# sandyresearch/chipmunk

Measured on AMD Instinct MI355X. Metric: DiT denoise steps/sec at fixed sparsity, higher is better.
Workload: dtype bf16

## Files before the change

chipmunk_amd/_native.py:

```python
from __future__ import annotations

import ctypes
import os

_HERE = os.path.dirname(os.path.abspath(__file__))
LIB_PATH = os.environ.get("CHIPMUNK_HIP_LIB") or os.path.join(_HERE, "lib", "libchipmunk_hip.so")

SYMBOLS = [
    "chipmunk_last_error", "chipmunk_abi_version", "chipmunk_set_option", "chipmunk_set_random_seed",
    "chipmunk_csp_attn", "chipmunk_csp_attn_out", "chipmunk_csp_128_attn", "chipmunk_dense_attn", "chipmunk_dense_colsum_attn",
    "chipmunk_csp_mlp_mm1", "chipmunk_csp_mlp_mm1_scatter", "chipmunk_csp_mlp_mm1_fp8", "chipmunk_csp_mlp_mm2_and_scatter_add", "chipmunk_csp_scatter_add", "chipmunk_csp_mlp_mm2",
    "chipmunk_csp_mlp_mm1_ragged", "chipmunk_csp_mlp_mm1_scatter_ragged", "chipmunk_csp_mlp_mm1_fp8_ragged", "chipmunk_csp_mlp_mm2_ragged",
    "chipmunk_csp_mlp_mm2_and_scatter_add_ragged", "chipmunk_csp_scatter_add_ragged", "chipmunk_block_mean_ragged", "chipmunk_transpose16_pitched",
    "chipmunk_topk_indices", "chipmunk_topk_delta_indices", "chipmunk_topk_mask", "chipmunk_mask_to_indices", "chipmunk_mask_to_sorted_indices", "chipmunk_packed_mask_to_indices", "chipmunk_copy_indices",
    "chipmunk_bitpack", "chipmunk_bitunpack", "chipmunk_transpose16", "chipmunk_block_mean", "chipmunk_quantize_fp8", "chipmunk_gather_rows", "chipmunk_qkv_split_norm", "chipmunk_dense_colsum_topk_mask", "chipmunk_dense_attn_strided", "chipmunk_csp_attn_out_ragged", "chipmunk_compact_indices", "chipmunk_residual_ln_modulate", "chipmunk_dense_colsum_attn_strided", "chipmunk_dense_colsum_topk_mask_strided", "chipmunk_release_scratch", "chipmunk_big_scratch_fallbacks",
    "chipmunk_host_alloc", "chipmunk_host_free", "chipmunk_copy_d2h_async", "chipmunk_copy_h2d_async", "chipmunk_host_bytes",
]

_lib = None


def lib() -> ctypes.CDLL:
    global _lib
    if _lib is None:
        if not os.path.exists(LIB_PATH):
            raise ImportError(
                f"{LIB_PATH} is missing: build it with `python -m chipmunk_amd.build` (hipcc --offload-arch=gfx950). "
                "chipmunk_amd has no CPU fallback.")
        _lib = ctypes.CDLL(LIB_PATH)
        _lib.chipmunk_last_error.restype = ctypes.c_char_p
        _lib.chipmunk_abi_version.restype = ctypes.c_int
        for item in filter(None, os.environ.get("CHIPMUNK_AMD_OPTIONS", "").split(",")):
            name, _, val = item.partition("=")
            if _lib.chipmunk_set_option(name.strip().encode(), int(val)) != 0:
                raise ValueError(f"CHIPMUNK_AMD_OPTIONS: {_lib.chipmunk_last_error().decode()}")
    return _lib


def last_error() -> str:
    return lib().chipmunk_last_error().decode()


def check(rc: int, what: str) -> None:
    if rc != 0:
        raise RuntimeError(f"{what}: {last_error()}")


def set_option(name: str, value: int) -> None:
    check(lib().chipmunk_set_option(name.encode(), int(value)), "chipmunk_set_option")


def manual_seed(seed: int) -> None:
    check(lib().chipmunk_set_random_seed(ctypes.c_uint64(int(seed) & 0xFFFFFFFFFFFFFFFF)), "chipmunk_set_random_seed")


class HostBuffer:

    def __init__(self, numel: int, dtype) -> None:
        import torch
        self.dtype = dtype
        self._numel = int(numel)
        self._itemsize = torch.empty(0, dtype=dtype).element_size()
        self.nbytes = self._numel * self._itemsize
        p = ctypes.c_void_p()
        check(lib().chipmunk_host_alloc(ctypes.c_size_t(max(self.nbytes, 1)), ctypes.byref(p)), "chipmunk_host_alloc")
        self.ptr = p.value

    def numel(self) -> int:
        return self._numel

    def element_size(self) -> int:
        return self._itemsize

    def is_pinned(self) -> bool:
        return True

    def free(self) -> None:
        if getattr(self, "ptr", None):
            lib().chipmunk_host_free(ctypes.c_void_p(self.ptr))
            self.ptr = None

    def __del__(self):
        try:
            self.free()
        except Exception:
            pass


def copy_d2h_async(host_ptr: int, dev_ptr: int, nbytes: int, stream: int) -> None:
    check(lib().chipmunk_copy_d2h_async(ctypes.c_void_p(host_ptr), ctypes.c_void_p(dev_ptr), ctypes.c_size_t(nbytes), ctypes.c_void_p(stream)),
          "chipmunk_copy_d2h_async")


def copy_h2d_async(dev_ptr: int, host_ptr: int, nbytes: int, stream: int) -> None:
    check(lib().chipmunk_copy_h2d_async(ctypes.c_void_p(dev_ptr), ctypes.c_void_p(host_ptr), ctypes.c_size_t(nbytes), ctypes.c_void_p(stream)),
          "chipmunk_copy_h2d_async")


def host_bytes() -> int:
    f = lib().chipmunk_host_bytes
    f.restype = ctypes.c_size_t
    return int(f())
```

chipmunk_amd/csrc/attn.hip:

```cpp
#include "common.h"
#include "attn_params.h"
#include <type_traits>

namespace {

constexpr int QG = 192;
constexpr int QW = 48;
constexpr int KVT = 32;
constexpr int NST = 4;
constexpr int KRING = 8;
constexpr int HD = 128;
constexpr int TILE_BYTES = KVT * HD * 2;
constexpr float SCALE_LOG2E = 0.08838834764f * 1.44269504089f;
constexpr int NSTV = NST + 1;
constexpr int KEY_RING_OFF = (NST + NSTV) * TILE_BYTES;
constexpr int CS_OFF = KEY_RING_OFF + KRING * 256;
constexpr int ATTN_LDS_BYTES = CS_OFF + 2 * 2 * 4 * KVT * 4;

__device__ __forceinline__ f32x4 mfma16(bf16x8 a, bf16x8 b, f32x4 c) {
    return __builtin_amdgcn_mfma_f32_16x16x32_bf16(a, b, c, 0, 0, 0);
}

#ifdef ATTN_PROF
__device__ unsigned long long g_attn_prof[8 * 8];
// ... 1062 lines not shown
    p.q = (const uint16_t *)q, p.k = (const uint16_t *)k, p.v = (const uint16_t *)v, p.o = (uint16_t *)o_out;
    p.o_in = (const uint16_t *)o_in;
    for (int i = 0; i < 3; ++i) p.qs[i] = q_strides[i], p.ks[i] = k_strides[i], p.vs[i] = v_strides[i], p.os[i] = o_strides[i];
    p.indices = indices, p.counts = counts;
    p.B = B, p.H = H, p.Nq = Nq, p.Nk = Nk, p.G = (Nq + QG - 1) / QG, p.idx_stride = idx_stride;
    p.o_scale = (float)o_scale;
    return launch_attn<true, true, false>(p, (hipStream_t)stream);
}

extern "C" int chipmunk_csp_attn_out_ragged(const void *q, const void *k, const void *v, const void *o_in, void *o_out,
                                            const int64_t q_strides[3], const int64_t k_strides[3], const int64_t v_strides[3],
                                            const int64_t o_strides[3], const int32_t *indices, const int64_t *idx_offsets,
                                            const int32_t *counts, int B, int H, int Nq, int Nk, int o_scale, void *stream) {
    if (int e = check_common(q, k, v, o_out, B, H, Nq, Nk)) return e;
    CM_CHECK(o_in != nullptr && ((uintptr_t)o_in & 15) == 0, "csp_attn_out_ragged: o_in missing or not 16-byte aligned");
    CM_CHECK(o_scale == 1 || o_scale == -1, "o_scale must be 1 or -1");
    CM_CHECK(indices && counts && idx_offsets, "csp_attn_out_ragged: indices / offsets / counts missing");
    CM_CHECK(((uintptr_t)indices & 15) == 0, "csp_attn_out_ragged: indices must be 16-byte aligned");
    if (int e = check_strides(q_strides, "q")) return e;
    if (int e = check_strides(k_strides, "k")) return e;
    if (int e = check_strides(v_strides, "v")) return e;
    if (int e = check_strides(o_strides, "o")) return e;
    AttnParams p = {};
    p.q = (const uint16_t *)q, p.k = (const uint16_t *)k, p.v = (const uint16_t *)v, p.o = (uint16_t *)o_out;
    p.o_in = (const uint16_t *)o_in;
    for (int i = 0; i < 3; ++i) p.qs[i] = q_strides[i], p.ks[i] = k_strides[i], p.vs[i] = v_strides[i], p.os[i] = o_strides[i];
    p.indices = indices, p.counts = counts, p.idx_off = idx_offsets;
    p.B = B, p.H = H, p.Nq = Nq, p.Nk = Nk, p.G = (Nq + QG - 1) / QG, p.idx_stride = 0;
    p.o_scale = (float)o_scale;
    return launch_attn<true, true, false>(p, (hipStream_t)stream);
}

extern "C" int chipmunk_csp_128_attn(const void *q, const void *k, const void *v, void *o, const int32_t *indices,
                                     const int32_t *counts, int B, int H, int Nq, int Nk, int idx_stride,
                                     void *stream) {
    if (int e = check_common(q, k, v, o, B, H, Nq, Nk)) return e;
    CM_CHECK(indices && counts, "csp_128_attn: indices / counts missing");
    AttnParams p = {};
    p.q = (const uint16_t *)q, p.k = (const uint16_t *)k, p.v = (const uint16_t *)v, p.o = (uint16_t *)o;
    contiguous_strides(p.qs, H, Nq), contiguous_strides(p.os, H, Nq);
    contiguous_strides(p.ks, H, Nk), contiguous_strides(p.vs, H, Nk);
    p.indices = indices, p.counts = counts;
    p.B = B, p.H = H, p.Nq = Nq, p.Nk = Nk, p.G = (Nq + QG - 1) / QG, p.idx_stride = idx_stride;
    p.o_scale = 1.f;
    return launch_attn<true, false, false>(p, (hipStream_t)stream);
}

static int output_strides(int64_t os[3], const int64_t *o_strides, int H, int Nq) {
    if (!o_strides) {
        contiguous_strides(os, H, Nq);
        return CHIPMUNK_OK;
    }
    for (int i = 0; i < 3; ++i) os[i] = o_strides[i];
    return check_strides(o_strides, "o");
}

extern "C" int chipmunk_dense_attn_strided(const void *q, const void *k, const void *v, const int64_t q_strides[3],
                                           const int64_t k_strides[3], const int64_t v_strides[3], void *o,
                                           const int64_t *o_strides, float *l, int B, int H, int Nq, int Nk, void *stream) {
    if (int e = check_common(q, k, v, o, B, H, Nq, Nk)) return e;
    CM_CHECK(l != nullptr, "dense_attn: l output missing");
    if (int e = check_strides(q_strides, "q")) return e;
    if (int e = check_strides(k_strides, "k")) return e;
    if (int e = check_strides(v_strides, "v")) return e;
    AttnParams p = {};
    p.q = (const uint16_t *)q, p.k = (const uint16_t *)k, p.v = (const uint16_t *)v, p.o = (uint16_t *)o;
    for (int i = 0; i < 3; ++i) p.qs[i] = q_strides[i], p.ks[i] = k_strides[i], p.vs[i] = v_strides[i];
    if (int e = output_strides(p.os, o_strides, H, Nq)) return e;
    p.l_out = l;
    p.B = B, p.H = H, p.Nq = Nq, p.Nk = Nk, p.G = (Nq + QG - 1) / QG;
    p.o_scale = 1.f;
    if (use_dense64(B, H, Nq, Nk)) {
        CM_CHECK((int64_t)Nk * p.ks[2] * 2 < (1ll << 32) && (int64_t)Nk * p.vs[2] * 2 < (1ll << 32),
                 "attention: one head's K or V spans more than 4 GiB (32-bit DMA offsets)");
        return chipmunk_dense64_launch(q, k, v, o, l, p.qs, p.ks, p.vs, p.os, B, H, Nq, Nk, (hipStream_t)stream);
    }
    return launch_attn<false, false, true>(p, (hipStream_t)stream);
}

extern "C" int chipmunk_dense_attn(const void *q, const void *k, const void *v, const int64_t q_strides[3],
                                   const int64_t k_strides[3], const int64_t v_strides[3], void *o, float *l, int B,
                                   int H, int Nq, int Nk, void *stream) {
    return chipmunk_dense_attn_strided(q, k, v, q_strides, k_strides, v_strides, o, nullptr, l, B, H, Nq, Nk, stream);
}

extern "C" int chipmunk_dense_colsum_attn_strided(const void *q, const void *k, const void *v, const int64_t q_strides[3],
                                                  const int64_t k_strides[3], const int64_t v_strides[3], const float *pin,
                                                  void *o, const int64_t *o_strides, void *cs, float *l, int B, int H, int Nq,
                                                  int Nk, int cs_stride, void *stream) {
    if (int e = check_common(q, k, v, o, B, H, Nq, Nk)) return e;
    CM_CHECK(l && cs && pin, "dense_colsum_attn: p / cs / l missing");
    CM_CHECK(cs_stride >= Nk, "dense_colsum_attn: cs row stride %d < Nk %d", cs_stride, Nk);
    if (int e = check_strides(q_strides, "q")) return e;
    if (int e = check_strides(k_strides, "k")) return e;
    if (int e = check_strides(v_strides, "v")) return e;
    AttnParams p = {};
    p.q = (const uint16_t *)q, p.k = (const uint16_t *)k, p.v = (const uint16_t *)v, p.o = (uint16_t *)o;
    for (int i = 0; i < 3; ++i) p.qs[i] = q_strides[i], p.ks[i] = k_strides[i], p.vs[i] = v_strides[i];
    if (int e = output_strides(p.os, o_strides, H, Nq)) return e;
    p.l_out = l, p.p_in = pin, p.cs = (uint16_t *)cs, p.cs_stride = cs_stride;
    p.B = B, p.H = H, p.Nq = Nq, p.Nk = Nk, p.G = (Nq + QG - 1) / QG;
    p.o_scale = 1.f;
    hipStream_t st = (hipStream_t)stream;
    int rc;
    if (chipmunk_get_option("attn_fused_colsum") == 5) {
        if (use_colsum64(B, H, Nq, Nk)) return chipmunk_colsum64_launch(p, st);
        return launch_attn<false, false, false, true>(p, st);
    }
    if (use_dense64(B, H, Nq, Nk)) {
        CM_CHECK((int64_t)Nk * p.ks[2] * 2 < (1ll << 32) && (int64_t)Nk * p.vs[2] * 2 < (1ll << 32),
                 "attention: one head's K or V spans more than 4 GiB (32-bit DMA offsets)");
        if (chipmunk_get_option("attn_fused_colsum") != 2) {
            int hc = H;
            uint16_t *part = nullptr;
            const int hc_min = chipmunk_get_option("attn_fused_colsum") == 4 ? 1 : 0;
            if (hc_min) hc = 1;
            for (; hc >= 1; hc /= 2) {
                part = (uint16_t *)chipmunk_big_scratch(st, chipmunk_colsum_part_bytes(hc == H ? B : 1, hc, Nq, Nk));
                if (part) break;
            }
            if (part && hc == H) return chipmunk_dense64_colsum_launch(p, part, st);
            if (part) {
                for (int b = 0; b < B; ++b)
                    for (int h0 = 0; h0 < H; h0 += hc) {
                        AttnParams c = p;
                        const int hn = H - h0 < hc ? H - h0 : hc;
                        const int64_t bh0 = (int64_t)b * H + h0;
                        c.q += b * p.qs[0] + h0 * p.qs[1], c.k += b * p.ks[0] + h0 * p.ks[1], c.v += b * p.vs[0] + h0 * p.vs[1];
                        c.o += b * p.os[0] + h0 * p.os[1];
                        c.l_out += bh0 * Nq, c.p_in += bh0 * Nq, c.cs += bh0 * p.G * (int64_t)cs_stride;
                        c.B = 1, c.H = hn;
                        if (int e = chipmunk_dense64_colsum_launch(c, part, st)) return e;
                    }
                return CHIPMUNK_OK;
            }
        }
        rc = chipmunk_dense64_launch(q, k, v, o, l, p.qs, p.ks, p.vs, p.os, B, H, Nq, Nk, st);
    } else {
        rc = launch_attn<false, false, true>(p, st);
    }
    if (rc != CHIPMUNK_OK) return rc;
    if (use_colsum64(B, H, Nq, Nk)) return chipmunk_colsum64_launch(p, st);
    return launch_attn<false, false, false, true>(p, st);
}

extern "C" int chipmunk_dense_colsum_attn(const void *q, const void *k, const void *v, const int64_t q_strides[3],
                                          const int64_t k_strides[3], const int64_t v_strides[3], const float *pin,
                                          void *o, void *cs, float *l, int B, int H, int Nq, int Nk, int cs_stride,
                                          void *stream) {
    return chipmunk_dense_colsum_attn_strided(q, k, v, q_strides, k_strides, v_strides, pin, o, nullptr, cs, l, B, H, Nq, Nk,
                                              cs_stride, stream);
}

extern "C" int chipmunk_dense_colsum_topk_mask_strided(const void *q, const void *k, const void *v, const int64_t q_strides[3],
                                               const int64_t k_strides[3], const int64_t v_strides[3], const float *pin, void *o,
                                               const int64_t *o_strides, float *l, int B, int H, int Nq, int Nk, const void *static_mask,
                                               int64_t static_stride, int static_rows, const void *group_flags, void *mask,
                                               int topk, double random_amount, void *stream) {
    if (int e = check_common(q, k, v, o, B, H, Nq, Nk)) return e;
    CM_CHECK(l && pin && mask, "dense_colsum_topk_mask: p / l / mask missing");
    if (int e = check_strides(q_strides, "q")) return e;
    if (int e = check_strides(k_strides, "k")) return e;
    if (int e = check_strides(v_strides, "v")) return e;
    hipStream_t st = (hipStream_t)stream;
    if (!use_dense64(B, H, Nq, Nk) || chipmunk_get_option("attn_fused_colsum") == 2 || (Nk & 3) || Nk > 1024 * 120)
        return CHIPMUNK_ERR_UNSUPPORTED;
    AttnParams p = {};
    p.q = (const uint16_t *)q, p.k = (const uint16_t *)k, p.v = (const uint16_t *)v, p.o = (uint16_t *)o;
    for (int i = 0; i < 3; ++i) p.qs[i] = q_strides[i], p.ks[i] = k_strides[i], p.vs[i] = v_strides[i];
    CM_CHECK((int64_t)Nk * p.ks[2] * 2 < (1ll << 32) && (int64_t)Nk * p.vs[2] * 2 < (1ll << 32),
             "attention: one head's K or V spans more than 4 GiB (32-bit DMA offsets)");
    if (int e = output_strides(p.os, o_strides, H, Nq)) return e;
    p.l_out = l, p.p_in = pin, p.cs = nullptr, p.cs_stride = 0;
    p.B = B, p.H = H, p.Nq = Nq, p.Nk = Nk, p.G = (Nq + QG - 1) / QG;
    p.o_scale = 1.f;
    uint16_t *part = (uint16_t *)chipmunk_big_scratch(st, chipmunk_colsum_part_bytes(B, H, Nq, Nk));
    if (!part) return CHIPMUNK_ERR_UNSUPPORTED;
    if (int e = chipmunk_dense64_colsum_launch(p, part, st)) return e;
    const int nrb = ((Nq + 255) / 256) * 2;
    return chipmunk_topk_mask_parts(part, chipmunk_colsum_part_stride(Nk), nrb, p.G, Nq, static_mask, static_stride, static_rows, group_flags, mask, B * H * p.G, Nk,
                                    topk, random_amount, st);
}

extern "C" int chipmunk_dense_colsum_topk_mask(const void *q, const void *k, const void *v, const int64_t q_strides[3],
                                               const int64_t k_strides[3], const int64_t v_strides[3], const float *pin, void *o,
                                               float *l, int B, int H, int Nq, int Nk, const void *static_mask,
                                               int64_t static_stride, int static_rows, const void *group_flags, void *mask,
                                               int topk, double random_amount, void *stream) {
    return chipmunk_dense_colsum_topk_mask_strided(q, k, v, q_strides, k_strides, v_strides, pin, o, nullptr, l, B, H, Nq, Nk,
                                                   static_mask, static_stride, static_rows, group_flags, mask, topk, random_amount,
                                                   stream);
}
```

chipmunk_amd/csrc/attn64.hip:

```cpp
#include "common.h"
#include "attn64_regs.h"
#include "attn_params.h"
#include "attn64_util.h"
#include <type_traits>

namespace {

constexpr int HD = 128;
constexpr int KT = 64;
constexpr int WROWS = 64, WGROWS = 256;
constexpr int TB = KT * HD * 2;
constexpr int NSL = 4;
constexpr int VRING = NSL * TB;
constexpr int LDS_BYTES = 2 * NSL * TB;
constexpr int PSTAGE = 64 * 128;
constexpr int LDS_BYTES_CSUM = LDS_BYTES + 4 * PSTAGE;
constexpr int CS_EXCH_BYTES = 2 * 4 * 64 * 4;
constexpr float SCALE_LOG2E = 0.08838834764f * 1.44269504089f;
constexpr float MAX_LAG = 4.0f;
#ifndef A64_ABL
#define A64_ABL 0
#endif
#ifndef A64_EB
#define A64_EB 20
#endif
#ifndef A64_EA
#define A64_EA 35
#endif
#ifndef A64_CSUM_VALU
#define A64_CSUM_VALU 1
#endif
#ifndef A64_VSPREAD
#define A64_VSPREAD 0
#endif
#ifndef A64_DMA_POS
#define A64_DMA_POS 2
#endif

constexpr int a64_ecum(int k) {
    return k <= 0 ? 0 : k <= 20 ? (k * A64_EB) / 20 : k <= 52 ? A64_EB + ((k - 20) * A64_EA) / 32
                                                              : (A64_EB + A64_EA + (k - 52) < 64 ? A64_EB + A64_EA + (k - 52) : 64);
}
constexpr int a64_cstep(int j) {
    int k = 0;
    while (a64_ecum(k) < 2 * j + 2) ++k;
    return k;
}
constexpr int a64_rk(int u) { return u == 0 ? 36 : u == 1 ? 38 : u == 2 ? 68 : 70; }
constexpr int a64_mk(int u) { return u == 0 ? 46 : u == 1 ? 48 : u == 2 ? 78 : 80; }

#ifdef ATTN64_PROF
__device__ unsigned long long g_a64_prof[4 * 8];
#define P64_DECL unsigned long long pt_ = 0, pacc_[7] = {0, 0, 0, 0, 0, 0, 0}; const bool prof_on_ = blockIdx.x == (gridDim.x / 2)
#define P64_START() do { if (prof_on_) pt_ = __builtin_amdgcn_s_memtime(); } while (0)
#define P64_MARK(i) do { if (prof_on_) { const unsigned long long n_ = __builtin_amdgcn_s_memtime(); pacc_[i] += n_ - pt_; pt_ = n_; } } while (0)
#define P64_END(w, n) do { if (prof_on_ && lane == 0) { for (int i_ = 0; i_ < 7; ++i_) g_a64_prof[(w) * 8 + i_] = pacc_[i_]; g_a64_prof[(w) * 8 + 7] = (n); } } while (0)
#else
#define P64_DECL
#define P64_START()
#define P64_MARK(i)
#define P64_END(w, n)
#endif

template <int KB, int QB, int KS>
__device__ __forceinline__ void mfma_qk(f32x16 &s) {
    constexpr int ka = 192 + (KB * 8 + KS) * 4, qa = 128 + (QB * 8 + KS) * 4;
    if constexpr (A64_ABL & 64) {
        constexpr int oa = (KB * 2 + QB) * 16;
        asm volatile("v_mfma_f32_32x32x16_bf16 a[%c0:%c1], a[%c2:%c3], a[%c4:%c5], a[%c0:%c1]" ::"i"(oa), "i"(oa + 15), "i"(ka), "i"(ka + 3), "i"(qa), "i"(qa + 3));
        return;
    }
    if constexpr (KS == 0)
        asm volatile("v_mfma_f32_32x32x16_bf16 %0, a[%c1:%c2], a[%c3:%c4], 0" : "=v"(s) : "i"(ka), "i"(ka + 3), "i"(qa), "i"(qa + 3));
    else
        asm volatile("v_mfma_f32_32x32x16_bf16 %0, a[%c1:%c2], a[%c3:%c4], %0" : "+v"(s) : "i"(ka), "i"(ka + 3), "i"(qa), "i"(qa + 3));
}
template <int QB, int DB>
__device__ __forceinline__ void mfma_pv(const u32x4 &vf, const u32x4 &pf) {
    constexpr int oa = (QB * 4 + DB) * 16;
    asm volatile("v_mfma_f32_32x32x16_bf16 a[%c2:%c3], %0, %1, a[%c2:%c3]" ::"v"(vf), "v"(pf), "i"(oa), "i"(oa + 15));
}
template <int KB, int KS, int SLOT>
__device__ __forceinline__ void lds_k(uint32_t addr) {
    constexpr int ka = 192 + (KB * 8 + KS) * 4;
    asm volatile("ds_read_b128 a[%c1:%c2], %0 offset:%c3" ::"v"(addr), "i"(ka), "i"(ka + 3), "i"(SLOT * TB + KB * 8192) : "memory");
}
__device__ __forceinline__ void cs_pair16x2(float &a, float &b, float &c, float &d) {
    asm volatile("v_permlane16_swap_b32 %0, %1\n\tv_permlane16_swap_b32 %2, %3\n\tv_add_f32 %0, %0, %1\n\tv_add_f32 %2, %2, %3"
                 : "+v"(a), "+v"(b), "+v"(c), "+v"(d));
}
__device__ __forceinline__ void cs_pair8(float &a, const float &b) {
    asm volatile("v_add_f32_dpp %0, %0, %0 row_mirror row_mask:0xf bank_mask:0x3\n\t"
                 "v_add_f32_dpp %0, %1, %1 row_mirror row_mask:0xf bank_mask:0xc" : "+v"(a) : "v"(b));
}
__device__ __forceinline__ void cs_pair4(float &a, const float &b) {
    asm volatile("v_add_f32_dpp %0, %0, %0 row_half_mirror row_mask:0xf bank_mask:0x5\n\t"
                 "v_add_f32_dpp %0, %1, %1 row_half_mirror row_mask:0xf bank_mask:0xa" : "+v"(a) : "v"(b));
}
template <int CTRL>
__device__ __forceinline__ float cs_pair_quad(float a, float b, bool hi) {
    const float keep = hi ? b : a, give = hi ? a : b;
    return keep + __uint_as_float((uint32_t)__builtin_amdgcn_update_dpp(0, (int)__float_as_uint(give), CTRL, 0xf, 0xf, true));
}
__global__ __launch_bounds__(256) void knorm_max_kernel(const uint16_t *k, const int64_t ks0, const int64_t ks1, const int64_t ks2, int H, int Nk,
                                                        float *out) {
    const int bh = blockIdx.y, b = bh / H, h = bh - b * H;
    const uint16_t *kb = k + b * ks0 + h * ks1;
    const int grp = threadIdx.x >> 4, li = threadIdx.x & 15;
    float best = 0.f;
#pragma unroll 4
    for (int row = blockIdx.x * 16 + grp; row < Nk; row += gridDim.x * 16) {
        const u32x4 v = *(const u32x4 *)(kb + (int64_t)row * ks2 + li * 8);
        float ss = 0.f;
#pragma unroll
        for (int e = 0; e < 4; ++e) {
            const float lo = __uint_as_float(v[e] << 16), hi = __uint_as_float(v[e] & 0xffff0000u);
            ss = __builtin_fmaf(lo, lo, ss);
            ss = __builtin_fmaf(hi, hi, ss);
        }
        best = fmaxf(best, row16_sum(ss));
    }
    __shared__ float red[256];
    red[threadIdx.x] = best;
    __syncthreads();
    for (int st = 128; st > 0; st >>= 1) {
        if ((int)threadIdx.x < st) red[threadIdx.x] = fmaxf(red[threadIdx.x], red[threadIdx.x + st]);
        __syncthreads();
    }
    if (threadIdx.x == 0) atomicMax((unsigned int *)(out + bh), __float_as_uint(__builtin_sqrtf(red[0])));
}

template <int MODE>
__global__ __launch_bounds__(256) __attribute__((amdgpu_waves_per_eu(1, 1))) void attn64_kernel(const AttnParams p) {
    constexpr bool GATHER = MODE == 1 || MODE == 2, INPLACE = MODE == 2;
    constexpr bool CSUM = MODE == 3;
    extern __shared__ __attribute__((aligned(16))) unsigned char smem[];
    const int tid = threadIdx.x, lane = tid & 63;
    const int w = __builtin_amdgcn_readfirstlane(tid >> 6);
    const int l31 = lane & 31, hf = lane >> 5, l15 = lane & 15, lg = lane >> 4;
    int wid = blockIdx.x, sp = 0, nsp = 1, slot0 = 0, tix = 0;
    if constexpr (GATHER) {
        const int wid0 = wid;
        wid = p.plan[2 * wid0];
        if (wid < 0) return;
        const int meta = p.plan[2 * wid0 + 1];
        sp = meta & 0xff, nsp = (meta >> 8) & 0xff;
        slot0 = tix = meta >> 16;
    }
    const int bh = wid / p.G, g = wid - bh * p.G;
    const int b = bh / p.H, h = bh - b * p.H;
    const int row0 = g * (GATHER ? 192 : WGROWS) + w * WROWS;
    const int count = GATHER ? p.counts[(int64_t)bh * p.G + g] : p.Nk;
    const int valid = count < p.Nk ? count : p.Nk;
    const int ntiles_all = (valid + KT - 1) / KT;
    const int tbeg = (int)((int64_t)ntiles_all * sp / nsp), tend = (int)((int64_t)ntiles_all * (sp + 1) / nsp);
    const int ntiles = tend - tbeg;
    const int T4 = (ntiles + 3) & ~3;

    const uint16_t *kbase = p.k + b * p.ks[0] + h * p.ks[1];
    const uint16_t *vbase = p.v + b * p.vs[0] + h * p.vs[1];
    const __amdgpu_buffer_rsrc_t krsrc = make_rsrc(kbase), vrsrc = make_rsrc(vbase);
    const uint32_t kstride_b = (uint32_t)p.ks[2] * 2u, vstride_b = (uint32_t)p.vs[2] * 2u;

    if (GATHER && w == 3) {
        const IndexRow irow = index_row(p, (int64_t)bh * p.G + g);
        const int32_t *idx = irow.ptr;
        uint32_t kswz[4];
#pragma unroll
        for (int i = 0; i < 4; ++i) kswz[i] = (uint32_t)(l15 ^ (4 * i + lg)) << 4;
        const uint32_t vswz = (uint32_t)(l15 ^ (lg << 2)) << 4;
        int ir[4][16];
        const bool idx_vec = ((uintptr_t)idx & 15) == 0 && (irow.width & 3) == 0;
        auto load_idx = [&](int T, int (&dst)[16]) {
            const int base = (tbeg + T) * KT + lg * 16;
            if (idx_vec && (tbeg + T) * KT + KT <= irow.width) {
#pragma unroll
                for (int j4 = 0; j4 < 4; ++j4) {
                    const u32x4 v4 = *(const u32x4 *)(idx + base + j4 * 4);
#pragma unroll
                    for (int e = 0; e < 4; ++e) dst[j4 * 4 + e] = (int)v4[e];
                }
            } else {
#pragma unroll
                for (int j = 0; j < 16; ++j) {
                    int pos = base + j;
                    pos = pos < irow.width ? pos : irow.width - 1;
                    dst[j] = idx[pos];
                }
            }
#pragma unroll
            for (int j = 0; j < 16; ++j) dst[j] = max(0, min(dst[j], p.Nk - 1));
        };
        auto all_k = [&](const int (&src)[16], int slot) {
#pragma unroll
            for (int pc = 0; pc < 16; ++pc) blds16(krsrc, __umul24((uint32_t)src[pc], kstride_b) + kswz[pc & 3], 0, smem + slot * TB + pc * 1024);
        };
        auto all_v = [&](const int (&src)[16], int slot) {
#pragma unroll
            for (int pc = 0; pc < 16; ++pc) blds16(vrsrc, __umul24((uint32_t)src[pc], vstride_b) + vswz, 0, smem + VRING + slot * TB + pc * 1024);
        };
        load_idx(0, ir[0]), load_idx(1, ir[1]), load_idx(2, ir[2]), load_idx(3, ir[3]);
        all_k(ir[0], 0);
        all_k(ir[1], 1), all_v(ir[0], 3);
        all_k(ir[2], 2), all_v(ir[0], 0);
        all_k(ir[3], 3), all_v(ir[1], 1);
        load_idx(4, ir[0]);
        asm volatile("s_waitcnt vmcnt(0)" ::: "memory");
        __syncthreads();
        auto loader_tile = [&](auto slc, int t) __attribute__((always_inline)) {
            constexpr int SL = decltype(slc)::value;
            asm volatile("s_waitcnt vmcnt(63)" ::: "memory");
            __builtin_amdgcn_s_barrier();
            load_idx(t + 5, ir[(SL + 1) & 3]);
            all_k(ir[SL], SL);
            all_v(ir[(SL + 2) & 3], (SL + 2) & 3);
        };
        for (int tb = 0;; tb += 4) {
            loader_tile(ic<0>{}, tb);
            if (tb >= T4) break;
            loader_tile(ic<1>{}, tb + 1);
            loader_tile(ic<2>{}, tb + 2);
            loader_tile(ic<3>{}, tb + 3);
        }
        asm volatile("s_waitcnt vmcnt(0)" ::: "memory");
        if (nsp > 1) {
            __syncthreads();
            __syncthreads();
            if (*(volatile int *)(smem) != nsp - 1) return;
            __syncthreads();
        }
        return;
    }

    asm volatile(A64_ZERO_O ::: A64_CLOBBER_ALL);
    float qss[2] = {0.f, 0.f};
    {
        const uint16_t *qp = p.q + b * p.qs[0] + h * p.qs[1];
        static_for<0, 16>([&](auto f) {
            constexpr int F = decltype(f)::value, qb = F >> 3, ks = F & 7;
            const int qrow = row0 + qb * 32 + l31;
            u32x4 val = {0u, 0u, 0u, 0u};
            if (qrow < p.Nq) val = *(const u32x4 *)(qp + (int64_t)qrow * p.qs[2] + ks * 16 + hf * 8);
            acc_write4<128 + F * 4>(val);
#pragma unroll
            for (int e = 0; e < 4; ++e) {
                const float lo = __uint_as_float(val[e] << 16), hi = __uint_as_float(val[e] & 0xffff0000u);
                qss[qb] = __builtin_fmaf(lo, lo, qss[qb]);
                qss[qb] = __builtin_fmaf(hi, hi, qss[qb]);
            }
        });
    }

    const uint32_t lds0 = (uint32_t)(uintptr_t)(__attribute__((address_space(3))) unsigned char *)smem;
    uint32_t kad[8];
#pragma unroll
    for (int ks = 0; ks < 8; ++ks) kad[ks] = lds0 + l31 * 256 + (((2 * ks + hf) ^ l15) << 4);
    uint32_t vad[4];
#pragma unroll
    for (int db = 0; db < 4; ++db)
        vad[db] = lds0 + VRING + (4 * hf + (l15 >> 2)) * 256 + (((db * 4 + 2 * (lg & 1) + ((l15 & 3) >> 1)) ^ ((l15 >> 2) << 2)) << 4) +
                  (l15 & 1) * 8;
    uint32_t kofs[4];
#pragma unroll
    for (int i = 0; i < 4; ++i) kofs[i] = (uint32_t)(w * 16 + 4 * i + lg) * kstride_b + ((uint32_t)(l15 ^ (4 * i + lg)) << 4);
    const uint32_t vofs = (uint32_t)(w * 16 + lg) * vstride_b + ((uint32_t)(l15 ^ (lg << 2)) << 4);

    const int last_base = p.Nk - KT;
    auto tile_base = [&](int T) { return T * KT < last_base ? T * KT : last_base; };
    auto issue_k1 = [&](uint32_t soff, uint32_t ldsw, int slot, int i) {
        blds16(krsrc, kofs[i], soff, smem + ldsw + slot * TB + i * 1024);
    };
    auto issue_v1 = [&](uint32_t soff, uint32_t ldsw, int slot, int i) {
        blds16(vrsrc, vofs, soff + (uint32_t)(4 * i) * vstride_b, smem + ldsw + VRING + slot * TB + i * 1024);
    };
    auto issue_k = [&](int T, int slot) {
        const uint32_t soff = (uint32_t)tile_base(T) * kstride_b;
#pragma unroll
        for (int i = 0; i < 4; ++i) issue_k1(soff, w * 4096, slot, i);
    };
    auto issue_v = [&](int T, int slot) {
        const uint32_t soff = (uint32_t)tile_base(T) * vstride_b;
#pragma unroll
        for (int i = 0; i < 4; ++i) issue_v1(soff, w * 4096, slot, i);
    };

    if constexpr (!GATHER) {
        issue_k(0, 0);
        issue_k(1, 1), issue_v(0, 3);
        issue_k(2, 2), issue_v(0, 0);
        issue_k(3, 3), issue_v(1, 1);
        asm volatile("s_waitcnt vmcnt(24)" ::: "memory");
    }
    __syncthreads();
    static_for<0, 16>([&](auto i) {
        constexpr int I = decltype(i)::value;
        lds_k<(I >> 3), (I & 7), 0>(kad[I & 7]);
    });
    asm volatile("s_waitcnt lgkmcnt(0)" ::: "memory");

    f32x16 s[4];
    float px[64];
    uint32_t pw[2][4][4] = {};
    float m[2] = {-INFINITY, -INFINITY}, nmsc[2] = {0.f, 0.f};
    float mlag[2] = {-INFINITY, -INFINITY};
    float lacc[2][2] = {{0.f, 0.f}, {0.f, 0.f}};
    float alpha[2] = {1.f, 1.f};
    float wq[2] = {0.f, 0.f}, lpq[2] = {-1.0e30f, -1.0e30f}, c4[2] = {0.f, 0.f}, c5 = 0.f;
    uint32_t csoff = 0, ex_w = 0, ex_r = 0;
    int cs_extra = 0;
    float cs_own = 0.f;
    __amdgpu_buffer_rsrc_t prsrc = krsrc;
    uint32_t pst_w = 0, pst_r = 0, csoff_mx = 0;
    u32x2 csf[8] = {};
    f32x4 csacc[2] = {{0.f, 0.f, 0.f, 0.f}, {0.f, 0.f, 0.f, 0.f}};
    float csout = 0.f;
    u32x4 cs_ones = {0x3f803f80u, 0x3f803f80u, 0x3f803f80u, 0x3f803f80u};
    if constexpr (CSUM) {
        static_assert(A64_CSUM_VALU, "the matrix-pipe column-sum probe (A64_CSUM_VALU=0) fills all 160 KiB of LDS with its P stage: no room for the exchange area of the in-workgroup combine; build round 5's tree for it");
        pin(cs_ones);
        const uint32_t pst = lds0 + LDS_BYTES + (uint32_t)w * PSTAGE;
        pst_w = pst + l31 * 128 + ((uint32_t)(hf ^ (l31 & 7)) << 4);
        const int prow = lg * 4 + (l15 >> 2);
        pst_r = pst + prow * 128 + ((uint32_t)(((l15 & 3) >> 1) ^ (prow & 7)) << 4) + (l15 & 1) * 8;
        csoff_mx = 2u * (uint32_t)(16 * lg + 8 * ((l15 >> 2) & 1) + 4 * (l15 >> 3) + (l15 & 3));
#pragma unroll
        for (int qb = 0; qb < 2; ++qb) {
            const int qrow = row0 + qb * 32 + l31;
            const float pl = qrow < p.Nq ? p.p_in[(int64_t)bh * p.Nq + qrow] : 0.f;
            lpq[qb] = pl > 0.f ? __builtin_amdgcn_logf(pl) : -1.0e30f;
        }
        const int rr = ((lane >> 4) & 1) | (((lane >> 3) & 1) << 1) | (((lane >> 2) & 1) << 2);
        csoff = 2u * (uint32_t)(32 * (lane & 1) + (rr & 3) + 8 * (2 * ((lane >> 1) & 1) + (rr >> 2)) + 4 * hf);
        const int nA = 3 - (4 * g) % 3;
        const int lead = w < nA ? 0 : nA, members = w < nA ? nA : 4 - nA;
        cs_extra = w == lead ? members : 0;
        ex_w = lds0 + LDS_BYTES + (uint32_t)w * 256u + (uint32_t)lane * 4u;
        ex_r = lds0 + LDS_BYTES + (uint32_t)(lead + 1) * 256u + (uint32_t)lane * 4u;
        prsrc = make_rsrc(p.cs_part + ((int64_t)bh * (p.G * 2) + (g * 2 + (w < nA ? 0 : 1))) * p.cs_pstride);
    }
#pragma unroll
    for (int e = 0; e < 64; ++e) px[e] = e < 20 ? 0.f : -INFINITY;

    auto vfrag_read = [&](auto dbc, auto offc) __attribute__((always_inline)) {
        constexpr int DB = decltype(dbc)::value, OFF = decltype(offc)::value;
        u32x2 lo, hi;
        asm volatile("ds_read_b64_tr_b16 %0, %2 offset:%c3\n\tds_read_b64_tr_b16 %1, %2 offset:%c4"
                     : "=&v"(lo), "=&v"(hi) : "v"(vad[DB]), "i"(OFF), "i"(OFF + 2048) : "memory");
        return (u32x4){lo[0], lo[1], hi[0], hi[1]};
    };

    static_assert(64 - A64_EB - A64_EA >= 0 && 64 - A64_EB - A64_EA <= 9, "the last steps must finish before gap 12 of the next PV phase");
    auto ecum = [](int k) constexpr { return a64_ecum(k); };
    auto finish_step = [&](auto kk, auto uwc) __attribute__((always_inline)) {
        constexpr int K = decltype(kk)::value;
        constexpr bool UW = decltype(uwc)::value != 0;
        if constexpr (!(A64_ABL & 1)) {
            static_for<ecum(K), ecum(K + 1)>([&](auto ii) {
                constexpr int I = decltype(ii)::value;
                if constexpr (A64_ABL & 32) px[I] = px[I] * 0.5f;
                else px[I] = __builtin_amdgcn_exp2f(px[I]);
                pin(px[I]);
            });
            static_for<ecum(K - 1), ecum(K)>([&](auto ii) {
                constexpr int I = decltype(ii)::value;
                lacc[(I >> 3) & 1][I & 1] += px[I];
                pin(lacc[(I >> 3) & 1][I & 1]);
            });
            static_for<(ecum(K - 1) >> 1), (ecum(K) >> 1)>([&](auto jj) {
                constexpr int J = decltype(jj)::value, I = 2 * J;
                pw[(I >> 3) & 1][I >> 4][(I & 7) >> 1] = pack_bf16x2(px[I], px[I + 1]);
                pin(pw[(I >> 3) & 1][I >> 4][(I & 7) >> 1]);
            });
            if constexpr (CSUM && UW && !A64_CSUM_VALU) {
                static_assert(a64_cstep(8 * 1 + 7) + 1 < a64_rk(0) && a64_cstep(8 * 3 + 7) + 1 < a64_rk(2), "a unit is read after its second fragment is stored");
                static_for<0, 4>([&](auto uu) {
                    constexpr int U = decltype(uu)::value, S = (U & 1) * 4;
                    if constexpr (K == a64_mk(U) || K == a64_mk(U) + 1) {
                        constexpr int H2 = K - a64_mk(U);
                        if constexpr (H2 == 0 && (U & 1) == 0)
                            asm volatile("s_waitcnt lgkmcnt(0)" : "+v"(csf[0]), "+v"(csf[1]), "+v"(csf[2]), "+v"(csf[3]), "+v"(csf[4]), "+v"(csf[5]), "+v"(csf[6]), "+v"(csf[7]) :: "memory");
                        const u32x4 fr = {csf[S + 2 * H2][0], csf[S + 2 * H2][1], csf[S + 2 * H2 + 1][0], csf[S + 2 * H2 + 1][1]};
                        if constexpr (H2 == 0) asm volatile("v_mfma_f32_16x16x32_bf16 %0, %1, %2, 0" : "=&v"(csacc[U & 1]) : "v"(cs_ones), "v"(fr));
                        else asm volatile("v_mfma_f32_16x16x32_bf16 %0, %1, %2, %0" : "+v"(csacc[U & 1]) : "v"(cs_ones), "v"(fr));
                    }
                    if constexpr (K == a64_mk(U) + 3) {
                        if constexpr (U == 0) csout = csacc[0][0];
                        else csout = lg == U ? csacc[U & 1][0] : csout;
                        pin(csout);
                    }
                    if constexpr (K == a64_rk(U) || K == a64_rk(U) + 1) {
                        constexpr int H2 = K - a64_rk(U);
                        uint32_t ad = pst_r;
                        if constexpr (U != 0) ad ^= (uint32_t)(U << 5);
                        asm volatile("ds_read_b64_tr_b16 %0, %2 offset:%c3\n\tds_read_b64_tr_b16 %1, %2 offset:%c4"
                                     : "=&v"(csf[S + 2 * H2]), "=&v"(csf[S + 2 * H2 + 1]) : "v"(ad), "i"(H2 * 4096), "i"(H2 * 4096 + 2048) : "memory");
                    }
                });
                static_for<0, 8>([&](auto ii) {
                    constexpr int U = decltype(ii)::value >> 1, QW = decltype(ii)::value & 1;
                    if constexpr (K == a64_cstep(8 * U + 4 * QW + 3) + 1) {
                        uint32_t ad = pst_w;
                        if constexpr (U != 0) ad ^= (uint32_t)(U << 5);
                        const u32x4 pf = {pw[QW][U][0], pw[QW][U][1], pw[QW][U][2], pw[QW][U][3]};
                        asm volatile("ds_write_b128 %0, %1 offset:%c2" ::"v"(ad), "v"(pf), "i"(QW * 4096) : "memory");
                    }
                });
            } else if constexpr (CSUM) {
                static_for<ecum(K - 3), ecum(K - 2)>([&](auto ii) {
                    constexpr int I = decltype(ii)::value;
                    if constexpr (UW) {
                        if constexpr (((I >> 3) & 1) == 1) { px[I] += px[I - 8]; pin(px[I]); }
                    } else {
                        if constexpr (((I >> 3) & 1) == 0) px[I] *= wq[0];
                        else px[I] = __builtin_fmaf(px[I], wq[1], px[I - 8]);
                        pin(px[I]);
                    }
                });
                static_for<ecum(K - 4), ecum(K - 3)>([&](auto ii) {
                    constexpr int I = decltype(ii)::value;
                    if constexpr ((I & 11) == 11) cs_pair16x2(px[I - 3], px[I - 2], px[I - 1], px[I]);
                });
                static_for<ecum(K - 5), ecum(K - 4)>([&](auto ii) {
                    constexpr int I = decltype(ii)::value;
                    if constexpr ((I & 11) == 11) cs_pair8(px[I - 3], px[I - 1]);
                });
                static_for<ecum(K - 6), ecum(K - 5)>([&](auto ii) {
                    constexpr int I = decltype(ii)::value;
                    if constexpr ((I & 15) == 15) cs_pair4(px[I - 7], px[I - 3]);
                });
                static_for<ecum(K - 7), ecum(K - 6)>([&](auto ii) {
                    constexpr int I = decltype(ii)::value;
                    if constexpr ((I & 31) == 31) { c4[I >> 5] = cs_pair_quad<0x4E>(px[I - 23], px[I - 7], (lane & 2) != 0); pin(c4[I >> 5]); }
                });
                static_for<ecum(K - 8), ecum(K - 7)>([&](auto ii) {
                    constexpr int I = decltype(ii)::value;
                    if constexpr (I == 63) { c5 = cs_pair_quad<0xB1>(c4[0], c4[1], (lane & 1) != 0); pin(c5); }
                });
            }
        }
    };

    P64_DECL;
    P64_START();
    auto tile = [&](auto slc, auto nmc, int t) __attribute__((always_inline)) {
        constexpr int SL = decltype(slc)::value;
        constexpr bool NOMAX = decltype(nmc)::value != 0;
        constexpr auto uwc = ic<(CSUM && decltype(nmc)::value == 2) ? 1 : 0>{};
        constexpr int VSL = (SL + 3) & 3;
        constexpr int KNSL = (SL + 1) & 3;
        uint32_t ldsw = w * 4096, ksoff = 0, vsoff = 0;
        if constexpr (!(A64_ABL & 16)) {
            if constexpr (!(A64_ABL & 256) && !GATHER) asm volatile("s_waitcnt vmcnt(16)" ::: "memory");
            if constexpr (!(A64_ABL & 128)) __builtin_amdgcn_s_barrier();
            if constexpr (!GATHER) {
                asm volatile("" : "+s"(ldsw));
                ksoff = (uint32_t)tile_base(t + 4) * kstride_b;
                vsoff = (uint32_t)tile_base(t + 2) * vstride_b;
            }
        }
        __builtin_amdgcn_sched_barrier(0);
        P64_MARK(0);

        u32x4 vf[16];
        static_for<0, 32>([&](auto gg) {
            constexpr int G = decltype(gg)::value;
            constexpr int ks = G >> 2, kb = (G >> 1) & 1, qb = G & 1;
            mfma_qk<kb, qb, ks>(s[kb * 2 + qb]);
            if constexpr (!(A64_ABL & 16) && !GATHER && ((A64_DMA_POS == 0 && G < 8) || (A64_DMA_POS == 2 && G >= 16 && (G & 1) == 0))) {
                constexpr int PC = A64_DMA_POS == 0 ? G : (G - 16) >> 1;
                if constexpr (PC < 4) issue_k1(ksoff, ldsw, SL, PC);
                else issue_v1(vsoff, ldsw, (SL + 2) & 3, PC - 4);
            }
            finish_step(ic<20 + G>{}, uwc);
            if constexpr (A64_VSPREAD ? (G & 1) == 0 : G < 16) {
                constexpr int f = A64_VSPREAD ? G >> 1 : G;
                if constexpr (A64_ABL & 4) vf[f] = (u32x4){(uint32_t)t, 1u, 2u, 3u};
                else vf[f] = vfrag_read(ic<(f & 3)>{}, ic<VSL * TB + (f >> 2) * 4096>{});
            }
            __builtin_amdgcn_sched_barrier(0);
        });
        P64_MARK(1);
        asm volatile("s_waitcnt lgkmcnt(0)"
                     : "+v"(vf[0]), "+v"(vf[1]), "+v"(vf[2]), "+v"(vf[3]), "+v"(vf[4]), "+v"(vf[5]), "+v"(vf[6]), "+v"(vf[7]), "+v"(vf[8]),
                       "+v"(vf[9]), "+v"(vf[10]), "+v"(vf[11]), "+v"(vf[12]), "+v"(vf[13]), "+v"(vf[14]), "+v"(vf[15]));
        __builtin_amdgcn_sched_barrier(0);
        P64_MARK(2);

        float mx[2];
        bool moved = false;
        const int dead = GATHER ? 0 : (t * KT - tile_base(t) < KT ? t * KT - tile_base(t) : KT);
        const int vleft = !GATHER ? KT : (t < ntiles ? valid - (tbeg + t) * KT : 0);
        auto phase_b_gap = [&](auto gg) __attribute__((always_inline)) {
            constexpr int G = decltype(gg)::value;
            constexpr int up = G >> 3, db = (G >> 1) & 3, qb = G & 1;
            const u32x4 pf = {pw[qb][up][0], pw[qb][up][1], pw[qb][up][2], pw[qb][up][3]};
            mfma_pv<qb, db>(vf[G >> 1], pf);
            constexpr bool UWT = decltype(uwc)::value != 0 && !A64_CSUM_VALU;
            if constexpr (G < (CSUM ? (UWT ? 32 : 17) : 12)) finish_step(ic<52 + G>{}, uwc);
            if constexpr (CSUM && G == (UWT ? 31 : 17)) {
                const uint32_t par2 = (uint32_t)(t & 1) * 1024u;
                const float mine = UWT ? csout : c5;
                if (!cs_extra) {
                    asm volatile("ds_write_b32 %0, %1" ::"v"(ex_w + (par2 ^ 1024u)), "v"(mine) : "memory");
                } else {
                    float x1 = 0.f, x2 = 0.f;
                    if (cs_extra >= 2) asm volatile("ds_read_b32 %0, %1" : "=v"(x1) : "v"(ex_r + par2) : "memory");
                    if (cs_extra >= 3) asm volatile("ds_read_b32 %0, %1 offset:256" : "=v"(x2) : "v"(ex_r + par2) : "memory");
                    asm volatile("ds_write_b32 %0, %1" ::"v"(ex_w + (par2 ^ 1024u)), "v"(mine) : "memory");
                    asm volatile("s_waitcnt lgkmcnt(1)" : "+v"(x1), "+v"(x2)::"memory");
                    const int tb2 = tile_base(t - 2), dd = (t - 2) * KT - tb2;
                    if (t > 1 && dd < KT) {
                        const uint32_t off = UWT ? csoff_mx : csoff;
                        if (dd <= 0 || (int)(off >> 1) >= dd) {
                            const uint16_t val = (uint16_t)(pack_bf16x2((cs_own + x1) + x2, 0.f) & 0xffffu);
                            if (p.probe & 16) __builtin_amdgcn_raw_buffer_store_b16(val, prsrc, off, (uint32_t)tb2 * 2u, 2);
                            else __builtin_amdgcn_raw_buffer_store_b16(val, prsrc, off, (uint32_t)tb2 * 2u, 0);
                        }
                    }
                }
                cs_own = mine;
            }
            if constexpr (!(A64_ABL & 16) && !GATHER && A64_DMA_POS == 1 && G >= 16 && (G & 1) == 0) {
                constexpr int PC = (G - 16) >> 1;
                if constexpr (PC < 4) issue_k1(ksoff, ldsw, SL, PC);
                else issue_v1(vsoff, ldsw, (SL + 2) & 3, PC - 4);
            }
            if constexpr (G < 16 && !(A64_ABL & 8)) {
                constexpr int J = G;
                lds_k<(J >> 3), (J & 7), KNSL>(kad[J & 7]);
            }
            if constexpr (G == 1 && !(A64_ABL & 2)) {
                if (!GATHER && __builtin_expect(dead > 0, 0)) {
                    int thr = dead - 4 * hf;
                    asm volatile("" : "+v"(thr));
#pragma unroll
                    for (int blk = 0; blk < 4; ++blk)
#pragma unroll
                        for (int r = 0; r < 16; ++r)
                            if ((blk >> 1) * 32 + (r & 3) + 8 * (r >> 2) < thr) s[blk][r] = -INFINITY;
                }
                if (GATHER && __builtin_expect(vleft < KT, 0)) {
                    int thr = vleft - hf;
                    asm volatile("" : "+v"(thr));
#pragma unroll
                    for (int blk = 0; blk < 4; ++blk)
#pragma unroll
                        for (int r = 0; r < 16; ++r)
                            if ((r & 3) * 16 + (blk >> 1) * 8 + 2 * (r >> 2) >= thr) s[blk][r] = -INFINITY;
                }
            }
            if constexpr (G >= 2 && G <= 9 && !(A64_ABL & 2) && !NOMAX) {
                constexpr int j = G - 2;
                constexpr int kb2 = j >> 2, r0 = (j & 3) * 4;
                if constexpr (j == 0)
                    asm volatile("v_max_f32 %0, %2, %3\n\tv_max_f32 %1, %6, %7\n\tv_max3_f32 %0, %0, %4, %5\n\tv_max3_f32 %1, %1, %8, %9"
                                 : "=&v"(mx[0]), "=&v"(mx[1])
                                 : "v"(s[0][0]), "v"(s[0][1]), "v"(s[0][2]), "v"(s[0][3]), "v"(s[1][0]), "v"(s[1][1]), "v"(s[1][2]), "v"(s[1][3]));
                else
                asm volatile("v_max3_f32 %0, %0, %2, %3\n\tv_max3_f32 %1, %1, %6, %7\n\tv_max3_f32 %0, %0, %4, %5\n\tv_max3_f32 %1, %1, %8, %9"
                             : "+v"(mx[0]), "+v"(mx[1])
                             : "v"(s[kb2 * 2][r0]), "v"(s[kb2 * 2][r0 + 1]), "v"(s[kb2 * 2][r0 + 2]), "v"(s[kb2 * 2][r0 + 3]),
                               "v"(s[kb2 * 2 + 1][r0]), "v"(s[kb2 * 2 + 1][r0 + 1]), "v"(s[kb2 * 2 + 1][r0 + 2]), "v"(s[kb2 * 2 + 1][r0 + 3]));
            }
            if constexpr (G == 10 && !(A64_ABL & 2) && !NOMAX) {
#pragma unroll
                for (int q2 = 0; q2 < 2; ++q2) {
                    float a = mx[q2], c = mx[q2];
                    lane_swap32(a, c);
                    mx[q2] = max2(a, c);
                    pin(mx[q2]);
                }
            }
            if constexpr (G >= 12 && G < 28 && !(A64_ABL & 2)) {
                static_for<(G - 12) * 4, (G - 11) * 4>([&](auto ii) {
                    constexpr int I = decltype(ii)::value;
                    constexpr int blk = (I >> 5) * 2 + ((I >> 3) & 1), r = ((I >> 4) & 1) * 8 + (I & 7);
                    px[I] = __builtin_fmaf(s[blk][r], SCALE_LOG2E, nmsc[(I >> 3) & 1]);
                    pin(px[I]);
                });
            }
            if constexpr (G >= 12) finish_step(ic<G - 12>{}, uwc);
            __builtin_amdgcn_sched_barrier(0);
        };
        static_for<0, 12>(phase_b_gap);
        P64_MARK(3);
        if constexpr (!(A64_ABL & 2) && !NOMAX) {
            constexpr float LAG_RAW = MAX_LAG / SCALE_LOG2E;
            if (__builtin_amdgcn_ballot_w64(mx[0] > mlag[0]) | __builtin_amdgcn_ballot_w64(mx[1] > mlag[1])) {
                moved = true;
#pragma unroll
                for (int q2 = 0; q2 < 2; ++q2) {
                    const float m_new = max2(m[q2], mx[q2]);
                    alpha[q2] = __builtin_amdgcn_exp2f((m[q2] - m_new) * SCALE_LOG2E);
                    lacc[q2][0] *= alpha[q2];
                    lacc[q2][1] *= alpha[q2];
                    m[q2] = m_new;
                    nmsc[q2] = -m_new * SCALE_LOG2E;
                    mlag[q2] = m_new + LAG_RAW;
                    if constexpr (CSUM) wq[q2] = fminf(__builtin_amdgcn_exp2f(m_new * SCALE_LOG2E + lpq[q2]), 1.0e37f);
                }
            }
        }
        __builtin_amdgcn_sched_barrier(0);
        P64_MARK(4);
        static_for<12, 32>(phase_b_gap);
        P64_MARK(5);
        if (__builtin_expect(moved, 0)) {
            float tmp;
            asm volatile("s_nop 7\n\ts_nop 7\n\ts_nop 7\n\t" A64_SCALE_QB0 : "=&v"(tmp) : "v"(alpha[0]));
            asm volatile(A64_SCALE_QB1 : "=&v"(tmp) : "v"(alpha[1]));
        }
        asm volatile("s_waitcnt lgkmcnt(0)" ::: "memory");
        __builtin_amdgcn_sched_barrier(0);
        P64_MARK(6);
    };

    bool nomax = false;
    if constexpr (!GATHER) {
        if (p.kmax) {
            const float km = p.kmax[bh];
            bool ok = true;
#pragma unroll
            for (int qb = 0; qb < 2; ++qb) {
                float a = qss[qb], c2 = qss[qb];
                lane_swap32(a, c2);
                const float mq = __builtin_sqrtf(a + c2) * km;
                ok = ok && (2.0f * mq * SCALE_LOG2E <= 64.0f);
                qss[qb] = mq;
            }
            nomax = __builtin_amdgcn_ballot_w64(!ok) == 0;
            if (nomax) {
#pragma unroll
                for (int qb = 0; qb < 2; ++qb) {
                    m[qb] = qss[qb], nmsc[qb] = -qss[qb] * SCALE_LOG2E, mlag[qb] = INFINITY;
                    if constexpr (CSUM) wq[qb] = fminf(__builtin_amdgcn_exp2f(qss[qb] * SCALE_LOG2E + lpq[qb]), 1.0e37f);
                }
            }
        }
    }
    bool unitw = false;
    if constexpr (CSUM) {
        if (nomax && !(p.probe & 4)) {
            bool ok = true;
#pragma unroll
            for (int qb = 0; qb < 2; ++qb) ok = ok && lpq[qb] > -1.0e29f && qss[qb] * SCALE_LOG2E + __builtin_fabsf(lpq[qb]) <= 80.0f;
            unitw = __builtin_amdgcn_ballot_w64(!ok) == 0;
            if (unitw) {
#pragma unroll
                for (int qb = 0; qb < 2; ++qb) m[qb] = -lpq[qb] / SCALE_LOG2E, nmsc[qb] = lpq[qb];
            }
        }
    }
    if (CSUM && unitw) {
        if constexpr (CSUM) {
            for (int tb = 0;; tb += 4) {
                tile(ic<0>{}, ic<2>{}, tb);
                if (tb >= T4) break;
                tile(ic<1>{}, ic<2>{}, tb + 1);
                tile(ic<2>{}, ic<2>{}, tb + 2);
                tile(ic<3>{}, ic<2>{}, tb + 3);
            }
        }
    } else if (nomax) {
        for (int tb = 0;; tb += 4) {
            tile(ic<0>{}, ic<1>{}, tb);
            if (tb >= T4) break;
            tile(ic<1>{}, ic<1>{}, tb + 1);
            tile(ic<2>{}, ic<1>{}, tb + 2);
            tile(ic<3>{}, ic<1>{}, tb + 3);
        }
    } else {
        for (int tb = 0;; tb += 4) {
            tile(ic<0>{}, ic<0>{}, tb);
            if (tb >= T4) break;
            tile(ic<1>{}, ic<0>{}, tb + 1);
            tile(ic<2>{}, ic<0>{}, tb + 2);
            tile(ic<3>{}, ic<0>{}, tb + 3);
        }
    }
    asm volatile("s_waitcnt vmcnt(0)" ::: "memory");
    P64_END(w, T4 + 1);
    if constexpr (CSUM) {
        asm volatile("s_waitcnt lgkmcnt(0)" ::: "memory");
        __builtin_amdgcn_s_barrier();
        if (cs_extra) {
            float x1 = 0.f, x2 = 0.f;
            const uint32_t par = (uint32_t)((T4 - 1) & 1) * 1024u;
            if (cs_extra >= 2) asm volatile("ds_read_b32 %0, %1" : "=v"(x1) : "v"(ex_r + par) : "memory");
            if (cs_extra >= 3) asm volatile("ds_read_b32 %0, %1 offset:256" : "=v"(x2) : "v"(ex_r + par) : "memory");
            asm volatile("s_waitcnt lgkmcnt(0)" : "+v"(x1), "+v"(x2)::"memory");
            const int tb1 = tile_base(T4 - 1), dd = (T4 - 1) * KT - tb1;
            const uint32_t off = (unitw && !A64_CSUM_VALU) ? csoff_mx : csoff;
            if (dd < KT && (dd <= 0 || (int)(off >> 1) >= dd))
                __builtin_amdgcn_raw_buffer_store_b16((uint16_t)(pack_bf16x2((cs_own + x1) + x2, 0.f) & 0xffffu), prsrc, off, (uint32_t)tb1 * 2u, 0);
        }
    }

    asm volatile("s_nop 7\n\ts_nop 7\n\ts_nop 7" ::: "memory");
    float o[128];
    static_for<0, 32>([&](auto ii) {
        constexpr int I = decltype(ii)::value;
        const f32x4 o4 = acc_read4<I * 4>();
        o[I * 4 + 0] = o4[0], o[I * 4 + 1] = o4[1], o[I * 4 + 2] = o4[2], o[I * 4 + 3] = o4[3];
    });
    float lq[2];
#pragma unroll
    for (int qb = 0; qb < 2; ++qb) {
        float lp = lacc[qb][0] + lacc[qb][1], lo2 = lp;
        lane_swap32(lp, lo2);
        lq[qb] = lp + lo2;
    }

    if constexpr (GATHER) {
        if (nsp > 1) {
            constexpr int SLICE_FLOATS = 26 * 256 * 4;
            int *ticket_s = (int *)smem;
            float *mine = p.ws + (int64_t)(slot0 + sp) * SLICE_FLOATS + tid;
#pragma unroll
            for (int i = 0; i < 128; ++i) mine[i * 192] = o[i];
            mine[128 * 192] = m[0], mine[129 * 192] = m[1], mine[130 * 192] = lq[0], mine[131 * 192] = lq[1];
            __syncthreads();
            if (tid == 0) {
                __builtin_amdgcn_fence(__ATOMIC_RELEASE, "agent");
                asm volatile("s_waitcnt vmcnt(0)" ::: "memory");
                *ticket_s = __hip_atomic_fetch_add(p.tickets + tix, 1, __ATOMIC_RELAXED, __HIP_MEMORY_SCOPE_AGENT);
            }
            __syncthreads();
            if (*ticket_s != nsp - 1) return;
            if (tid == 0) {
                __hip_atomic_store(p.tickets + tix, 0, __ATOMIC_RELAXED, __HIP_MEMORY_SCOPE_AGENT);
                __builtin_amdgcn_fence(__ATOMIC_ACQUIRE, "agent");
            }
            __syncthreads();
#pragma unroll
            for (int i = 0; i < 128; ++i) o[i] = 0.f;
            m[0] = m[1] = -INFINITY, lq[0] = lq[1] = 0.f;
            for (int s2 = 0; s2 < nsp; ++s2) {
                const float *oth = p.ws + (int64_t)(slot0 + s2) * SLICE_FLOATS + tid;
#pragma unroll
                for (int qb = 0; qb < 2; ++qb) {
                    const float ms = oth[(128 + qb) * 192], ls = oth[(130 + qb) * 192];
                    const float m_new = fmaxf(m[qb], ms);
                    if (m_new == -INFINITY) continue;
                    const float a = __builtin_amdgcn_exp2f((m[qb] - m_new) * SCALE_LOG2E);
                    const float c = __builtin_amdgcn_exp2f((ms - m_new) * SCALE_LOG2E);
                    m[qb] = m_new;
                    lq[qb] = lq[qb] * a + ls * c;
#pragma unroll
                    for (int i = 0; i < 64; ++i) o[qb * 64 + i] = o[qb * 64 + i] * a + oth[(qb * 64 + i) * 192] * c;
                }
            }
        }
    }

#pragma unroll
    for (int qb = 0; qb < 2; ++qb) {
        const float l = lq[qb];
        const float inv = l > 0.f ? __builtin_amdgcn_rcpf(l) : 0.f;
        const int qrow = row0 + qb * 32 + l31;
        if (qrow >= p.Nq) continue;
        const int64_t ooff = b * p.os[0] + h * p.os[1] + (int64_t)qrow * p.os[2] + 4 * hf;
        uint16_t *op = p.o + ooff;
#pragma unroll
        for (int i = 0; i < 16; ++i) {
            const int db = i >> 2, r4 = i & 3;
            const float *o4 = o + (qb * 4 + db) * 16 + r4 * 4;
            float x0 = o4[0] * inv, x1 = o4[1] * inv, x2 = o4[2] * inv, x3 = o4[3] * inv;
            u32x2 out;
            if constexpr (INPLACE) {
                const u32x2 old = *(const u32x2 *)(p.o_in + ooff + db * 32 + r4 * 8);
                const float a0 = round_bf16(x0 * p.o_scale), a1 = round_bf16(x1 * p.o_scale);
                const float a2 = round_bf16(x2 * p.o_scale), a3 = round_bf16(x3 * p.o_scale);
                out[0] = pack_bf16x2(__uint_as_float(old[0] << 16) + a0, __uint_as_float(old[0] & 0xffff0000u) + a1);
                out[1] = pack_bf16x2(__uint_as_float(old[1] << 16) + a2, __uint_as_float(old[1] & 0xffff0000u) + a3);
            } else {
                out[0] = pack_bf16x2(x0, x1);
                out[1] = pack_bf16x2(x2, x3);
            }
            *(u32x2 *)(op + db * 32 + r4 * 8) = out;
        }
        if (!GATHER && p.l_out && hf == 0)
            p.l_out[(int64_t)bh * p.Nq + qrow] = 1.0f / (__builtin_amdgcn_exp2f(m[qb] * SCALE_LOG2E) * l);
    }
}

template <int QB, int KB, int KS>
__device__ __forceinline__ void mfma_cs(f32x16 &d, const f32x16 &c0) {
    constexpr int qa = (QB * 8 + KS) * 4, ka = 192 + (KB * 8 + KS) * 4;
    if constexpr (KS == 0)
        asm volatile("v_mfma_f32_32x32x16_bf16 %0, a[%c2:%c3], a[%c4:%c5], %1" : "=&v"(d) : "v"(c0), "i"(qa), "i"(qa + 3), "i"(ka), "i"(ka + 3));
    else
        asm volatile("v_mfma_f32_32x32x16_bf16 %0, a[%c1:%c2], a[%c3:%c4], %0" : "+v"(d) : "i"(qa), "i"(qa + 3), "i"(ka), "i"(ka + 3));
}

__global__ __launch_bounds__(256) __attribute__((amdgpu_waves_per_eu(1, 1))) void colsum64_kernel(const AttnParams p) {
    extern __shared__ __attribute__((aligned(16))) unsigned char smem[];
    const int tid = threadIdx.x, lane = tid & 63;
    const int w = __builtin_amdgcn_readfirstlane(tid >> 6);
    const int l31 = lane & 31, hf = lane >> 5, l15 = lane & 15, lg = lane >> 4;
    const int G4 = (p.G + 3) / 4;
    const int wid = blockIdx.x;
    const int bh = __builtin_amdgcn_readfirstlane(wid / G4), g = (wid - bh * G4) * 4 + w;
    const int b = __builtin_amdgcn_readfirstlane(bh / p.H), h = bh - b * p.H;
    const int row0 = g * 192;
    const int ntiles = (p.Nk + KT - 1) / KT;
    const int T4 = (ntiles + 3) & ~3;
    const uint16_t *kbase = p.k + b * p.ks[0] + h * p.ks[1];
    const __amdgpu_buffer_rsrc_t krsrc = make_rsrc(kbase);
    const uint32_t kstride_b = (uint32_t)p.ks[2] * 2u;

    asm volatile("" ::: A64_CLOBBER_ALL);
    {
        const uint16_t *qp = p.q + b * p.qs[0] + h * p.qs[1];
        static_for<0, 48>([&](auto f) {
            constexpr int F = decltype(f)::value, qb = F >> 3, ks = F & 7;
            const int qrow = row0 + qb * 32 + l31;
            bf16x8 val = {};
            if (g < p.G && qrow < p.Nq) val = *(const bf16x8 *)(qp + (int64_t)qrow * p.qs[2] + ks * 16 + hf * 8);
#pragma unroll
            for (int e = 0; e < 8; ++e) val[e] = (__bf16)((float)val[e] * SCALE_LOG2E);
            acc_write4<F * 4>(__builtin_bit_cast(u32x4, val));
        });
    }
    f32x16 offs[6];
#pragma unroll
    for (int qb = 0; qb < 6; ++qb)
#pragma unroll
        for (int r = 0; r < 16; ++r) {
            const int qr = row0 + qb * 32 + (r & 3) + 8 * (r >> 2) + 4 * hf;
            const float pl = (g < p.G && qr < p.Nq) ? p.p_in[(int64_t)bh * p.Nq + qr] : 0.f;
            offs[qb][r] = pl > 0.f ? __builtin_amdgcn_logf(pl) : -1.0e30f;
        }

    const uint32_t lds0 = (uint32_t)(uintptr_t)(__attribute__((address_space(3))) unsigned char *)smem;
    uint32_t kad[8];
#pragma unroll
    for (int ks = 0; ks < 8; ++ks) kad[ks] = lds0 + l31 * 256 + (((2 * ks + hf) ^ l15) << 4);
    uint32_t kofs[4];
#pragma unroll
    for (int i = 0; i < 4; ++i) kofs[i] = (uint32_t)(w * 16 + 4 * i + lg) * kstride_b + ((uint32_t)(l15 ^ (4 * i + lg)) << 4);
    const int last_base = p.Nk - KT;
    auto tile_base = [&](int T) { return T * KT < last_base ? T * KT : last_base; };
// ... 203 lines not shown
```

chipmunk_amd/csrc/attn_params.h:

```cpp
#pragma once
#include <stdint.h>
#include <hip/hip_runtime.h>

struct AttnParams {
    const uint16_t *q, *k, *v;
    uint16_t *o;
    const uint16_t *o_in;
    int64_t qs[3], ks[3], vs[3], os[3];
    const int32_t *indices, *counts;
    const int64_t *idx_off;
    float *l_out;
    const float *p_in;
    uint16_t *cs;
    int cs_stride;
    int B, H, Nq, Nk, G, idx_stride;
    float o_scale;
    int split_full, nsplit;
    float *ws;
    int32_t *tickets;
    const int32_t *plan;
    int xcd_chunks;
    const float *kmax;
    uint16_t *cs_part;
    int cs_pstride;
    int probe;
};


int chipmunk_csp64_launch(const AttnParams &p, int inplace, int grid, hipStream_t stream);
int chipmunk_dense64_colsum_launch(const AttnParams &p, uint16_t *part, hipStream_t stream);
int chipmunk_topk_mask_parts(const uint16_t *part, int part_stride, int nrb, int groups_per_bh, int Nq, const void *static_mask, int64_t static_stride,
                             int static_rows, const void *group_flags, void *mask, int rows, int n, int k, double random_amount,
                             hipStream_t stream);
size_t chipmunk_colsum_part_bytes(int B, int H, int Nq, int Nk);
int chipmunk_colsum_part_stride(int Nk);
int chipmunk_colsum64_launch(const AttnParams &p, hipStream_t stream);
int chipmunk_csp96_launch(const AttnParams &p, int inplace, int grid, hipStream_t stream);
const float *chipmunk_knorm_max(const uint16_t *k, const int64_t ks[3], int B, int H, int Nk, hipStream_t stream);

__host__ __device__ inline int colsum_part_rows(int j, int nwg, int &r0, int &r1) {
    const int a = (3 * j) >> 2, w0 = 3 * j - 4 * a;
    r0 = 2 * a + (w0 ? 1 : 0);
    r1 = 2 * (a + 1);
    return (w0 >= 2 && a + 1 < nwg) ? 2 : 1;
}

struct IndexRow {
    const int32_t *ptr;
    int width;
};
__device__ __forceinline__ IndexRow index_row(const AttnParams &p, int64_t item) {
    if (p.idx_off) {
        const int64_t o = p.idx_off[item];
        return {p.indices + o, (int)(p.idx_off[item + 1] - o)};
    }
    return {p.indices + item * p.idx_stride, p.idx_stride};
}
```

chipmunk_amd/csrc/indexed_io.hip:

```cpp
#include "common.h"
#include "attn_params.h"

namespace {

__device__ __forceinline__ uint32_t wave_incl_scan(uint32_t x) {
    x += (uint32_t)__builtin_amdgcn_update_dpp(0, (int)x, 0x111, 0xf, 0xf, true);
    x += (uint32_t)__builtin_amdgcn_update_dpp(0, (int)x, 0x112, 0xf, 0xf, true);
    x += (uint32_t)__builtin_amdgcn_update_dpp(0, (int)x, 0x114, 0xf, 0xf, true);
    x += (uint32_t)__builtin_amdgcn_update_dpp(0, (int)x, 0x118, 0xf, 0xf, true);
    x += (uint32_t)__builtin_amdgcn_update_dpp(0, (int)x, 0x142, 0xa, 0xf, false);
    x += (uint32_t)__builtin_amdgcn_update_dpp(0, (int)x, 0x143, 0xc, 0xf, false);
    return x;
}
struct M2IParams {
    const uint8_t *mask;
    int32_t *indices;
    int32_t *counts;
    int n, pad_n, multiple_of;
};

template <bool PACKED, bool SORTED = false>
__global__ __launch_bounds__(256) void mask_to_indices_kernel(const M2IParams p) {
    extern __shared__ __attribute__((aligned(16))) unsigned char smem[];
    const int n = p.n;
// ... 321 lines not shown
#pragma unroll
        for (int j = 0; j < 16; ++j)
            if (keepbits & (1u << j)) {
                const int c = pass0 + j * 1024 + tid;
                out[base + tot[j * 16 + w] + before[j]] = c;
                if constexpr (DELTA) xc[c] = x[c];
            }
        base += tot[256];
        __syncthreads();
    }
    const int kept = base;
    const int mod = kept % p.multiple_of;
    const int pad = mod == 0 ? 0 : p.multiple_of - mod;
    if (tid == 0) p.counts[row] = kept + pad;
    if (pad > 0) {
        int pbase = 0;
        const int slot = compact_slot(my_last_invalid != -1, lane, w, wave_tot, pbase);
        if (slot >= 0 && slot < pad) {
            out[kept + slot] = my_last_invalid;
            if constexpr (DELTA) xc[my_last_invalid] = x[my_last_invalid];
        }
    }
}

template <typename T>
__global__ __launch_bounds__(256) void copy_indices_kernel(const T *src, T *dst, const int32_t *inds,
                                                           const int32_t *counts, int M, int R, int F) {
    const int64_t grow = blockIdx.x;
    const int64_t b = grow / ((int64_t)M * R);
    const int base_m = (int)((grow % ((int64_t)M * R)) / R);
    const int cnt = counts[b * M + base_m];
    const int32_t *ii = inds + (b * M + base_m) * (int64_t)F;
    for (int c = threadIdx.x; c < cnt; c += 256) {
        const int col = ii[c];
        dst[grow * F + col] = src[grow * F + col];
    }
}

__global__ __launch_bounds__(256) void bitpack_kernel(const uint8_t *mask, uint8_t *packed, int64_t n) {
    const int64_t nb = (n + 7) >> 3;
    for (int64_t i = (int64_t)blockIdx.x * 256 + threadIdx.x; i < nb; i += (int64_t)gridDim.x * 256) {
        uint8_t byte = 0;
        if (i * 8 + 8 <= n && ((((uintptr_t)mask) & 7) == 0)) {
            unsigned long long v = *(const unsigned long long *)(mask + i * 8);
#pragma unroll
            for (int j = 0; j < 8; ++j) byte |= (uint8_t)((((v >> (8 * j)) & 0xffull) != 0) << j);
        } else {
            for (int j = 0; j < 8 && i * 8 + j < n; ++j) byte |= (uint8_t)((mask[i * 8 + j] != 0) << j);
        }
        packed[i] = byte;
    }
}
__global__ __launch_bounds__(256) void bitunpack_kernel(const uint8_t *packed, uint8_t *mask, int64_t n) {
    const int64_t nb = (n + 7) >> 3;
    for (int64_t i = (int64_t)blockIdx.x * 256 + threadIdx.x; i < nb; i += (int64_t)gridDim.x * 256) {
        const uint8_t byte = packed[i];
        if (i * 8 + 8 <= n && ((((uintptr_t)mask) & 7) == 0)) {
            unsigned long long v = 0;
#pragma unroll
            for (int j = 0; j < 8; ++j) v |= (unsigned long long)((byte >> j) & 1u) << (8 * j);
            *(unsigned long long *)(mask + i * 8) = v;
        } else {
            for (int j = 0; j < 8 && i * 8 + j < n; ++j) mask[i * 8 + j] = (byte >> j) & 1u;
        }
    }
}

__global__ __launch_bounds__(256) void transpose16_kernel(const uint16_t *src, uint16_t *dst, int R, int C, int ld) {
    __shared__ __attribute__((aligned(16))) uint16_t tile[64][72];
    const int64_t boff = (int64_t)blockIdx.z * R * C;
    const int r0 = blockIdx.y * 64, c0 = blockIdx.x * 64;
    const int tid = threadIdx.x;
#pragma unroll
    for (int i = 0; i < 2; ++i) {
        const int item = i * 256 + tid, r = item >> 3, ch = item & 7;
        u32x4 v = {0u, 0u, 0u, 0u};
        if (r0 + r < R && c0 + ch * 8 + 8 <= C) v = *(const u32x4 *)(src + boff + (int64_t)(r0 + r) * C + c0 + ch * 8);
        else if (r0 + r < R)
            for (int e = 0; e < 8; ++e)
                if (c0 + ch * 8 + e < C) {
                    const uint32_t x = src[boff + (int64_t)(r0 + r) * C + c0 + ch * 8 + e];
                    v[e >> 1] |= x << (16 * (e & 1));
                }
#pragma unroll
        for (int e = 0; e < 4; ++e) {
            tile[ch * 8 + 2 * e][r] = (uint16_t)(v[e] & 0xffffu);
            tile[ch * 8 + 2 * e + 1][r] = (uint16_t)(v[e] >> 16);
        }
    }
    __syncthreads();
#pragma unroll
    for (int i = 0; i < 2; ++i) {
        const int item = i * 256 + tid, c = item >> 3, ch = item & 7;
        if (c0 + c >= C) continue;
        uint16_t *d = dst + (int64_t)blockIdx.z * C * ld + (int64_t)(c0 + c) * ld + r0 + ch * 8;
        if (r0 + ch * 8 + 8 <= ld && ((ld & 7) == 0)) *(u32x4 *)d = *(const u32x4 *)&tile[c][ch * 8];
        else
            for (int e = 0; e < 8; ++e)
                if (r0 + ch * 8 + e < ld) d[e] = tile[c][ch * 8 + e];
    }
}

__global__ __launch_bounds__(256) void compact_indices_kernel(const int32_t *indices, int64_t idx_stride, const int32_t *counts,
                                                             const int64_t *offsets, int32_t *flat) {
    const int64_t r = blockIdx.x;
    const int32_t *src = indices + r * idx_stride;
    const int64_t o = offsets[r];
    int32_t *dst = flat + o;
    const int width = (int)(offsets[r + 1] - o);
    int c = counts[r];
    c = c < 0 ? 0 : (c < width ? c : width);
    c = c < idx_stride ? c : (int)idx_stride;
    if ((((uintptr_t)src | (uintptr_t)dst) & 15) == 0) {
        const int c4 = c >> 2;
        for (int i = threadIdx.x; i < c4; i += 256) ((u32x4 *)dst)[i] = ((const u32x4 *)src)[i];
        for (int i = (c4 << 2) + threadIdx.x; i < c; i += 256) dst[i] = src[i];
    } else {
        for (int i = threadIdx.x; i < c; i += 256) dst[i] = src[i];
    }
    for (int i = c + threadIdx.x; i < width; i += 256) dst[i] = 0;
}

size_t m2i_lds_bytes(int n, bool sorted) {
    const int NI = (n + 31) >> 5, NB = (NI + 63) >> 6;
    if (sorted) return (size_t)NB * 64 * 4 + (size_t)(NB + 1) * 4 + 16;
    return (size_t)NB * 64 * 4 + (size_t)32 * NB * 8 + (size_t)32 * NB * 4 + 33 * 4 + 16;
}

template <bool PACKED, bool SORTED = false>
int launch_m2i(const void *mask, int32_t *indices, int32_t *counts, int64_t rows, int n, int pad_n, int multiple_of,
               void *stream) {
    CM_CHECK(mask && indices && counts, "mask_to_indices: null pointer");
    CM_CHECK(rows >= 0 && n > 0 && pad_n >= n && multiple_of > 0, "mask_to_indices: bad sizes rows=%lld n=%d pad_n=%d multiple_of=%d",
             (long long)rows, n, pad_n, multiple_of);
    CM_CHECK(rows < (1ll << 31), "mask_to_indices: too many rows");
    if (PACKED) CM_CHECK(n % 8 == 0, "packed_mask_to_indices: n must be a multiple of 8 (got %d)", n);
    const size_t lds = m2i_lds_bytes(n, SORTED);
    CM_CHECK(lds <= 160 * 1024, "mask_to_indices: row length %d needs %zu B of LDS (> 160 KiB)", n, lds);
    if (rows == 0) return CHIPMUNK_OK;
    auto kern = mask_to_indices_kernel<PACKED, SORTED>;
    if (lds > 64 * 1024) (void)hipFuncSetAttribute((const void *)kern, hipFuncAttributeMaxDynamicSharedMemorySize, (int)lds);
    M2IParams p = {(const uint8_t *)mask, indices, counts, n, pad_n, multiple_of};
    hipLaunchKernelGGL(kern, dim3((unsigned)rows), dim3(256), lds, (hipStream_t)stream, p);
    CM_LAUNCH_CHECK();
    return CHIPMUNK_OK;
}


struct TopkMaskParams {
    const uint16_t *cs;
    const uint8_t *stat;
    const uint8_t *groups;
    uint8_t *mask;
    int64_t cs_stride, stat_stride;
    int rows, n, k, stat_rows;
    float random_amount;
    uint32_t salt;
    const uint16_t *parts;
    int64_t pstride;
    int nrb, ngroups, nq;
};

__device__ __forceinline__ uint32_t bf16_key(uint32_t u) {
    return (u & 0x8000u) ? (~u & 0xffffu) : (u | 0x8000u);
}

template <int KPT, bool ALIGNED, bool PARTS = false>
__global__ __launch_bounds__(1024) void topk_mask_kernel(const TopkMaskParams p) {
    constexpr int NV = KPT / 4;
    __shared__ int wave_cnt[16];
    const int tid = threadIdx.x, lane = tid & 63, w = tid >> 6;
    const int row = blockIdx.x;
    const int n = p.n;
    const uint16_t *x = nullptr;
    int prow = 1;
    int64_t row1 = 0;
    if constexpr (PARTS) {
        const int bh = row / p.ngroups, g = row - bh * p.ngroups;
        int r0, r1;
        prow = colsum_part_rows(g, p.nrb / 2, r0, r1);
        x = p.parts + ((int64_t)bh * p.nrb + r0) * p.pstride;
        row1 = (int64_t)(r1 - r0) * p.pstride;
    } else {
        x = p.cs + (int64_t)row * p.cs_stride;
    }
    const uint32_t lane_off8 = 8u * (uint32_t)tid;
    const uint32_t lane_off4 = 4u * (uint32_t)tid;
    uint32_t key[NV][2];
    constexpr int LB = NV % 10 == 0 ? 10 : (NV % 8 == 0 ? 8 : (NV % 6 == 0 ? 6 : 4));
    static_assert(NV % LB == 0, "NV must split into whole load batches");
#pragma unroll
    for (int j0 = 0; j0 < NV; j0 += LB) {
        uint32_t raw[LB][2];
#pragma unroll
        for (int jj = 0; jj < LB; ++jj) {
            const int c = 4 * tid + 4096 * (j0 + jj);
            uint32_t v0 = 0xffffffffu, v1 = 0xffffffffu;
            if constexpr (ALIGNED) {
                if (c < n) {
                    const u32x2 v = *(const u32x2 *)((const unsigned char *)(x + 4096 * (j0 + jj)) + lane_off8);
                    v0 = v[0], v1 = v[1];
                    if constexpr (PARTS) {
                        if (prow == 2) {
                            float a0 = __uint_as_float(v0 << 16), a1 = __uint_as_float(v0 & 0xffff0000u);
                            float a2 = __uint_as_float(v1 << 16), a3 = __uint_as_float(v1 & 0xffff0000u);
                            const u32x2 y = *(const u32x2 *)((const unsigned char *)(x + row1 + 4096 * (j0 + jj)) + lane_off8);
                            a0 += __uint_as_float(y[0] << 16), a1 += __uint_as_float(y[0] & 0xffff0000u);
                            a2 += __uint_as_float(y[1] << 16), a3 += __uint_as_float(y[1] & 0xffff0000u);
                            v0 = pack_bf16x2(a0, a1), v1 = pack_bf16x2(a2, a3);
                        }
                    }
                }
            } else if (c < n) {
                v0 = v1 = 0;
#pragma unroll
                for (int e = 0; e < 4; ++e) {
                    const uint32_t u = c + e < n ? x[c + e] : 0xffffu;
                    if (e < 2) v0 |= u << (16 * e);
                    else v1 |= u << (16 * (e - 2));
                }
            }
            raw[jj][0] = v0, raw[jj][1] = v1;
        }
#pragma unroll
        for (int jj = 0; jj < LB; ++jj) {
            key[j0 + jj][0] = bf16_key(raw[jj][0] & 0xffffu) | (bf16_key(raw[jj][0] >> 16) << 16);
            key[j0 + jj][1] = bf16_key(raw[jj][1] & 0xffffu) | (bf16_key(raw[jj][1] >> 16) << 16);
        }
        __builtin_amdgcn_sched_barrier(0);
    }
    auto block_count = [&](int mine) {
#pragma unroll
        for (int d = 32; d > 0; d >>= 1) mine += __shfl_xor(mine, d);
        if (lane == 0) wave_cnt[w] = mine;
        __syncthreads();
        int t = 0;
#pragma unroll
        for (int i = 0; i < 16; ++i) t += wave_cnt[i];
        __syncthreads();
        return t;
    };
    const bool active = p.groups == nullptr || p.groups[row] != 0;
    const int k = p.k < n ? p.k : n;
    uint32_t thr = 0x10000u;
    int ties_to_take = 0;
    if (active && k > 0) {
        uint32_t res = 0;
        for (int bit = 15; bit >= 0; --bit) {
            const uint32_t cand = res | (1u << bit);
            const uint32_t cm1 = (cand - 1u) | ((cand - 1u) << 16);
            const uint32_t one2 = 0x00010001u;
            uint32_t cnt2 = 0;
#pragma unroll
            for (int j = 0; j < NV; ++j)
#pragma unroll
                for (int h = 0; h < 2; ++h) {
                    uint32_t d;
                    asm volatile("v_pk_sub_u16 %0, %1, %2 clamp\n\tv_pk_min_u16 %0, %0, %3" : "=&v"(d) : "v"(key[j][h]), "v"(cm1), "v"(one2));
                    asm volatile("v_pk_add_u16 %0, %0, %1" : "+v"(cnt2) : "v"(d));
                }
            const int mine = (int)(cnt2 & 0xffffu) + (int)(cnt2 >> 16);
            if (block_count(mine) >= k) res = cand;
        }
        thr = res;
        int gt = 0;
#pragma unroll
        for (int j = 0; j < NV; ++j)
#pragma unroll
            for (int h = 0; h < 2; ++h) {
                uint32_t kw = key[j][h];
                asm volatile("" : "+v"(kw));
                gt += ((kw & 0xffffu) > thr ? 1 : 0) + ((kw >> 16) > thr ? 1 : 0);
            }
        ties_to_take = k - block_count(gt);
    }
    int my_ties = 0;
    if (ties_to_take > 0) {
#pragma unroll
        for (int j = 0; j < NV; ++j)
#pragma unroll
            for (int h = 0; h < 2; ++h) {
                uint32_t kw = key[j][h];
                asm volatile("" : "+v"(kw));
                my_ties += ((kw & 0xffffu) == thr ? 1 : 0) + ((kw >> 16) == thr ? 1 : 0);
            }
    }
    int tie_budget = 0;
    {
        int incl = my_ties;
#pragma unroll
        for (int d = 1; d < 64; d <<= 1) {
            const int o = __shfl_up(incl, d);
            if (lane >= d) incl += o;
        }
        if (lane == 63) wave_cnt[w] = incl;
        __syncthreads();
        int before = incl - my_ties;
#pragma unroll
        for (int i = 0; i < 16; ++i) before += i < w ? wave_cnt[i] : 0;
        __syncthreads();
        tie_budget = ties_to_take - before;
    }
    uint8_t *out = p.mask + (int64_t)row * n;
    const uint8_t *st = p.stat ? p.stat + (int64_t)(row % p.stat_rows) * p.stat_stride : nullptr;
    const bool rnd = active && p.random_amount > 0.f;
    auto combined4 = [&](int c0, uint32_t &v0, uint32_t &v1) {
        const u32x2 v = *(const u32x2 *)(x + c0);
        v0 = v[0], v1 = v[1];
        if constexpr (PARTS) {
            float a0 = __uint_as_float(v0 << 16), a1 = __uint_as_float(v0 & 0xffff0000u);
            float a2 = __uint_as_float(v1 << 16), a3 = __uint_as_float(v1 & 0xffff0000u);
            if (prow == 2) {
                const u32x2 y = *(const u32x2 *)(x + row1 + c0);
                a0 += __uint_as_float(y[0] << 16), a1 += __uint_as_float(y[0] & 0xffff0000u);
                a2 += __uint_as_float(y[1] << 16), a3 += __uint_as_float(y[1] & 0xffff0000u);
            }
            v0 = pack_bf16x2(a0, a1), v1 = pack_bf16x2(a2, a3);
        }
    };
    uint32_t first = x[0];
    if constexpr (PARTS) {
        uint32_t f0, f1;
        combined4(0, f0, f1);
        first = f0 & 0xffffu;
    }
    const uint32_t salt = p.salt ^ (first * 0x27D4EB2Fu);
    const int nsteps = (n + 4095) / 4096;
    auto emit = [&](auto keyed, int c, uint32_t v0, uint32_t v1, uint32_t sb) {
        uint32_t bytes = 0;
        if constexpr (decltype(keyed)::value) asm volatile("" : "+v"(v0), "+v"(v1));
#pragma unroll
        for (int e = 0; e < 4; ++e) {
            const uint32_t half = ((e < 2 ? v0 : v1) >> (16 * (e & 1))) & 0xffffu;
            const uint32_t kv = decltype(keyed)::value ? half : bf16_key(half);
            bool keep = kv > thr;
            const bool tie = kv == thr && tie_budget > 0 && c + e < n;
            tie_budget -= tie ? 1 : 0;
            keep = keep || tie;
            if (rnd && !keep) keep = hash_uniform(row, c + e, salt) < p.random_amount;
            keep = keep || ((sb >> (8 * e)) & 0xffu) != 0;
            bytes |= (keep ? 1u : 0u) << (8 * e);
        }
        if constexpr (ALIGNED) {
            *(uint32_t *)(out + c) = bytes;
        } else {
#pragma unroll
            for (int e = 0; e < 4; ++e)
                if (c + e < n) out[c + e] = (uint8_t)(bytes >> (8 * e));
        }
    };
    if constexpr (ALIGNED) {
        constexpr int OB = 5;
#pragma unroll
        for (int j0 = 0; j0 < NV; j0 += OB) {
            uint32_t sbv[OB];
#pragma unroll
            for (int jj = 0; jj < OB; ++jj) {
                const int c = 4 * tid + 4096 * (j0 + jj);
                sbv[jj] = (j0 + jj < NV && st && c < n) ? *(const uint32_t *)(st + c) : 0u;
            }
            __builtin_amdgcn_sched_barrier(0);
#pragma unroll
            for (int jj = 0; jj < OB; ++jj) {
                if constexpr (true) {
                    const int c = 4 * tid + 4096 * (j0 + jj);
                    if (j0 + jj < NV && c < n) emit(std::integral_constant<int, 1>{}, c, key[(j0 + jj) < NV ? (j0 + jj) : 0][0], key[(j0 + jj) < NV ? (j0 + jj) : 0][1], sbv[jj]);
                    asm volatile("" ::: "memory");
                }
            }
            __builtin_amdgcn_sched_barrier(0);
        }
    } else {
        for (int j = 0; j < nsteps; ++j) {
            const int c = 4 * tid + 4096 * j;
            if (c >= n) break;
            uint32_t v0 = 0, v1 = 0, sb = 0;
#pragma unroll
            for (int e = 0; e < 4; ++e) {
                const uint32_t u = c + e < n ? x[c + e] : 0xffffu;
                if (e < 2) v0 |= u << (16 * e);
                else v1 |= u << (16 * (e - 2));
                if (st && c + e < n) sb |= (uint32_t)st[c + e] << (8 * e);
            }
            emit(std::integral_constant<int, 0>{}, c, v0, v1, sb);
        }
    }
}

}

extern "C" int chipmunk_mask_to_indices(const void *mask, int32_t *indices, int32_t *counts, int64_t rows, int n,
                                        int pad_n, int multiple_of, void *stream) {
    return launch_m2i<false>(mask, indices, counts, rows, n, pad_n, multiple_of, stream);
}

extern "C" int chipmunk_packed_mask_to_indices(const void *packed, int32_t *indices, int32_t *counts, int64_t rows,
                                               int n, int pad_n, int multiple_of, void *stream) {
    return launch_m2i<true>(packed, indices, counts, rows, n, pad_n, multiple_of, stream);
}

static int launch_topk(const void *activation, void *cache, int dtype, int32_t *indices, int32_t *counts, int rows,
                       int cols, double sparsity_amount, int multiple_of, double random_amount, void *stream) {
    CM_CHECK(activation && indices && counts, "topk_indices: null pointer");
    CM_CHECK(rows >= 0 && cols >= 1024, "topk_indices: rows >= 0 and cols >= 1024 required (the quantile is taken over the first 1024 columns); got rows=%d cols=%d", rows, cols);
    CM_CHECK(multiple_of > 0, "topk_indices: multiple_of must be positive");
    CM_CHECK(sparsity_amount >= 0.0 && sparsity_amount <= 1.0, "topk_indices: sparsity_amount must be in [0,1]");
    if (rows == 0) return CHIPMUNK_OK;
    TopkParams p = {activation, cache, indices, counts, rows, cols, multiple_of, (float)sparsity_amount, (float)random_amount,
                    random_amount > 0.0 ? chipmunk_next_random_salt() : 0u};
    hipStream_t s = (hipStream_t)stream;
#define LAUNCH_TOPK(T)                                                                                           \
    do {                                                                                                         \
        if (cache) hipLaunchKernelGGL((topk_indices_kernel<T, true>), dim3(rows), dim3(1024), 0, s, p);          \
        else hipLaunchKernelGGL((topk_indices_kernel<T, false>), dim3(rows), dim3(1024), 0, s, p);               \
    } while (0)
    switch (dtype) {
        case CHIPMUNK_DTYPE_BF16: LAUNCH_TOPK(uint16_t); break;
        case CHIPMUNK_DTYPE_FP16: LAUNCH_TOPK(_Float16); break;
        case CHIPMUNK_DTYPE_FP32: LAUNCH_TOPK(float); break;
        default: CM_CHECK(false, "topk_indices: unsupported dtype code %d", dtype);
    }
#undef LAUNCH_TOPK
    CM_LAUNCH_CHECK();
    return CHIPMUNK_OK;
}

extern "C" int chipmunk_mask_to_sorted_indices(const void *mask, int packed, int32_t *indices, int32_t *counts,
                                               int64_t rows, int n, int pad_n, int multiple_of, void *stream) {
    return packed ? launch_m2i<true, true>(mask, indices, counts, rows, n, pad_n, multiple_of, stream)
                  : launch_m2i<false, true>(mask, indices, counts, rows, n, pad_n, multiple_of, stream);
}

extern "C" int chipmunk_topk_indices(const void *activation, int dtype, int32_t *indices, int32_t *counts, int rows,
                                     int cols, double sparsity_amount, int multiple_of, double random_amount,
                                     void *stream) {
    return launch_topk(activation, nullptr, dtype, indices, counts, rows, cols, sparsity_amount, multiple_of,
                       random_amount, stream);
}

extern "C" int chipmunk_topk_delta_indices(const void *activation, void *cache, int dtype, int32_t *indices,
                                           int32_t *counts, int rows, int cols, double sparsity_amount,
                                           int multiple_of, double random_amount, void *stream) {
    CM_CHECK(cache != nullptr, "topk_delta_indices: cache missing");
    return launch_topk(activation, cache, dtype, indices, counts, rows, cols, sparsity_amount, multiple_of,
                       random_amount, stream);
}

extern "C" int chipmunk_copy_indices(const void *src, void *dst, const int32_t *inds, const int32_t *counts, int B,
                                     int M, int R, int F, int elem_size, void *stream) {
    CM_CHECK(src && dst && inds && counts, "copy_indices: null pointer");
    CM_CHECK(B >= 0 && M > 0 && R > 0 && F > 0, "copy_indices: bad sizes");
    CM_CHECK(elem_size == 2 || elem_size == 4, "copy_indices: element size must be 2 or 4 bytes (got %d)", elem_size);
    const int64_t rows = (int64_t)B * M * R;
    if (rows == 0) return CHIPMUNK_OK;
    CM_CHECK(rows < (1ll << 31), "copy_indices: too many rows");
    hipStream_t s = (hipStream_t)stream;
    if (elem_size == 2)
        hipLaunchKernelGGL(copy_indices_kernel<uint16_t>, dim3((unsigned)rows), dim3(256), 0, s, (const uint16_t *)src,
                           (uint16_t *)dst, inds, counts, M, R, F);
    else
        hipLaunchKernelGGL(copy_indices_kernel<uint32_t>, dim3((unsigned)rows), dim3(256), 0, s, (const uint32_t *)src,
                           (uint32_t *)dst, inds, counts, M, R, F);
    CM_LAUNCH_CHECK();
    return CHIPMUNK_OK;
}

extern "C" int chipmunk_bitpack(const void *mask, void *packed, int64_t n, void *stream) {
    CM_CHECK(mask && packed && n >= 0, "bitpack: bad arguments");
    if (n == 0) return CHIPMUNK_OK;
    const int64_t nb = (n + 7) >> 3;
    const unsigned grid = (unsigned)((nb + 255) / 256 < 8192 ? (nb + 255) / 256 : 8192);
    hipLaunchKernelGGL(bitpack_kernel, dim3(grid), dim3(256), 0, (hipStream_t)stream, (const uint8_t *)mask,
                       (uint8_t *)packed, n);
    CM_LAUNCH_CHECK();
    return CHIPMUNK_OK;
}

extern "C" int chipmunk_bitunpack(const void *packed, void *mask, int64_t n, void *stream) {
    CM_CHECK(mask && packed && n >= 0, "bitunpack: bad arguments");
    if (n == 0) return CHIPMUNK_OK;
    const int64_t nb = (n + 7) >> 3;
    const unsigned grid = (unsigned)((nb + 255) / 256 < 8192 ? (nb + 255) / 256 : 8192);
    hipLaunchKernelGGL(bitunpack_kernel, dim3(grid), dim3(256), 0, (hipStream_t)stream, (const uint8_t *)packed,
                       (uint8_t *)mask, n);
    CM_LAUNCH_CHECK();
    return CHIPMUNK_OK;
}

extern "C" int chipmunk_transpose16(const void *src, void *dst, int B, int R, int C, void *stream) {
    CM_CHECK(src && dst && B > 0 && R > 0 && C > 0, "transpose16: bad arguments");
    CM_CHECK((C & 7) == 0 || true, "unreachable");
    hipLaunchKernelGGL(transpose16_kernel, dim3((C + 63) / 64, (R + 63) / 64, B), dim3(256), 0, (hipStream_t)stream,
                       (const uint16_t *)src, (uint16_t *)dst, R, C, R);
    CM_LAUNCH_CHECK();
    return CHIPMUNK_OK;
}

extern "C" int chipmunk_transpose16_pitched(const void *src, void *dst, int B, int R, int C, int ld, void *stream) {
    CM_CHECK(src && dst && B > 0 && R > 0 && C > 0, "transpose16: bad arguments");
    CM_CHECK(ld >= R, "transpose16: the output pitch ld (%d) must be at least R (%d)", ld, R);
    hipLaunchKernelGGL(transpose16_kernel, dim3((C + 63) / 64, (ld + 63) / 64, B), dim3(256), 0, (hipStream_t)stream,
                       (const uint16_t *)src, (uint16_t *)dst, R, C, ld);
    CM_LAUNCH_CHECK();
    return CHIPMUNK_OK;
}

template <typename V>
__global__ __launch_bounds__(256) void gather_rows_kernel(const V *src, V *dst, const int32_t *map, int64_t n_out,
                                                          int64_t n_src, int64_t cpr, int64_t total) {
    for (int64_t idx = (int64_t)blockIdx.x * 256 + threadIdx.x; idx < total; idx += (int64_t)gridDim.x * 256) {
        const int64_t row = idx / cpr, c = idx - row * cpr;
        const int64_t o = row / n_out, r = row - o * n_out;
        dst[idx] = src[(o * n_src + map[r]) * cpr + c];
    }
}

extern "C" int chipmunk_gather_rows(const void *src, void *dst, const int32_t *map, int64_t outer, int64_t n_src,
                                    int64_t n_out, int64_t row_bytes, void *stream) {
    CM_CHECK(src && dst && map, "gather_rows: null pointer");
    CM_CHECK(outer >= 0 && n_src > 0 && n_out >= 0 && row_bytes > 0, "gather_rows: bad sizes");
    if (outer == 0 || n_out == 0) return CHIPMUNK_OK;
    hipStream_t s = (hipStream_t)stream;
    const uintptr_t align = (uintptr_t)src | (uintptr_t)dst | (uintptr_t)row_bytes;
#define LAUNCH_GATHER(V)                                                                                              \
    do {                                                                                                              \
        const int64_t cpr = row_bytes / (int64_t)sizeof(V), total = outer * n_out * cpr;                               \
        const int64_t blocks = (total + 255) / 256;                                                                    \
        hipLaunchKernelGGL((gather_rows_kernel<V>), dim3((unsigned)(blocks > 65536 * 16 ? 65536 * 16 : blocks)),       \
                           dim3(256), 0, s, (const V *)src, (V *)dst, map, n_out, n_src, cpr, total);                  \
    } while (0)
    if ((align & 15) == 0) LAUNCH_GATHER(u32x4);
    else if ((align & 3) == 0) LAUNCH_GATHER(uint32_t);
    else if ((align & 1) == 0) LAUNCH_GATHER(uint16_t);
    else LAUNCH_GATHER(uint8_t);
#undef LAUNCH_GATHER
    CM_LAUNCH_CHECK();
    return CHIPMUNK_OK;
}

int chipmunk_topk_mask_parts(const uint16_t *part, int part_stride, int nrb, int groups_per_bh, int Nq, const void *static_mask, int64_t static_stride,
                             int static_rows, const void *group_flags, void *mask, int rows, int n, int k, double random_amount,
                             hipStream_t s) {
    CM_CHECK(part && mask && rows >= 0 && n > 0 && (n & 3) == 0 && n <= 1024 * 120 && k >= 0 && part_stride >= n && (part_stride & 3) == 0, "topk_mask_parts: bad arguments");
    CM_CHECK(!static_mask || (static_rows > 0 && static_stride >= n && (static_stride & 3) == 0 && ((uintptr_t)static_mask & 3) == 0),
             "topk_mask_parts: bad static mask geometry");
    CM_CHECK(((uintptr_t)mask & 3) == 0 && ((uintptr_t)part & 7) == 0, "topk_mask_parts: unaligned buffers");
    if (rows == 0) return CHIPMUNK_OK;
    TopkMaskParams p = {nullptr, (const uint8_t *)static_mask, (const uint8_t *)group_flags, (uint8_t *)mask, 0, static_stride,
                        rows, n, k, static_mask ? static_rows : 1, (float)random_amount,
                        random_amount > 0.0 ? chipmunk_next_random_salt() : 0u};
    p.parts = part, p.pstride = part_stride, p.nrb = nrb, p.ngroups = groups_per_bh, p.nq = Nq;
    if (n <= 1024 * 16) hipLaunchKernelGGL((topk_mask_kernel<16, true, true>), dim3(rows), dim3(1024), 0, s, p);
    else if (n <= 1024 * 48) hipLaunchKernelGGL((topk_mask_kernel<48, true, true>), dim3(rows), dim3(1024), 0, s, p);
    else hipLaunchKernelGGL((topk_mask_kernel<120, true, true>), dim3(rows), dim3(1024), 0, s, p);
    CM_LAUNCH_CHECK();
    return CHIPMUNK_OK;
}

__global__ __launch_bounds__(256) void qkv_split_norm_kernel(const uint16_t *qkv, int64_t row_stride, const uint16_t *qw,
                                                             const uint16_t *kw, uint16_t *q, uint16_t *k, uint16_t *v, int64_t n,
                                                             int H, float eps, int64_t segments, const float *fcos, const float *fsin,
                                                             int64_t rope_rows) {
    const int l15 = threadIdx.x & 15;
    u32x4 wq = {0x3f803f80u, 0x3f803f80u, 0x3f803f80u, 0x3f803f80u}, wk = wq;
    if (qw) wq = *(const u32x4 *)(qw + l15 * 8);
    if (kw) wk = *(const u32x4 *)(kw + l15 * 8);
    for (int64_t seg = ((int64_t)blockIdx.x * 256 + threadIdx.x) >> 4; seg < segments; seg += ((int64_t)gridDim.x * 256) >> 4) {
        const int64_t tok = seg / (3 * H);
        const int rem = (int)(seg - tok * 3 * H), which = rem / H, h = rem - which * H;
        u32x4 x = *(const u32x4 *)(qkv + tok * row_stride + (int64_t)rem * 128 + l15 * 8);
        uint16_t *dst = (which == 0 ? q : which == 1 ? k : v) + ((int64_t)h * n + tok) * 128 + l15 * 8;
        if (which < 2) {
            float f[8], ss = 0.f;
#pragma unroll
            for (int e = 0; e < 4; ++e) {
                f[2 * e] = __uint_as_float(x[e] << 16), f[2 * e + 1] = __uint_as_float(x[e] & 0xffff0000u);
                ss = __builtin_fmaf(f[2 * e], f[2 * e], ss);
                ss = __builtin_fmaf(f[2 * e + 1], f[2 * e + 1], ss);
            }
            ss = row16_sum(ss);
            const float r = 1.0f / __builtin_sqrtf(ss * (1.0f / 128.0f) + eps);
            const u32x4 w = which == 0 ? wq : wk;
#pragma unroll
            for (int e = 0; e < 4; ++e) {
                float a = f[2 * e] * r, b = f[2 * e + 1] * r;
                round_bf16_pair(a, b);
                x[e] = pack_bf16x2(a * __uint_as_float(w[e] << 16), b * __uint_as_float(w[e] & 0xffff0000u));
            }
            if (fcos && tok < rope_rows) {
                const f32x4 c0 = *(const f32x4 *)(fcos + tok * 128 + l15 * 8), c1 = *(const f32x4 *)(fcos + tok * 128 + l15 * 8 + 4);
                const f32x4 s0 = *(const f32x4 *)(fsin + tok * 128 + l15 * 8), s1 = *(const f32x4 *)(fsin + tok * 128 + l15 * 8 + 4);
#pragma unroll
                for (int e = 0; e < 4; ++e) {
                    const float re = __uint_as_float(x[e] << 16), im = __uint_as_float(x[e] & 0xffff0000u);
                    const float cr = e < 2 ? c0[2 * e] : c1[2 * e - 4], ci = e < 2 ? c0[2 * e + 1] : c1[2 * e - 3];
                    const float sr = e < 2 ? s0[2 * e] : s1[2 * e - 4], si = e < 2 ? s0[2 * e + 1] : s1[2 * e - 3];
                    x[e] = pack_bf16x2(re * cr + (-im) * sr, im * ci + re * si);
                }
            }
        }
        *(u32x4 *)dst = x;
    }
}

extern "C" int chipmunk_qkv_split_norm(const void *qkv, int64_t row_stride, const void *q_weight, const void *k_weight, void *q,
                                       void *k, void *v, int64_t n, int heads, float eps, const float *freqs_cos,
                                       const float *freqs_sin, int64_t rope_rows, void *stream) {
    CM_CHECK(qkv && q && k && v, "qkv_split_norm: null pointer");
    CM_CHECK(n >= 0 && heads > 0 && row_stride >= (int64_t)3 * heads * 128, "qkv_split_norm: bad sizes");
    CM_CHECK((((uintptr_t)qkv | (uintptr_t)q | (uintptr_t)k | (uintptr_t)v | (uintptr_t)q_weight | (uintptr_t)k_weight) & 15) == 0 &&
                 (row_stride & 7) == 0 && (((uintptr_t)freqs_cos | (uintptr_t)freqs_sin) & 15) == 0,
             "qkv_split_norm: pointers and the row stride must be 16-byte aligned");
    CM_CHECK((freqs_cos == nullptr) == (freqs_sin == nullptr) && rope_rows >= 0 && rope_rows <= n, "qkv_split_norm: bad rotary arguments");
    if (n == 0) return CHIPMUNK_OK;
    const int64_t segments = n * 3 * heads, blocks = (segments + 15) / 16;
    hipLaunchKernelGGL(qkv_split_norm_kernel, dim3((unsigned)(blocks > 256 * 64 ? 256 * 64 : blocks)), dim3(256), 0, (hipStream_t)stream,
                       (const uint16_t *)qkv, row_stride, (const uint16_t *)q_weight, (const uint16_t *)k_weight, (uint16_t *)q,
                       (uint16_t *)k, (uint16_t *)v, n, heads, eps, segments, freqs_cos, freqs_sin, freqs_cos ? rope_rows : 0);
    CM_LAUNCH_CHECK();
    return CHIPMUNK_OK;
}

extern "C" int chipmunk_topk_mask(const void *cs, int64_t cs_stride, const void *static_mask, int64_t static_stride,
                                  int static_rows, const void *group_flags, void *mask, int rows, int n, int k,
                                  double random_amount, void *stream) {
    CM_CHECK(cs && mask, "topk_mask: null pointer");
    CM_CHECK(rows >= 0 && n > 0 && k >= 0, "topk_mask: bad sizes (rows=%d n=%d k=%d)", rows, n, k);
    CM_CHECK(cs_stride >= n, "topk_mask: cs row stride %lld < n %d", (long long)cs_stride, n);
    CM_CHECK(n <= 1024 * 120, "topk_mask: rows of more than 122880 columns are not supported (got %d)", n);
    CM_CHECK(!static_mask || (static_rows > 0 && static_stride >= n), "topk_mask: bad static mask geometry");
    CM_CHECK(random_amount >= 0.0 && random_amount <= 1.0, "topk_mask: random_amount must be in [0,1]");
    if (rows == 0) return CHIPMUNK_OK;
    TopkMaskParams p = {(const uint16_t *)cs, (const uint8_t *)static_mask, (const uint8_t *)group_flags, (uint8_t *)mask,
                        cs_stride, static_stride, rows, n, k, static_mask ? static_rows : 1, (float)random_amount,
                        random_amount > 0.0 ? chipmunk_next_random_salt() : 0u};
    hipStream_t s = (hipStream_t)stream;
    const bool aligned = n % 4 == 0 && (((uintptr_t)cs) & 7) == 0 && (cs_stride * 2) % 8 == 0 && (((uintptr_t)mask) & 3) == 0 &&
                         (!static_mask || ((((uintptr_t)static_mask) & 3) == 0 && static_stride % 4 == 0));
#define LAUNCH_TM(KPT)                                                                                       \
    do {                                                                                                     \
        if (aligned) hipLaunchKernelGGL((topk_mask_kernel<KPT, true>), dim3(rows), dim3(1024), 0, s, p);     \
        else hipLaunchKernelGGL((topk_mask_kernel<KPT, false>), dim3(rows), dim3(1024), 0, s, p);            \
    } while (0)
    if (n <= 1024 * 16) LAUNCH_TM(16);
    else if (n <= 1024 * 48) LAUNCH_TM(48);
    else LAUNCH_TM(120);
#undef LAUNCH_TM
    CM_LAUNCH_CHECK();
    return CHIPMUNK_OK;
}

extern "C" int chipmunk_compact_indices(const int32_t *indices, int64_t idx_stride, const int32_t *counts, const int64_t *offsets,
                                        int32_t *flat, int64_t rows, void *stream) {
    CM_CHECK(indices && counts && offsets && flat, "compact_indices: null pointer");
    CM_CHECK(rows >= 0 && rows < (1ll << 31) && idx_stride > 0, "compact_indices: bad sizes rows=%lld idx_stride=%lld", (long long)rows,
             (long long)idx_stride);
    if (rows == 0) return CHIPMUNK_OK;
    hipLaunchKernelGGL(compact_indices_kernel, dim3((unsigned)rows), dim3(256), 0, (hipStream_t)stream, indices, idx_stride, counts,
                       offsets, flat);
    CM_LAUNCH_CHECK();
    return CHIPMUNK_OK;
}
```

chipmunk_amd/csrc/torch_registry.cpp:

```cpp
#include <ATen/ATen.h>
#include <ATen/hip/impl/HIPStreamMasqueradingAsCUDA.h>
#include <Python.h>
#include <c10/core/DeviceGuard.h>
#include <torch/library.h>

#include <vector>

#include "../../include/chipmunk_hip.h"

extern "C" {
PyObject *PyInit_cuda(void) {
    static struct PyModuleDef module_def = {PyModuleDef_HEAD_INIT, "cuda", NULL, -1, NULL};
    return PyModule_Create(&module_def);
}
}

namespace chipmunk {
namespace {

void *cur_stream(const at::Tensor &t) {
    return (void *)c10::hip::getCurrentHIPStreamMasqueradingAsCUDA(t.device().index()).stream();
}
void check(int rc, const char *op) { TORCH_CHECK(rc == 0, "chipmunk::", op, ": ", chipmunk_last_error()); }

// ... 423 lines not shown
    int dtype;
    switch (activation.scalar_type()) {
        case at::kBFloat16: dtype = CHIPMUNK_DTYPE_BF16; break;
        case at::kHalf: dtype = CHIPMUNK_DTYPE_FP16; break;
        case at::kFloat: dtype = CHIPMUNK_DTYPE_FP32; break;
        default: TORCH_CHECK(false, "Unsupported dtype for topk_indices");
    }
    c10::DeviceGuard guard(activation.device());
    check(chipmunk_topk_indices(activation.data_ptr(), dtype, indices.data_ptr<int>(), counts.data_ptr<int>(),
                                (int)(activation.size(0) * activation.size(1)), (int)activation.size(2),
                                sparsity_amount, (int)multiple_of, random_amount, cur_stream(activation)),
          "topk_indices");
}

void topk_delta_indices(at::Tensor activation, at::Tensor cache, at::Tensor indices, at::Tensor counts,
                        double sparsity_amount, int64_t multiple_of, double random_amount) {
    CHECK_DEV(activation); CHECK_DEV(cache); CHECK_DEV(indices); CHECK_DEV(counts);
    CHECK_CONTIG(activation); CHECK_CONTIG(cache); CHECK_CONTIG(indices); CHECK_CONTIG(counts);
    TORCH_CHECK(activation.dim() == 3 && cache.sizes() == activation.sizes(), "activation and cache must be [batch, rows, cols]");
    TORCH_CHECK(cache.scalar_type() == activation.scalar_type(), "activation and cache must have the same dtype");
    CHECK_I32(indices); CHECK_I32(counts);
    TORCH_CHECK(indices.sizes() == activation.sizes(), "indices must have the shape of activation");
    TORCH_CHECK(counts.numel() == activation.size(0) * activation.size(1), "counts must be [batch, rows]");
    int dtype;
    switch (activation.scalar_type()) {
        case at::kBFloat16: dtype = CHIPMUNK_DTYPE_BF16; break;
        case at::kHalf: dtype = CHIPMUNK_DTYPE_FP16; break;
        case at::kFloat: dtype = CHIPMUNK_DTYPE_FP32; break;
        default: TORCH_CHECK(false, "Unsupported dtype for topk_delta_indices");
    }
    c10::DeviceGuard guard(activation.device());
    check(chipmunk_topk_delta_indices(activation.data_ptr(), cache.data_ptr(), dtype, indices.data_ptr<int>(),
                                      counts.data_ptr<int>(), (int)(activation.size(0) * activation.size(1)),
                                      (int)activation.size(2), sparsity_amount, (int)multiple_of, random_amount,
                                      cur_stream(activation)),
          "topk_delta_indices");
}

std::vector<at::Tensor> mask_to_indices(at::Tensor mask, int64_t multiple_of, int64_t pad_to_multiple_of) {
    TORCH_CHECK(mask.dim() == 4, "mask must be 4-dimensional [b, h, m, n]");
    TORCH_CHECK(mask.scalar_type() == at::kBool, "mask must be bool type");
    CHECK_DEV(mask);
    TORCH_CHECK(multiple_of > 0 && pad_to_multiple_of > 0, "multiple_of and pad_to_multiple_of must be positive");
    mask = mask.contiguous();
    const int64_t b = mask.size(0), h = mask.size(1), m = mask.size(2), n = mask.size(3);
    const int64_t pad_n = ((n + pad_to_multiple_of - 1) / pad_to_multiple_of) * pad_to_multiple_of;
    c10::DeviceGuard guard(mask.device());
    at::Tensor indices = at::empty({b, h, m, pad_n}, mask.options().dtype(at::kInt));
    at::Tensor counts = at::empty({b, h, m}, mask.options().dtype(at::kInt));
    check(chipmunk_mask_to_indices(mask.data_ptr(), indices.data_ptr<int>(), counts.data_ptr<int>(), b * h * m, (int)n,
                                   (int)pad_n, (int)multiple_of, cur_stream(mask)),
          "mask_to_indices");
    return {indices, counts};
}

std::vector<at::Tensor> packed_mask_to_indices(at::Tensor packed, at::IntArrayRef shape, int64_t multiple_of,
                                               int64_t pad_to_multiple_of) {
    TORCH_CHECK(packed.scalar_type() == at::kByte && packed.is_contiguous(), "packed must be a contiguous uint8 tensor");
    CHECK_DEV(packed);
    TORCH_CHECK(shape.size() == 4, "shape must be [b, h, m, n]");
    const int64_t b = shape[0], h = shape[1], m = shape[2], n = shape[3];
    TORCH_CHECK(n % 8 == 0, "n must be a multiple of 8");
    TORCH_CHECK(packed.numel() * 8 >= b * h * m * n, "packed is too short for the given shape");
    const int64_t pad_n = ((n + pad_to_multiple_of - 1) / pad_to_multiple_of) * pad_to_multiple_of;
    c10::DeviceGuard guard(packed.device());
    at::Tensor indices = at::empty({b, h, m, pad_n}, packed.options().dtype(at::kInt));
    at::Tensor counts = at::empty({b, h, m}, packed.options().dtype(at::kInt));
    check(chipmunk_packed_mask_to_indices(packed.data_ptr(), indices.data_ptr<int>(), counts.data_ptr<int>(),
                                          b * h * m, (int)n, (int)pad_n, (int)multiple_of, cur_stream(packed)),
          "packed_mask_to_indices");
    return {indices, counts};
}

at::Tensor transpose_last2(at::Tensor x) {
    CHECK_DEV(x);
    TORCH_CHECK(x.dim() >= 2 && x.element_size() == 2, "transpose_last2: need a >=2-D tensor of a 16-bit dtype");
    x = x.contiguous();
    const int64_t R = x.size(-2), C = x.size(-1), B = x.numel() / (R * C);
    auto sizes = x.sizes().vec();
    std::swap(sizes[sizes.size() - 1], sizes[sizes.size() - 2]);
    c10::DeviceGuard guard(x.device());
    at::Tensor out = at::empty(sizes, x.options());
    check(chipmunk_transpose16(x.data_ptr(), out.data_ptr(), (int)B, (int)R, (int)C, cur_stream(x)), "transpose_last2");
    return out;
}

at::Tensor transpose_last2_pitched(at::Tensor x, int64_t ld) {
    CHECK_DEV(x);
    TORCH_CHECK(x.dim() >= 2 && x.element_size() == 2, "transpose_last2_pitched: need a >=2-D tensor of a 16-bit dtype");
    x = x.contiguous();
    const int64_t R = x.size(-2), C = x.size(-1), B = x.numel() / (R * C);
    TORCH_CHECK(ld >= R, "transpose_last2_pitched: ld must be at least the row count");
    auto sizes = x.sizes().vec();
    sizes[sizes.size() - 2] = C;
    sizes[sizes.size() - 1] = ld;
    c10::DeviceGuard guard(x.device());
    at::Tensor out = at::empty(sizes, x.options());
    check(chipmunk_transpose16_pitched(x.data_ptr(), out.data_ptr(), (int)B, (int)R, (int)C, (int)ld, cur_stream(x)), "transpose_last2_pitched");
    return out;
}

at::Tensor block_mean(at::Tensor x, int64_t mbm) {
    CHECK_DEV(x);
    TORCH_CHECK(x.dim() == 3 && x.scalar_type() == at::kBFloat16, "block_mean: need a [b, n, c] bfloat16 tensor");
    TORCH_CHECK(mbm > 0 && x.size(1) > 0, "block_mean: mbm and n must be positive");
    x = x.contiguous();
    c10::DeviceGuard guard(x.device());
    const int64_t n = x.size(1), blocks = (n + mbm - 1) / mbm;
    at::Tensor out = at::empty({x.size(0), blocks, x.size(2)}, x.options());
    if (n % mbm == 0) {
        check(chipmunk_block_mean(x.data_ptr(), out.data_ptr(), x.size(0) * n, (int)x.size(2), (int)mbm, cur_stream(x)), "block_mean");
    } else {
        for (int64_t b = 0; b < x.size(0); ++b)
            check(chipmunk_block_mean_ragged(x[b].data_ptr(), out[b].data_ptr(), n, (int)x.size(2), (int)mbm, cur_stream(x)), "block_mean");
    }
    return out;
}

at::Tensor quantize_fp8(at::Tensor x, at::Tensor scale, double max_value) {
    CHECK_DEV(x); CHECK_DEV(scale);
    TORCH_CHECK(x.scalar_type() == at::kBFloat16, "quantize_fp8: x must be bfloat16");
    TORCH_CHECK(scale.scalar_type() == at::kFloat && scale.numel() == 1, "quantize_fp8: scale must be a one-element float32 tensor");
    TORCH_CHECK(x.numel() % 8 == 0, "quantize_fp8: the element count must be a multiple of 8");
    x = x.contiguous();
    c10::DeviceGuard guard(x.device());
    at::Tensor out = at::empty(x.sizes(), x.options().dtype(at::kFloat8_e4m3fn));
    check(chipmunk_quantize_fp8(x.data_ptr(), scale.data_ptr<float>(), out.data_ptr(), x.numel(), (float)max_value, cur_stream(x)), "quantize_fp8");
    return out;
}

std::vector<at::Tensor> mask_to_sorted_indices(at::Tensor mask, at::IntArrayRef shape, int64_t multiple_of,
                                               int64_t pad_to_multiple_of) {
    CHECK_DEV(mask);
    const bool packed = mask.scalar_type() == at::kByte;
    TORCH_CHECK(packed || mask.scalar_type() == at::kBool, "mask must be bool, or uint8 bit-packed with a shape");
    mask = mask.contiguous();
    std::vector<int64_t> shp = packed ? shape.vec() : mask.sizes().vec();
    TORCH_CHECK(shp.size() == 4, "shape must be [b, h, m, n]");
    const int64_t b = shp[0], h = shp[1], m = shp[2], n = shp[3];
    if (packed) TORCH_CHECK(n % 8 == 0 && mask.numel() * 8 >= b * h * m * n, "bad packed mask");
    const int64_t pad_n = ((n + pad_to_multiple_of - 1) / pad_to_multiple_of) * pad_to_multiple_of;
    c10::DeviceGuard guard(mask.device());
    at::Tensor indices = at::empty({b, h, m, pad_n}, mask.options().dtype(at::kInt));
    at::Tensor counts = at::empty({b, h, m}, mask.options().dtype(at::kInt));
    check(chipmunk_mask_to_sorted_indices(mask.data_ptr(), packed ? 1 : 0, indices.data_ptr<int>(),
                                          counts.data_ptr<int>(), b * h * m, (int)n, (int)pad_n, (int)multiple_of,
                                          cur_stream(mask)),
          "mask_to_sorted_indices");
    return {indices, counts};
}

std::vector<at::Tensor> dense_colsum_attn_layout(at::Tensor q, at::Tensor k, at::Tensor v, at::Tensor p, bool token_major_o);
at::Tensor topk_mask(at::Tensor cs, int64_t k, double random_amount, const c10::optional<at::Tensor> &groups,
                     const c10::optional<at::Tensor> &static_mask);
std::vector<at::Tensor> dense_colsum_topk_mask(at::Tensor q, at::Tensor k, at::Tensor v, at::Tensor p, int64_t k_top, double random_amount,
                                               const c10::optional<at::Tensor> &groups, const c10::optional<at::Tensor> &static_mask,
                                               bool token_major_o) {
    CHECK_DEV(q); CHECK_DEV(k); CHECK_DEV(v); CHECK_DEV(p);
    CHECK_BF16(q); CHECK_BF16(k); CHECK_BF16(v);
    const bool shapes_ok = q.dim() == 4 && k.dim() == 4 && v.dim() == 4 && q.size(3) == 128 && q.stride(3) == 1 && k.stride(3) == 1 &&
                           v.stride(3) == 1 && p.scalar_type() == at::kFloat && p.is_contiguous();
    if (shapes_ok) {
        const int64_t B = q.size(0), H = q.size(1), Nq = q.size(2), Nk = k.size(2), G = (Nq + 191) / 192;
        const void *st = nullptr, *gf = nullptr;
        int64_t st_stride = 0, st_rows = 1;
        at::Tensor stc, gfc;
        bool ok = p.numel() == B * H * Nq;
        if (ok && static_mask.has_value() && static_mask->defined()) {
            stc = *static_mask;
            ok = stc.is_cuda() && stc.scalar_type() == at::kBool && stc.dim() == 4 && stc.size(3) == Nk && stc.size(2) == G && stc.size(1) == H &&
                 (stc.size(0) == 1 || stc.size(0) == B) && stc.stride(3) == 1 && stc.stride(1) == G * stc.stride(2) &&
                 (stc.size(0) == 1 || stc.stride(0) == H * stc.stride(1));
            if (ok) st = stc.data_ptr(), st_stride = stc.stride(2), st_rows = stc.size(0) * H * G;
        }
        if (ok && groups.has_value() && groups->defined()) {
            gfc = *groups;
            ok = gfc.is_cuda() && gfc.scalar_type() == at::kBool && gfc.dim() == 4 && gfc.size(3) == 1 && gfc.size(2) == G && gfc.size(1) == H &&
                 (gfc.size(0) == 1 || gfc.size(0) == B);
            if (ok) {
                gfc = gfc.expand({B, H, G, 1}).contiguous();
                gf = gfc.data_ptr();
            }
        }
        if (ok) {
            c10::DeviceGuard guard(q.device());
            at::Tensor o = alloc_o(q, q, token_major_o);
            const int64_t os[3] = {o.stride(0), o.stride(1), o.stride(2)};
            at::Tensor l = at::empty({B, H, Nq, 1}, q.options().dtype(at::kFloat));
            at::Tensor mask = at::empty({B, H, G, Nk}, q.options().dtype(at::kBool));
            const int64_t qs[3] = {q.stride(0), q.stride(1), q.stride(2)}, ks[3] = {k.stride(0), k.stride(1), k.stride(2)},
                          vs[3] = {v.stride(0), v.stride(1), v.stride(2)};
            const int rc = chipmunk_dense_colsum_topk_mask_strided(q.data_ptr(), k.data_ptr(), v.data_ptr(), qs, ks, vs, p.data_ptr<float>(), o.data_ptr(),
                                                           os, l.data_ptr<float>(), (int)B, (int)H, (int)Nq, (int)Nk, st, st_stride, (int)st_rows, gf,
                                                           mask.data_ptr(), (int)k_top, random_amount, cur_stream(q));
            if (rc == CHIPMUNK_OK) return {o, mask, l};
            if (rc != CHIPMUNK_ERR_UNSUPPORTED) check(rc, "dense_colsum_topk_mask");
        }
    }
    auto ocl = dense_colsum_attn_layout(q, k, v, p, token_major_o);
    at::Tensor cs = ocl[1];
    const int64_t Nk = k.size(2), G = (q.size(2) + 191) / 192;
    if (cs.size(-1) != Nk || cs.size(-2) != G) cs = cs.slice(-2, 0, G).slice(-1, 0, Nk);
    return {ocl[0], topk_mask(cs, k_top, random_amount, groups, static_mask), ocl[2]};
}

at::Tensor topk_mask(at::Tensor cs, int64_t k, double random_amount, const c10::optional<at::Tensor> &groups,
                     const c10::optional<at::Tensor> &static_mask) {
    CHECK_DEV(cs); CHECK_BF16(cs);
    TORCH_CHECK(cs.dim() == 4 && cs.stride(3) == 1, "cs must be [B, H, G, N] with a contiguous last dim");
    const int64_t B = cs.size(0), H = cs.size(1), G = cs.size(2), N = cs.size(3);
    if (!(cs.stride(1) == G * cs.stride(2) && (B == 1 || cs.stride(0) == H * cs.stride(1)))) cs = cs.contiguous();
    const int64_t rows = B * H * G;
    c10::DeviceGuard guard(cs.device());
    at::Tensor mask = at::empty({B, H, G, N}, cs.options().dtype(at::kBool));
    const void *st = nullptr, *gf = nullptr;
    int64_t st_stride = 0, st_rows = 1;
    at::Tensor stc, gfc;
    if (static_mask.has_value() && static_mask->defined()) {
        stc = *static_mask;
        CHECK_DEV(stc);
        TORCH_CHECK(stc.scalar_type() == at::kBool && stc.dim() == 4 && stc.size(3) == N && stc.size(2) == G &&
                    stc.size(1) == H && (stc.size(0) == 1 || stc.size(0) == B), "static_mask must be bool [1|B, H, G, N]");
        if (!(stc.stride(3) == 1 && stc.stride(1) == G * stc.stride(2) && (stc.size(0) == 1 || stc.stride(0) == H * stc.stride(1))))
            stc = stc.contiguous();
        st = stc.data_ptr(), st_stride = stc.stride(2), st_rows = stc.size(0) * H * G;
    }
    if (groups.has_value() && groups->defined()) {
        gfc = *groups;
        CHECK_DEV(gfc);
        TORCH_CHECK(gfc.scalar_type() == at::kBool && gfc.dim() == 4 && gfc.size(3) == 1 && gfc.size(2) == G &&
                    gfc.size(1) == H && (gfc.size(0) == 1 || gfc.size(0) == B), "groups must be bool [1|B, H, G, 1]");
        gfc = gfc.expand({B, H, G, 1}).contiguous();
        gf = gfc.data_ptr();
    }
    check(chipmunk_topk_mask(cs.data_ptr(), cs.stride(2), st, st_stride, (int)st_rows, gf, mask.data_ptr(), (int)rows, (int)N,
                             (int)k, random_amount, cur_stream(cs)),
          "topk_mask");
    return mask;
}

at::Tensor bitpack(at::Tensor mask) {
    TORCH_CHECK(mask.scalar_type() == at::kBool, "mask must be bool type");
    CHECK_DEV(mask);
    mask = mask.contiguous();
    c10::DeviceGuard guard(mask.device());
    at::Tensor packed = at::empty({(mask.numel() + 7) / 8}, mask.options().dtype(at::kByte));
    check(chipmunk_bitpack(mask.data_ptr(), packed.data_ptr(), mask.numel(), cur_stream(mask)), "bitpack");
    return packed;
}
at::Tensor bitunpack(at::Tensor packed, at::IntArrayRef shape) {
    TORCH_CHECK(packed.scalar_type() == at::kByte && packed.is_contiguous(), "packed must be a contiguous uint8 tensor");
    CHECK_DEV(packed);
    int64_t n = 1;
    for (auto d : shape) n *= d;
    TORCH_CHECK(packed.numel() * 8 >= n, "packed is too short for the given shape");
    c10::DeviceGuard guard(packed.device());
    at::Tensor mask = at::empty(shape, packed.options().dtype(at::kBool));
    check(chipmunk_bitunpack(packed.data_ptr(), mask.data_ptr(), n, cur_stream(packed)), "bitunpack");
    return mask;
}

std::vector<at::Tensor> qkv_split_norm(at::Tensor qkv, const c10::optional<at::Tensor> &q_weight, const c10::optional<at::Tensor> &k_weight,
                                       int64_t heads, double eps, const c10::optional<at::Tensor> &freqs_cos,
                                       const c10::optional<at::Tensor> &freqs_sin) {
    CHECK_DEV(qkv); CHECK_BF16(qkv);
    TORCH_CHECK(qkv.dim() == 2 && qkv.stride(1) == 1 && qkv.size(1) >= 3 * heads * 128, "qkv_split_norm: qkv must be [n, >= 3*heads*128] with a contiguous last dim");
    const void *qw = nullptr, *kw = nullptr;
    at::Tensor qwc, kwc;
    if (q_weight.has_value() && q_weight->defined()) { qwc = q_weight->contiguous(); CHECK_DEV(qwc); CHECK_BF16(qwc); TORCH_CHECK(qwc.numel() == 128); qw = qwc.data_ptr(); }
    if (k_weight.has_value() && k_weight->defined()) { kwc = k_weight->contiguous(); CHECK_DEV(kwc); CHECK_BF16(kwc); TORCH_CHECK(kwc.numel() == 128); kw = kwc.data_ptr(); }
    const int64_t n = qkv.size(0);
    const float *fc = nullptr, *fs = nullptr;
    int64_t rope_rows = 0;
    at::Tensor fcc, fsc;
    if (freqs_cos.has_value() && freqs_cos->defined()) {
        TORCH_CHECK(freqs_sin.has_value() && freqs_sin->defined(), "qkv_split_norm: freqs_cos without freqs_sin");
        fcc = freqs_cos->contiguous(), fsc = freqs_sin->contiguous();
        CHECK_DEV(fcc); CHECK_DEV(fsc);
        TORCH_CHECK(fcc.scalar_type() == at::kFloat && fsc.scalar_type() == at::kFloat && fcc.dim() == 2 && fcc.size(1) == 128 &&
                    fsc.sizes() == fcc.sizes() && fcc.size(0) <= n, "qkv_split_norm: freqs must be float32 [rows <= n, 128]");
        fc = fcc.data_ptr<float>(), fs = fsc.data_ptr<float>(), rope_rows = fcc.size(0);
    }
    c10::DeviceGuard guard(qkv.device());
    at::Tensor out = at::empty({3, 1, heads, n, 128}, qkv.options());
    check(chipmunk_qkv_split_norm(qkv.data_ptr(), qkv.stride(0), qw, kw, out[0].data_ptr(), out[1].data_ptr(), out[2].data_ptr(), n,
                                  (int)heads, (float)eps, fc, fs, rope_rows, cur_stream(qkv)),
          "qkv_split_norm");
    return {out[0], out[1], out[2]};
}

at::Tensor gather_rows(at::Tensor src, at::Tensor map) {
    CHECK_DEV(src);
    CHECK_DEV(map);
    TORCH_CHECK(src.dim() >= 2, "gather_rows: src must be [..., n, d]");
    TORCH_CHECK(map.scalar_type() == at::kInt && map.dim() == 1 && map.is_contiguous(), "gather_rows: map must be a contiguous int32 vector");
    src = src.contiguous();
    const int64_t n_src = src.size(-2), d = src.size(-1), n_out = map.numel();
    const int64_t outer = n_src * d == 0 ? 0 : src.numel() / (n_src * d);
    auto sizes = src.sizes().vec();
    sizes[sizes.size() - 2] = n_out;
    c10::DeviceGuard guard(src.device());
    at::Tensor dst = at::empty(sizes, src.options());
    if (dst.numel() == 0) return dst;
    check(chipmunk_gather_rows(src.data_ptr(), dst.data_ptr(), map.data_ptr<int>(), outer, n_src, n_out,
                               d * (int64_t)src.element_size(), cur_stream(src)),
          "gather_rows");
    return dst;
}

}

TORCH_LIBRARY(chipmunk, m) {
    m.def("csp_mlp_mm1(Tensor a, Tensor b_colmajor, Tensor(c!) c, Tensor bias, Tensor pa_cache_colmajor, Tensor indices, Tensor indices_counts) -> ()");
    m.def("csp_mlp_mm2_and_scatter_add(Tensor packed, Tensor(unpacked_colmajor!) unpacked_colmajor, Tensor sp_inds, Tensor sp_counts, Tensor mma_a, Tensor mma_b, Tensor mma_c, int num_sms_scatter_add, int matmul_kernel) -> ()");

    m.def("csp_attn(Tensor q, Tensor k, Tensor v, Tensor o, Tensor indices, Tensor indices_counts, int o_scale) -> ()");
    m.def("csp_128_attn(Tensor q, Tensor k, Tensor v, Tensor indices, Tensor indices_counts) -> Tensor");
    m.def("dense_attn(Tensor q, Tensor k, Tensor v) -> Tensor[]");
    m.def("dense_colsum_attn(Tensor q, Tensor k, Tensor v, Tensor p) -> Tensor[]");

    m.def("copy_indices(Tensor bmfc1, Tensor(bm_mid_cache!) bm_mid_cache, Tensor sp_inds, Tensor sp_counts) -> ()");
    m.def("topk_indices(Tensor activation, Tensor(indices!) indices, Tensor counts, float sparsity_amount, int multiple_of, float random_amount) -> ()");
    m.def("csp_scatter_add(Tensor packed, Tensor(unpacked_colmajor!) unpacked_colmajor, Tensor sp_inds, Tensor sp_counts, int num_sms) -> ()");
    m.def("mask_to_indices(Tensor mask, int multiple_of, int pad_to_multiple_of) -> Tensor[]");

    m.def("csp_attn_out(Tensor q, Tensor k, Tensor v, Tensor o_in, Tensor indices, Tensor indices_counts, int o_scale) -> Tensor");
    m.def("csp_mlp_mm1_scatter(Tensor a, Tensor b_colmajor, Tensor(c!) c, Tensor bias, Tensor(pa_cache_colmajor!) pa_cache_colmajor, Tensor indices, Tensor indices_counts) -> ()");
    m.def("csp_mlp_mm2(Tensor mma_a, Tensor mma_b, Tensor indices, Tensor counts, Tensor(mma_c!) mma_c) -> ()");
    m.def("csp_mlp_mm1_fp8(Tensor a, Tensor b, Tensor(c!) c, Tensor bias, Tensor(pa_cache_colmajor!) pa_cache_colmajor, Tensor indices, Tensor indices_counts, Tensor scale_a, Tensor scale_b, bool update_cache) -> ()");
    m.def("csp_mlp_mm1_fp8_scatter(Tensor a, Tensor b, Tensor(c!) c, Tensor bias, Tensor(pa_cache_colmajor!) pa_cache_colmajor, Tensor indices, Tensor indices_counts, Tensor scale_a, Tensor scale_b) -> ()");
    m.def("topk_delta_indices(Tensor activation, Tensor(cache!) cache, Tensor(indices!) indices, Tensor(counts!) counts, float sparsity_amount, int multiple_of, float random_amount) -> ()");
    m.def("packed_mask_to_indices(Tensor packed, int[] shape, int multiple_of, int pad_to_multiple_of) -> Tensor[]");
    m.def("mask_to_sorted_indices(Tensor mask, int[] shape, int multiple_of, int pad_to_multiple_of) -> Tensor[]");
    m.def("topk_mask(Tensor cs, int k, float random_amount, Tensor? groups, Tensor? static_mask) -> Tensor");
    m.def("dense_colsum_topk_mask(Tensor q, Tensor k, Tensor v, Tensor p, int k_top, float random_amount, Tensor? groups, Tensor? static_mask, bool token_major_o=False) -> Tensor[]");
    m.def("dense_attn_layout(Tensor q, Tensor k, Tensor v, bool token_major_o) -> Tensor[]");
    m.def("dense_colsum_attn_layout(Tensor q, Tensor k, Tensor v, Tensor p, bool token_major_o) -> Tensor[]");
    m.def("compact_indices(Tensor indices, Tensor counts) -> Tensor[]");
    m.def("csp_attn_out_ragged(Tensor q, Tensor k, Tensor v, Tensor o_in, Tensor indices, Tensor offsets, Tensor indices_counts, int o_scale) -> Tensor");
    m.def("residual_ln_modulate(Tensor x, Tensor? y, Tensor? gate, Tensor shift, Tensor scale, float eps) -> Tensor[]");
    m.def("transpose_last2(Tensor x) -> Tensor");
    m.def("transpose_last2_pitched(Tensor x, int ld) -> Tensor");
    m.def("block_mean(Tensor x, int mbm) -> Tensor");
    m.def("quantize_fp8(Tensor x, Tensor scale, float max_value) -> Tensor");
    m.def("bitpack(Tensor mask) -> Tensor");
    m.def("bitunpack(Tensor packed, int[] shape) -> Tensor");
    m.def("gather_rows(Tensor src, Tensor map) -> Tensor");
    m.def("qkv_split_norm(Tensor qkv, Tensor? q_weight, Tensor? k_weight, int heads, float eps, Tensor? freqs_cos=None, Tensor? freqs_sin=None) -> Tensor[]");
}

TORCH_LIBRARY_IMPL(chipmunk, CUDA, m) {
    m.impl("qkv_split_norm", &qkv_split_norm);
    m.impl("csp_mlp_mm1_fp8_scatter", &csp_mlp_mm1_fp8_scatter);
    m.impl("dense_colsum_topk_mask", &dense_colsum_topk_mask);
    m.impl("csp_mlp_mm1", &csp_mlp_mm1);
    m.impl("csp_mlp_mm2_and_scatter_add", &csp_mlp_mm2_and_scatter_add);
    m.impl("copy_indices", &copy_indices);
    m.impl("topk_indices", &topk_indices);
    m.impl("csp_scatter_add", &csp_scatter_add);
    m.impl("mask_to_indices", &mask_to_indices);
    m.impl("csp_attn", &csp_attn);
    m.impl("csp_128_attn", &csp_128_attn);
    m.impl("dense_attn", &dense_attn);
    m.impl("dense_colsum_attn", &dense_colsum_attn);
    m.impl("compact_indices", &compact_indices);
    m.impl("residual_ln_modulate", &residual_ln_modulate);
    m.impl("csp_attn_out_ragged", &csp_attn_out_ragged);
    m.impl("dense_attn_layout", &dense_attn_layout);
    m.impl("dense_colsum_attn_layout", &dense_colsum_attn_layout);
    m.impl("csp_attn_out", &csp_attn_out);
    m.impl("csp_mlp_mm1_scatter", &csp_mlp_mm1_scatter);
    m.impl("csp_mlp_mm2", &csp_mlp_mm2);
    m.impl("csp_mlp_mm1_fp8", &csp_mlp_mm1_fp8);
    m.impl("topk_delta_indices", &topk_delta_indices);
    m.impl("packed_mask_to_indices", &packed_mask_to_indices);
    m.impl("mask_to_sorted_indices", &mask_to_sorted_indices);
    m.impl("topk_mask", &topk_mask);
    m.impl("transpose_last2", &transpose_last2);
    m.impl("transpose_last2_pitched", &transpose_last2_pitched);
    m.impl("block_mean", &block_mean);
    m.impl("quantize_fp8", &quantize_fp8);
    m.impl("bitpack", &bitpack);
    m.impl("bitunpack", &bitunpack);
    m.impl("gather_rows", &gather_rows);
}

}
```

chipmunk_amd/modules/attn.py:

```python
from __future__ import annotations

from typing import Optional, Tuple

import torch
import torch.nn.functional as F
from torch import Tensor, nn

from .. import ops
from ..ops.voxel import get_local_indices_with_text
from ..util.config import GLOBAL_CONFIG, amd_key
from ..util.layer_counter import LayerCounter
from ..util.storage import AttnStorage
from ..util.storage.offloaded_tensor import release_kept_offloaded, release_resident, reserve_kept_offloaded, reserve_resident

singleton_static_mask: Optional[Tensor] = None
singleton_video_query_groups: Optional[Tensor] = None


def _cdiv(a: int, b: int) -> int:
    return (a + b - 1) // b


def _dense_attn_raw(q: Tensor, k: Tensor, v: Tensor, token_major_o: bool):
    return torch.ops.chipmunk.dense_attn_layout(q, k, v, True) if token_major_o else torch.ops.chipmunk.dense_attn(q, k, v)


class SparseDiffAttn(nn.Module):
    def __init__(self, layer_num: int, layer_counter: LayerCounter, storage_slot: int = 0, query_group_offset: int = 0):
        super().__init__()
        self.layer_num = layer_num
        self.layer_counter = layer_counter
        self.query_group_offset = query_group_offset
        self.storage = AttnStorage(layer_num, init_names=["indices", "out_cache"], slot=storage_slot)
        self.mask_shape = [None] * GLOBAL_CONFIG["num_model_invocations_per_inference_step"]
        self._unpacked = [None] * GLOBAL_CONFIG["num_model_invocations_per_inference_step"]

    def initialize_static_mask(self, seq_shape: Tuple, txt_len: int, local_heads_num: int, device: torch.device):
        if len(seq_shape) == 2:
            raise NotImplementedError("Not yet implemented for 2D sequences")
        tt, th, tw = seq_shape
        cfg = GLOBAL_CONFIG["attn"]
        n_video = tt * th * tw
        topk = int(cfg["top_keys"] * n_video)
        lv = cfg["local_voxels"]
        mask, _, _ = get_local_indices_with_text(vid_shape=(tt, th, tw), txt_len=txt_len, voxel_shape=(4, 6, 8),
                                                 local_shape=(lv, lv, lv), rk=cfg["random_keys"], device=device)
        if cfg["local_1d_window"] > 0:
            window = int(cfg["local_1d_window"] * n_video)
            for qg in range(n_video // 192):
                centre = qg * 192 + 96
                mask[qg, max(0, centre - window // 2):min(n_video, centre + window // 2)] = True
        mask = mask[None, None, :, :].expand(1, local_heads_num, -1, -1).contiguous()
        sparse_groups = (mask.sum(dim=-1, keepdim=True) + topk) < (n_video + txt_len)
        global singleton_static_mask, singleton_video_query_groups
        singleton_static_mask = mask
        singleton_video_query_groups = sparse_groups

    def _static(self, heads: int, qg: int, n: int):
        g0 = self.query_group_offset
        assert heads <= singleton_static_mask.shape[1] or singleton_static_mask.shape[1] == 1, (
            f"this module serves {heads} heads but initialize_static_mask() built {singleton_static_mask.shape[1]} head planes "
            "(local_heads_num): build the static mask for the largest head chunk")
        h = min(heads, singleton_static_mask.shape[1])
        return (singleton_static_mask[:, :h, g0:g0 + qg, :n], singleton_video_query_groups[:, :h, g0:g0 + qg, :])

    def random_and_topk(self, cs: Tensor, topk: int) -> Tensor:
        cfg = GLOBAL_CONFIG["attn"]
        qg, n = cs.shape[-2], cs.shape[-1]
        static, groups = self._static(cs.shape[1], qg, n)
        if cs.is_cuda and amd_key("attn", "fused_topk_mask") and cs.dtype == torch.bfloat16 and n <= 122880:
            return ops.topk_mask(cs, topk, 0.01, groups, static)
        mask = torch.randint(0, 100, cs.shape, device=cs.device, dtype=torch.uint8) == 0
        mask.scatter_(-1, cs.topk(k=topk, dim=-1).indices, True)
        mask.logical_and_(groups)
        mask.logical_or_(static)
        return mask

    def release_kept_indices(self) -> None:
        for inv, old in enumerate(self._unpacked):
            if old is not None:
                self._release_kept(old)
                self._unpacked[inv] = None

    @staticmethod
    def _release_kept(kept) -> None:
        release_resident(kept[3])
        if kept[4]:
            release_kept_offloaded(kept[3])

    def __del__(self):
        try:
            self.release_kept_indices()
        except Exception:
            pass

    @torch.compiler.disable
    def _remember_indices(self, inds: Tensor, counts: Tensor) -> None:
        inv = self.layer_counter.cur_model_invocation_per_step
        old, self._unpacked[inv] = self._unpacked[inv], None
        if old is not None:
            self._release_kept(old)
        self.storage.indices.suppress_current(False)
        if not (inds.is_cuda and amd_key("attn", "keep_unpacked_indices") and amd_key("attn", "fused_residual")
                and (self.storage.indices.is_resident() or amd_key("attn", "keep_unpacked_indices_offloaded"))):
            return
        if not reserve_resident(0):
            return
        flat, offsets = ops.compact_indices(inds, counts)
        nbytes = 4 * flat.numel() + 8 * offsets.numel() + 4 * counts.numel()
        off_mode = not self.storage.indices.is_resident()
        if off_mode and not reserve_kept_offloaded(nbytes):
            return
        if not reserve_resident(nbytes):
            if off_mode:
                release_kept_offloaded(nbytes)
            return
        self._unpacked[inv] = (flat, offsets, counts, nbytes, off_mode)
        self.storage.indices.suppress_current(off_mode and bool(GLOBAL_CONFIG["attn"]["recompute_mask"]))

    def _kept_indices(self):
        kept = self._unpacked[self.layer_counter.cur_model_invocation_per_step]
        if kept is not None and GLOBAL_CONFIG["attn"]["should_compress_indices"] and (
                self.storage.indices.is_resident() or amd_key("attn", "keep_unpacked_indices_offloaded")):
            return kept[:3]
        return None

    def _stored_indices(self, multiple_of: int, bm: int):
        cfg = GLOBAL_CONFIG["attn"]
        if cfg["should_compress_indices"]:
            if self.storage.indices.is_suppressed():
                self.storage.indices.suppress_current(False)
                self.storage.indices.load_async()
                self.storage.indices.load_async_wait()
            packed = self.storage.get_indices()
            shape = self.mask_shape[self.layer_counter.cur_model_invocation_per_step]
            if amd_key("attn", "fused_packed_mask_to_indices") and packed.is_cuda and shape[-1] % 8 == 0:
                if amd_key("attn", "sorted_indices"):
                    return ops.mask_to_sorted_indices(packed, shape, multiple_of, bm)
                return ops.packed_mask_to_indices(packed, shape, multiple_of, bm)
            return ops.mask_to_indices(ops.bitunpack(packed, shape), multiple_of, bm)
        return self.storage.get_indices(), self.storage.get_counts()

    def _fast_attention(self, q: Tensor, k: Tensor, v: Tensor, inference_step: int, do_full_step: bool) -> Tensor:
        cfg = GLOBAL_CONFIG["attn"]
        bm = cfg["mbm"]
        assert bm == 192, "The kernel was written for BM=192. You may need to change the kernel."
        do_padding = cfg["pad_qkv_before_kernel"]
        multiple_of = 128 if do_padding else cfg["counts_multiple_of"]

        tm = bool(q.is_cuda and amd_key("attn", "token_major_output"))
        if self.layer_num < cfg["first_n_dense_layers"]:
            o, _ = ops.dense_attn(q, k, v, tm)
            return o

        if do_full_step:
            if inference_step == 0:
                o, lse = ops.dense_attn(q, k, v, tm) if do_padding else _dense_attn_raw(q, k, v, tm)
                lse[..., k.shape[-2]:, :] = 0
                self.storage.set_lse_constants(lse)
                return o

            if inference_step == 1 or cfg["recompute_mask"]:
                prev_lse = self.storage.get_lse_constants()
                tk = int(multiple_of * round((cfg["top_keys"] * k.shape[-2]) / multiple_of))
                mask = bs = None
                if (q.is_cuda and cfg["should_compress_indices"] and tk > 0 and amd_key("attn", "fused_colsum_topk")
                        and amd_key("attn", "fused_topk_mask") and k.shape[-2] <= 122880):
                    static, groups = self._static(q.shape[1], _cdiv(q.shape[-2], bm), k.shape[-2])
                    o, mask, lse = ops.dense_colsum_topk_mask(q, k, v, prev_lse, tk, 0.01, groups, static, tm)
                elif do_padding:
                    o, bs, lse = ops.dense_colsum_attn(q, k, v, prev_lse, tm)
                else:
                    o, bs, lse = (torch.ops.chipmunk.dense_colsum_attn_layout(q, k, v, prev_lse, True) if tm else
                                  torch.ops.chipmunk.dense_colsum_attn(q, k, v, prev_lse))
                lse[..., k.shape[-2]:, :] = 0
                self.storage.set_lse_constants(lse)
                if cfg["should_compress_indices"]:
                    if mask is not None:
                        pass
                    elif tk > 0:
                        mask = self.random_and_topk(bs, tk)
                    else:
                        mask = self._static(bs.shape[1], bs.shape[-2], bs.shape[-1])[0]
                    packed, mask_shape = ops.bitpack(mask)
                    self.mask_shape[self.layer_counter.cur_model_invocation_per_step] = mask_shape
                    self.storage.set_indices(packed)
                    if mask.is_cuda and amd_key("attn", "fused_packed_mask_to_indices") and amd_key("attn", "sorted_indices"):
                        inds, counts = ops.mask_to_sorted_indices(mask, mask.shape, multiple_of, bm)
                    else:
                        inds, counts = ops.mask_to_indices(mask, multiple_of, bm)
                    self._remember_indices(inds, counts)
                else:
                    kseq = k.shape[-2]
                    bs = bs[..., :_cdiv(kseq, bm), :kseq]
                    inds = torch.topk(bs, k=tk, dim=-1).indices
                    counts = torch.full((q.shape[0], q.shape[1], _cdiv(q.shape[-2], bm)), tk, device=q.device,
                                        dtype=torch.int32)
                    pad = torch.empty((*counts.shape, q.shape[-2] - tk), device=q.device, dtype=torch.int32)
                    inds = torch.cat([inds, pad], dim=-1).to(torch.int32)
                    self.storage.set_indices(inds)
                    self.storage.set_counts(counts)
            else:
                o, _ = ops.dense_attn(q, k, v, tm)

            if not cfg["recompute_mask"]:
                inds, counts = self._stored_indices(multiple_of, bm)

            if o.is_cuda and amd_key("attn", "fused_residual"):
                o_cache = ops.csp_attn_out(q, k, v, o, inds, counts, -1)
            elif do_padding:
                o_cache = o - ops.csp_attn(q, k, v, inds, counts)
            else:
                o_cache = o.clone()
                ops.csp_attn_inplace(q, k, v, o_cache, inds, counts, -1)
            self.storage.set_out_cache(o_cache)
            return o

        o = self.storage.get_out_cache()
        kept = self._kept_indices() if (o.is_cuda and amd_key("attn", "fused_residual")) else None
        if kept is not None:
            return ops.csp_attn_out_ragged(q, k, v, o, kept[0], kept[1], kept[2], 1)
        inds, counts = self._stored_indices(multiple_of, bm)
        if do_padding:
            if o.is_cuda and amd_key("attn", "fused_residual"):
                return ops.csp_attn_out(q, k, v, o, inds, counts, 1)
            return o + ops.csp_attn(q, k, v, inds, counts)
        persistent = self.storage.out_cache.is_resident()
        if o.is_cuda and amd_key("attn", "fused_residual") and persistent:
            return ops.csp_attn_out(q, k, v, o, inds, counts, 1)
        if persistent:
            o = o.clone()
        ops.csp_attn_inplace(q, k, v, o, inds, counts, 1)
        return o

    def forward(self, q: Tensor, k: Tensor, v: Tensor) -> Tensor:
        if not GLOBAL_CONFIG["attn"]["is_enabled"]:
            return F.scaled_dot_product_attention(q, k, v)
        do_full_step = self.layer_counter.should_do_full_attn_step()
        out = self._fast_attention(q, k, v, self.layer_counter.cur_inference_step, do_full_step)
        self.layer_counter.increment()
        return out

    def __call__(self, *args, **kwargs):
        return self.forward(*args, **kwargs)
```

chipmunk_amd/ops/_fake.py:

```python
import torch


def _o_like(q, token_major):
    B, H, N, D = q.shape
    return q.new_empty((B, N, H, D)).permute(0, 2, 1, 3) if token_major else q.new_empty((B, H, N, D))


def _register():
    lib = torch.library

    @lib.register_fake("chipmunk::csp_128_attn")
    def _(q, k, v, indices, indices_counts):
        return torch.empty_like(q)

    @lib.register_fake("chipmunk::csp_attn_out")
    def _(q, k, v, o_in, indices, indices_counts, o_scale):
        return torch.empty_like(o_in)

    @lib.register_fake("chipmunk::residual_ln_modulate")
    def _(x, y, gate, shift, scale, eps):
        return [torch.empty_like(x), torch.empty_like(x)] if y is not None else [torch.empty_like(x)]

    @lib.register_fake("chipmunk::csp_attn_out_ragged")
    def _(q, k, v, o_in, indices, offsets, indices_counts, o_scale):
        return torch.empty_like(o_in)

    @lib.register_fake("chipmunk::dense_attn")
    def _(q, k, v):
        return [_o_like(q, False), q.new_empty((q.shape[0], q.shape[1], q.shape[2], 1), dtype=torch.float32)]

    @lib.register_fake("chipmunk::dense_attn_layout")
    def _(q, k, v, token_major_o):
        return [_o_like(q, token_major_o), q.new_empty((q.shape[0], q.shape[1], q.shape[2], 1), dtype=torch.float32)]

    @lib.register_fake("chipmunk::dense_colsum_attn_layout")
    def _(q, k, v, p, token_major_o):
        groups = (q.shape[2] + 191) // 192
        return [_o_like(q, token_major_o),
                q.new_empty((q.shape[0], q.shape[1], groups, max(q.shape[2], k.shape[2]))),
                q.new_empty((q.shape[0], q.shape[1], q.shape[2], 1), dtype=torch.float32)]

    @lib.register_fake("chipmunk::dense_colsum_attn")
    def _(q, k, v, p):
        groups = (q.shape[2] + 191) // 192
        return [_o_like(q, False),
                q.new_empty((q.shape[0], q.shape[1], groups, max(q.shape[2], k.shape[2]))),
                q.new_empty((q.shape[0], q.shape[1], q.shape[2], 1), dtype=torch.float32)]

    @lib.register_fake("chipmunk::mask_to_indices")
    def _(mask, multiple_of, pad_to_multiple_of):
        b, h, m, n = mask.shape
        pad_n = (n + pad_to_multiple_of - 1) // pad_to_multiple_of * pad_to_multiple_of
        return [mask.new_empty((b, h, m, pad_n), dtype=torch.int32), mask.new_empty((b, h, m), dtype=torch.int32)]

    @lib.register_fake("chipmunk::packed_mask_to_indices")
    def _(packed, shape, multiple_of, pad_to_multiple_of):
        b, h, m, n = shape
        pad_n = (n + pad_to_multiple_of - 1) // pad_to_multiple_of * pad_to_multiple_of
        return [packed.new_empty((b, h, m, pad_n), dtype=torch.int32), packed.new_empty((b, h, m), dtype=torch.int32)]

    @lib.register_fake("chipmunk::topk_mask")
    def _(cs, k, random_amount, groups, static_mask):
        return cs.new_empty(cs.shape, dtype=torch.bool)

    @lib.register_fake("chipmunk::block_mean")
    def _(x, mbm):
        return x.new_empty((x.shape[0], (x.shape[1] + mbm - 1) // mbm, x.shape[2]))

    @lib.register_fake("chipmunk::transpose_last2")
    def _(x):
        return x.new_empty(x.shape[:-2] + (x.shape[-1], x.shape[-2]))

    @lib.register_fake("chipmunk::transpose_last2_pitched")
    def _(x, ld):
        return x.new_empty(x.shape[:-2] + (x.shape[-1], ld))

    @lib.register_fake("chipmunk::quantize_fp8")
    def _(x, scale, max_value):
        return x.new_empty(x.shape, dtype=torch.float8_e4m3fn)

    @lib.register_fake("chipmunk::bitpack")
    def _(mask):
        return mask.new_empty(((mask.numel() + 7) // 8,), dtype=torch.uint8)

    @lib.register_fake("chipmunk::bitunpack")
    def _(packed, shape):
        return packed.new_empty(tuple(shape), dtype=torch.bool)

    @lib.register_fake("chipmunk::gather_rows")
    def _(src, map):
        shape = list(src.shape)
        shape[-2] = map.shape[0]
        return src.new_empty(shape)

    @lib.register_fake("chipmunk::dense_colsum_topk_mask")
    def _(q, k, v, p, k_top, random_amount, groups, static_mask, token_major_o=False):
        B, H, Nq, D = q.shape
        G = (Nq + 191) // 192
        return [_o_like(q, token_major_o), q.new_empty((B, H, G, k.shape[2]), dtype=torch.bool),
                q.new_empty((B, H, Nq, 1), dtype=torch.float32)]

    @lib.register_fake("chipmunk::qkv_split_norm")
    def _(qkv, q_weight, k_weight, heads, eps, freqs_cos=None, freqs_sin=None):
        out = qkv.new_empty((3, 1, heads, qkv.shape[0], 128))
        return [out[0], out[1], out[2]]


_register()
```

chipmunk_amd/ops/attn.py:

```python
from __future__ import annotations

from typing import Tuple

import torch
import torch.nn.functional as F

PM = 192


def _pad_len(n: int) -> int:
    return ((n + PM - 1) // PM) * PM


def _last_dim_contiguous(t: torch.Tensor) -> torch.Tensor:
    return t if t.stride(-1) == 1 else t.contiguous()


def dense_attn(q: torch.Tensor, k: torch.Tensor, v: torch.Tensor, token_major_o: bool = False) -> Tuple[torch.Tensor, torch.Tensor]:
    n = q.shape[-2]
    q, k, v = _last_dim_contiguous(q), _last_dim_contiguous(k), _last_dim_contiguous(v)
    o, l = torch.ops.chipmunk.dense_attn_layout(q, k, v, True) if token_major_o else torch.ops.chipmunk.dense_attn(q, k, v)
    padded = _pad_len(n)
    if padded != n:
        l = F.pad(l, (0, 0, 0, padded - n))
    return o, l


def dense_colsum_attn(q: torch.Tensor, k: torch.Tensor, v: torch.Tensor, p: torch.Tensor, token_major_o: bool = False
                      ) -> Tuple[torch.Tensor, torch.Tensor, torch.Tensor]:
    n = q.shape[-2]
    padded = _pad_len(n)
    assert p.shape[-2] in (n, padded), "p must be the l vector of the previous full step"
    p_rows = p[..., :n, :].contiguous()
    q, k, v = _last_dim_contiguous(q), _last_dim_contiguous(k), _last_dim_contiguous(v)
    if token_major_o:
        o, cs, l = torch.ops.chipmunk.dense_colsum_attn_layout(q, k, v, p_rows, True)
    else:
        o, cs, l = torch.ops.chipmunk.dense_colsum_attn(q, k, v, p_rows)
    if padded != n:
        l = F.pad(l, (0, 0, 0, padded - n))
    kseq = k.shape[-2]
    kgroups = (kseq + PM - 1) // PM
    if cs.shape[-2] != kgroups or cs.shape[-1] != kseq:
        cs = cs[..., :kgroups, :kseq]
    return o, cs, l


def dense_colsum_topk_mask(q: torch.Tensor, k: torch.Tensor, v: torch.Tensor, p: torch.Tensor, k_top: int, random_amount: float,
                           groups, static_mask, token_major_o: bool = False) -> Tuple[torch.Tensor, torch.Tensor, torch.Tensor]:
    n = q.shape[-2]
    padded = _pad_len(n)
    assert p.shape[-2] in (n, padded), "p must be the l vector of the previous full step"
    o, mask, l = torch.ops.chipmunk.dense_colsum_topk_mask(_last_dim_contiguous(q), _last_dim_contiguous(k), _last_dim_contiguous(v),
                                                           p[..., :n, :].contiguous(), k_top, random_amount, groups, static_mask,
                                                           token_major_o)
    if padded != n:
        l = F.pad(l, (0, 0, 0, padded - n))
    return o, mask, l


def csp_attn(q: torch.Tensor, k: torch.Tensor, v: torch.Tensor, indices: torch.Tensor,
             indices_counts: torch.Tensor) -> torch.Tensor:
    return torch.ops.chipmunk.csp_128_attn(q.contiguous(), k.contiguous(), v.contiguous(), indices.contiguous(),
                                           indices_counts.contiguous())


def csp_attn_inplace(q: torch.Tensor, k: torch.Tensor, v: torch.Tensor, o: torch.Tensor, indices: torch.Tensor,
                     indices_counts: torch.Tensor, o_scale: int) -> None:
    torch.ops.chipmunk.csp_attn(q, k, v, o, indices, indices_counts, o_scale)


def csp_attn_out(q: torch.Tensor, k: torch.Tensor, v: torch.Tensor, o_in: torch.Tensor, indices: torch.Tensor,
                 indices_counts: torch.Tensor, o_scale: int) -> torch.Tensor:
    return torch.ops.chipmunk.csp_attn_out(q, k, v, o_in, indices, indices_counts, o_scale)


def compact_indices(indices: torch.Tensor, indices_counts: torch.Tensor) -> Tuple[torch.Tensor, torch.Tensor]:
    return tuple(torch.ops.chipmunk.compact_indices(indices.contiguous(), indices_counts.contiguous()))


def csp_attn_out_ragged(q: torch.Tensor, k: torch.Tensor, v: torch.Tensor, o_in: torch.Tensor, indices: torch.Tensor,
                        offsets: torch.Tensor, indices_counts: torch.Tensor, o_scale: int) -> torch.Tensor:
    return torch.ops.chipmunk.csp_attn_out_ragged(q, k, v, o_in, indices, offsets, indices_counts, o_scale)


__all__ = ["csp_attn", "csp_attn_inplace", "csp_attn_out", "csp_attn_out_ragged", "compact_indices", "dense_attn", "dense_colsum_attn",
           "dense_colsum_topk_mask"]
```

chipmunk_amd/ops/indexed_io.py:

```python
from __future__ import annotations

from typing import List, Optional, Sequence

import torch


def copy_indices(bm_fc1: torch.Tensor, bm_mid_cache: torch.Tensor, indices: torch.Tensor, counts: torch.Tensor) -> None:
    torch.ops.chipmunk.copy_indices(bm_fc1, bm_mid_cache, indices, counts)


def topk_indices(activations: torch.Tensor, indices_out: torch.Tensor, counts_out: torch.Tensor,
                 sparsity_amount: float, multiple_of: int, rk: float) -> None:
    torch.ops.chipmunk.topk_indices(activations, indices_out, counts_out, sparsity_amount, multiple_of, rk)


def scatter_add(packed: torch.Tensor, unpacked: torch.Tensor, indices: torch.Tensor, counts: torch.Tensor,
                num_sms: int) -> None:
    torch.ops.chipmunk.csp_scatter_add(packed.unsqueeze(0), unpacked.unsqueeze(0), indices.unsqueeze(0),
                                       counts.unsqueeze(0), num_sms)


def mask_to_indices(mask: torch.Tensor, multiple_of: int, pad_to_multiple_of: int) -> List[torch.Tensor]:
    return torch.ops.chipmunk.mask_to_indices(mask, multiple_of, pad_to_multiple_of)


def packed_mask_to_indices(packed: torch.Tensor, shape: Sequence[int], multiple_of: int,
                           pad_to_multiple_of: int) -> List[torch.Tensor]:
    return torch.ops.chipmunk.packed_mask_to_indices(packed, list(shape), multiple_of, pad_to_multiple_of)


def mask_to_sorted_indices(mask: torch.Tensor, shape: Sequence[int], multiple_of: int,
                           pad_to_multiple_of: int) -> List[torch.Tensor]:
    return torch.ops.chipmunk.mask_to_sorted_indices(mask, list(shape), multiple_of, pad_to_multiple_of)


def topk_mask(cs: torch.Tensor, k: int, random_amount: float = 0.0, groups: Optional[torch.Tensor] = None,
              static_mask: Optional[torch.Tensor] = None) -> torch.Tensor:
    return torch.ops.chipmunk.topk_mask(cs, k, random_amount, groups, static_mask)


def manual_seed(seed: int) -> None:
    from .._native import manual_seed as _seed
    _seed(seed)
```

chipmunk_amd/util/config.py:

```python
from __future__ import annotations

import copy
from typing import Any, Dict

import yaml

BASE_CONFIG: Dict[str, Any] = {
    "num_model_invocations_per_inference_step": 1,
    "should_profile": False,
    "generation_index": 0,
    "steps": 50,
    "world_size": 1,
    "mlp": {
        "is_enabled": True,
        "is_fp8": False,
        "top_keys": "dd",
        "random_keys": 0.05,
        "full_step_every": 10,
        "block_mask_cache": 2,
        "first_n_dense_layers": 2,
        "counts_multiple_of": 256,
        "bm": 128,
        "mbm": 128,
    },
    "patchify": {
        "is_enabled": True,
        "chunk_size_1": 8,
        "chunk_size_2": 4,
    },
    "attn": {
        "is_enabled": True,
        "top_keys": 0.05,
        "random_keys": 0.01,
        "local_voxels": 0,
        "local_1d_window": 0,
        "first_n_dense_layers": 2,
        "full_step_every": 10,
        "full_step_schedule": None,
        "recompute_mask": True,
        "should_compress_indices": True,
        "counts_multiple_of": 128,
        "pad_qkv_before_kernel": True,
        "mbm": 192,
    },
    "offloading": {
        "global_disable_offloading": False,
        "mlp.out_cache": False,
        "mlp.indices": False,
        "mlp.counts": False,
        "mlp.sparse_act_T": False,
        "mlp.blockmean_mid_cache": False,
        "attn.out_cache": True,
        "attn.indices": True,
        "attn.counts": False,
        "attn.lse_constants": False,
        "text_encoders": True,
    },
    "step_caching": {
        "is_enabled": True,
        "skip_step_schedule": {7, 11, 13, 14, 15, 17, 18, 19, 21, 22, 23, 25, 26, 27, 29, 31, 33, 34, 35, 37, 38, 39,
                               41, 42, 43},
    },
}

AMD_EXTRA_KEYS: Dict[str, Any] = {
    "offloading.keep_resident_if_fits": False,
    "offloading.hbm_budget_gb": 200.0,
    "offloading.native_host_pool": True,
    "attn.fused_packed_mask_to_indices": True,
    "attn.sorted_indices": True,
    "mlp.fused_topk_delta": True,
    "mlp.fused_block_mean": True,
    "mlp.fused_fp8_quantize": True,
    "attn.fused_residual": True,
    "attn.fused_topk_mask": True,
    "attn.fused_colsum_topk": True,
    "mlp.fused_scatter": True,
    "attn.token_major_output": False,
    "attn.keep_unpacked_indices": True,
    "attn.keep_unpacked_indices_offloaded": True,
    "attn.kept_indices_offloaded_budget_gb": 8.0,
}
BASE_CONFIG["offloading"]["keep_resident_if_fits"] = AMD_EXTRA_KEYS["offloading.keep_resident_if_fits"]
BASE_CONFIG["offloading"]["hbm_budget_gb"] = AMD_EXTRA_KEYS["offloading.hbm_budget_gb"]
BASE_CONFIG["offloading"]["native_host_pool"] = AMD_EXTRA_KEYS["offloading.native_host_pool"]
BASE_CONFIG["attn"]["fused_packed_mask_to_indices"] = AMD_EXTRA_KEYS["attn.fused_packed_mask_to_indices"]
BASE_CONFIG["attn"]["sorted_indices"] = AMD_EXTRA_KEYS["attn.sorted_indices"]
BASE_CONFIG["mlp"]["fused_topk_delta"] = AMD_EXTRA_KEYS["mlp.fused_topk_delta"]
BASE_CONFIG["attn"]["fused_residual"] = AMD_EXTRA_KEYS["attn.fused_residual"]
BASE_CONFIG["attn"]["fused_topk_mask"] = AMD_EXTRA_KEYS["attn.fused_topk_mask"]
BASE_CONFIG["attn"]["fused_colsum_topk"] = AMD_EXTRA_KEYS["attn.fused_colsum_topk"]
BASE_CONFIG["mlp"]["fused_scatter"] = AMD_EXTRA_KEYS["mlp.fused_scatter"]
BASE_CONFIG["attn"]["token_major_output"] = AMD_EXTRA_KEYS["attn.token_major_output"]
BASE_CONFIG["attn"]["keep_unpacked_indices"] = AMD_EXTRA_KEYS["attn.keep_unpacked_indices"]
BASE_CONFIG["attn"]["keep_unpacked_indices_offloaded"] = AMD_EXTRA_KEYS["attn.keep_unpacked_indices_offloaded"]
BASE_CONFIG["attn"]["kept_indices_offloaded_budget_gb"] = AMD_EXTRA_KEYS["attn.kept_indices_offloaded_budget_gb"]

GLOBAL_CONFIG: Dict[str, Any] = copy.deepcopy(BASE_CONFIG)


def amd_key(section: str, key: str) -> Any:
    return GLOBAL_CONFIG.get(section, {}).get(key, AMD_EXTRA_KEYS[f"{section}.{key}"])


def update_global_config(config: Dict[str, Any]) -> None:
    GLOBAL_CONFIG.update(config)


def _deep_update(dst: Dict[str, Any], src: Dict[str, Any]) -> None:
    for key, value in src.items():
        if isinstance(value, dict) and isinstance(dst.get(key), dict):
            _deep_update(dst[key], value)
        else:
            dst[key] = value


def load_from_file(config_file: str) -> None:
    with open(config_file, "r") as f:
        loaded = yaml.safe_load(f)
    if loaded:
        _deep_update(GLOBAL_CONFIG, loaded)
        print(f"CHIPMUNK: using config file {config_file}")


def reset_to_base() -> None:
    fresh = copy.deepcopy(BASE_CONFIG)
    GLOBAL_CONFIG.clear()
    GLOBAL_CONFIG.update(fresh)
```

include/chipmunk_hip.h:

```cpp
#ifndef CHIPMUNK_HIP_H
#define CHIPMUNK_HIP_H

#include <stdint.h>

#ifdef __cplusplus
extern "C" {
#endif

#define CHIPMUNK_OK 0
#define CHIPMUNK_ERR_INVALID 1
#define CHIPMUNK_ERR_LAUNCH 2
#define CHIPMUNK_ERR_UNSUPPORTED 3

#define CHIPMUNK_DTYPE_BF16 0
#define CHIPMUNK_DTYPE_FP16 1
#define CHIPMUNK_DTYPE_FP32 2

const char *chipmunk_last_error(void);
int chipmunk_abi_version(void);
int chipmunk_set_option(const char *name, int value);
int chipmunk_set_random_seed(uint64_t seed);

int chipmunk_csp_attn(const void *q, const void *k, const void *v, void *o, const int64_t q_strides[3],
                      const int64_t k_strides[3], const int64_t v_strides[3], const int64_t o_strides[3],
                      const int32_t *indices, const int32_t *counts, int B, int H, int Nq, int Nk, int idx_stride,
                      int o_scale, void *stream);

int chipmunk_csp_attn_out(const void *q, const void *k, const void *v, const void *o_in, void *o_out,
                          const int64_t q_strides[3], const int64_t k_strides[3], const int64_t v_strides[3],
                          const int64_t o_strides[3], const int32_t *indices, const int32_t *counts, int B, int H,
                          int Nq, int Nk, int idx_stride, int o_scale, void *stream);

int chipmunk_csp_attn_out_ragged(const void *q, const void *k, const void *v, const void *o_in, void *o_out,
                                 const int64_t q_strides[3], const int64_t k_strides[3], const int64_t v_strides[3],
                                 const int64_t o_strides[3], const int32_t *indices, const int64_t *idx_offsets,
                                 const int32_t *counts, int B, int H, int Nq, int Nk, int o_scale, void *stream);
int chipmunk_compact_indices(const int32_t *indices, int64_t idx_stride, const int32_t *counts, const int64_t *offsets,
                             int32_t *flat, int64_t rows, void *stream);

int chipmunk_csp_128_attn(const void *q, const void *k, const void *v, void *o, const int32_t *indices,
                          const int32_t *counts, int B, int H, int Nq, int Nk, int idx_stride, void *stream);

int chipmunk_dense_attn(const void *q, const void *k, const void *v, const int64_t q_strides[3],
                        const int64_t k_strides[3], const int64_t v_strides[3], void *o, float *l, int B, int H,
                        int Nq, int Nk, void *stream);

int chipmunk_dense_attn_strided(const void *q, const void *k, const void *v, const int64_t q_strides[3],
                                const int64_t k_strides[3], const int64_t v_strides[3], void *o, const int64_t *o_strides,
                                float *l, int B, int H, int Nq, int Nk, void *stream);
int chipmunk_dense_colsum_attn_strided(const void *q, const void *k, const void *v, const int64_t q_strides[3],
                                       const int64_t k_strides[3], const int64_t v_strides[3], const float *p, void *o,
                                       const int64_t *o_strides, void *cs, float *l, int B, int H, int Nq, int Nk,
                                       int cs_stride, void *stream);
int chipmunk_dense_colsum_topk_mask_strided(const void *q, const void *k, const void *v, const int64_t q_strides[3],
                                            const int64_t k_strides[3], const int64_t v_strides[3], const float *p, void *o,
                                            const int64_t *o_strides, float *l, int B, int H, int Nq, int Nk,
                                            const void *static_mask, int64_t static_stride, int static_rows,
                                            const void *group_flags, void *mask, int k_top, double random_amount, void *stream);

int chipmunk_dense_colsum_attn(const void *q, const void *k, const void *v, const int64_t q_strides[3],
                               const int64_t k_strides[3], const int64_t v_strides[3], const float *p, void *o,
                               void *cs, float *l, int B, int H, int Nq, int Nk, int cs_stride, void *stream);

int chipmunk_residual_ln_modulate(const void *x, const void *y, const void *gate, const void *shift, const void *scale,
                                  void *x_out, void *xm, int64_t rows, int cols, double eps, void *stream);

int chipmunk_csp_mlp_mm1(const void *a, const void *b, void *c, const void *bias, const void *pa_cache,
                         const int32_t *indices, const int32_t *counts, int M, int K, int F, void *stream);

int chipmunk_csp_mlp_mm1_scatter(const void *a, const void *b, void *c, const void *bias, void *pa_cache,
                                 const int32_t *indices, const int32_t *counts, int M, int K, int F, void *stream);

int chipmunk_csp_mlp_mm1_fp8(const void *a, const void *b, void *c, const void *bias, void *pa_cache,
                             const int32_t *indices, const int32_t *counts, const float *scale_a,
                             const float *scale_b, int M, int K, int F, int update_cache, void *stream);

int chipmunk_csp_mlp_mm2_and_scatter_add(const void *packed, void *unpacked_colmajor, const int32_t *indices,
                                         const int32_t *counts, const void *mma_a, const void *mma_b, void *mma_c,
                                         int M, int F, int N2, int num_sms_scatter_add, void *stream);

int chipmunk_csp_scatter_add(const void *packed, void *unpacked_colmajor, const int32_t *indices,
                             const int32_t *counts, int M, int F, int num_sms, void *stream);

int chipmunk_csp_mlp_mm2(const void *mma_a, const void *mma_b, void *mma_c, const int32_t *indices,
                         const int32_t *counts, int M, int F, int N2, void *stream);

int chipmunk_csp_mlp_mm1_ragged(const void *a, const void *b, void *c, const void *bias, const void *pa_cache,
                                const int32_t *indices, const int32_t *counts, int M, int K, int F, int ldc, void *stream);
int chipmunk_csp_mlp_mm1_scatter_ragged(const void *a, const void *b, void *c, const void *bias, void *pa_cache,
                                        const int32_t *indices, const int32_t *counts, int M, int K, int F, int ldc,
                                        void *stream);
int chipmunk_csp_mlp_mm1_fp8_ragged(const void *a, const void *b, void *c, const void *bias, void *pa_cache,
                                    const int32_t *indices, const int32_t *counts, const float *scale_a,
                                    const float *scale_b, int M, int K, int F, int ldc, int update_cache, void *stream);
int chipmunk_csp_mlp_mm2_ragged(const void *mma_a, const void *mma_b, void *mma_c, const int32_t *indices,
                                const int32_t *counts, int M, int F, int N2, void *stream);
int chipmunk_csp_mlp_mm2_and_scatter_add_ragged(const void *packed, void *unpacked_colmajor, const int32_t *indices,
                                                const int32_t *counts, const void *mma_a, const void *mma_b, void *mma_c,
                                                int M, int F, int N2, int ldc, void *stream);
int chipmunk_csp_scatter_add_ragged(const void *packed, void *unpacked_colmajor, const int32_t *indices,
                                    const int32_t *counts, int M, int F, int ldc, void *stream);

int chipmunk_topk_indices(const void *activation, int dtype, int32_t *indices, int32_t *counts, int rows, int cols,
                          double sparsity_amount, int multiple_of, double random_amount, void *stream);

int chipmunk_topk_delta_indices(const void *activation, void *cache, int dtype, int32_t *indices, int32_t *counts,
                                int rows, int cols, double sparsity_amount, int multiple_of, double random_amount,
                                void *stream);

int chipmunk_dense_colsum_topk_mask(const void *q, const void *k, const void *v, const int64_t q_strides[3],
                                    const int64_t k_strides[3], const int64_t v_strides[3], const float *p, void *o, float *l,
                                    int B, int H, int Nq, int Nk, const void *static_mask, int64_t static_stride, int static_rows,
                                    const void *group_flags, void *mask, int k_top, double random_amount, void *stream);

int chipmunk_topk_mask(const void *cs, int64_t cs_stride, const void *static_mask, int64_t static_stride,
                       int static_rows, const void *group_flags, void *mask, int rows, int n, int k,
                       double random_amount, void *stream);

int chipmunk_mask_to_indices(const void *mask, int32_t *indices, int32_t *counts, int64_t rows, int n, int pad_n,
                             int multiple_of, void *stream);

int chipmunk_packed_mask_to_indices(const void *packed, int32_t *indices, int32_t *counts, int64_t rows, int n,
                                    int pad_n, int multiple_of, void *stream);

int chipmunk_mask_to_sorted_indices(const void *mask, int packed, int32_t *indices, int32_t *counts, int64_t rows,
                                    int n, int pad_n, int multiple_of, void *stream);

int chipmunk_copy_indices(const void *src, void *dst, const int32_t *inds, const int32_t *counts, int B, int M, int R,
                          int F, int elem_size, void *stream);

int chipmunk_transpose16(const void *src, void *dst, int B, int R, int C, void *stream);
int chipmunk_transpose16_pitched(const void *src, void *dst, int B, int R, int C, int ld, void *stream);

int chipmunk_block_mean(const void *x, void *out, int64_t rows, int C, int mbm, void *stream);
int chipmunk_block_mean_ragged(const void *x, void *out, int64_t rows, int C, int mbm, void *stream);

int chipmunk_quantize_fp8(const void *x, const float *scale, void *out, int64_t n, float max_value, void *stream);

int chipmunk_bitpack(const void *mask, void *packed, int64_t n, void *stream);
int chipmunk_bitunpack(const void *packed, void *mask, int64_t n, void *stream);

int chipmunk_gather_rows(const void *src, void *dst, const int32_t *map, int64_t outer, int64_t n_src, int64_t n_out,
                         int64_t row_bytes, void *stream);

int chipmunk_host_alloc(size_t bytes, void **host_ptr);
int chipmunk_host_free(void *host_ptr);
int chipmunk_copy_d2h_async(void *host_dst, const void *dev_src, size_t bytes, void *stream);
int chipmunk_copy_h2d_async(void *dev_dst, const void *host_src, size_t bytes, void *stream);
size_t chipmunk_host_bytes(void);

int chipmunk_release_scratch(void);
int chipmunk_big_scratch_fallbacks(void);

int chipmunk_qkv_split_norm(const void *qkv, int64_t row_stride, const void *q_weight, const void *k_weight, void *q, void *k,
                            void *v, int64_t n, int heads, float eps, const float *freqs_cos, const float *freqs_sin,
                            int64_t rope_rows, void *stream);

#ifdef __cplusplus
}
#endif
#endif
```

Before: 0.5582.

## Emit bitpacked top-k mask directly from fused colsum kernel and defer colsum store

Adds a packed-output mode to the fused dense-colsum top-k mask kernel, so the bool mask is written directly as bits via DPP lane combining. The separate bitpack pass and the full byte mask write/read are skipped on the default attention step path. It also moves the cross-wave column-sum LDS wait and partial store to the end of the phase (A64_CS_LATE) so LDS reads overlap more compute. This adds a new code path with alignment constraints (Nk multiple of 8) and more register pressure from carried csx values.

```diff
diff --git a/chipmunk_amd/_native.py b/chipmunk_amd/_native.py
--- a/chipmunk_amd/_native.py
+++ b/chipmunk_amd/_native.py
@@ -14,6 +14,7 @@
     "chipmunk_csp_mlp_mm2_and_scatter_add_ragged", "chipmunk_csp_scatter_add_ragged", "chipmunk_block_mean_ragged", "chipmunk_transpose16_pitched",
     "chipmunk_topk_indices", "chipmunk_topk_delta_indices", "chipmunk_topk_mask", "chipmunk_mask_to_indices", "chipmunk_mask_to_sorted_indices", "chipmunk_packed_mask_to_indices", "chipmunk_copy_indices",
     "chipmunk_bitpack", "chipmunk_bitunpack", "chipmunk_transpose16", "chipmunk_block_mean", "chipmunk_quantize_fp8", "chipmunk_gather_rows", "chipmunk_qkv_split_norm", "chipmunk_dense_colsum_topk_mask", "chipmunk_dense_attn_strided", "chipmunk_csp_attn_out_ragged", "chipmunk_compact_indices", "chipmunk_residual_ln_modulate", "chipmunk_dense_colsum_attn_strided", "chipmunk_dense_colsum_topk_mask_strided", "chipmunk_release_scratch", "chipmunk_big_scratch_fallbacks",
+    "chipmunk_topk_mask_packed", "chipmunk_dense_colsum_topk_mask_packed_strided",
     "chipmunk_host_alloc", "chipmunk_host_free", "chipmunk_copy_d2h_async", "chipmunk_copy_h2d_async", "chipmunk_host_bytes",
 ]
 
diff --git a/chipmunk_amd/csrc/attn.hip b/chipmunk_amd/csrc/attn.hip
--- a/chipmunk_amd/csrc/attn.hip
+++ b/chipmunk_amd/csrc/attn.hip
@@ -1238,18 +1238,18 @@
                                               cs_stride, stream);
 }
 
-extern "C" int chipmunk_dense_colsum_topk_mask_strided(const void *q, const void *k, const void *v, const int64_t q_strides[3],
-                                               const int64_t k_strides[3], const int64_t v_strides[3], const float *pin, void *o,
-                                               const int64_t *o_strides, float *l, int B, int H, int Nq, int Nk, const void *static_mask,
-                                               int64_t static_stride, int static_rows, const void *group_flags, void *mask,
-                                               int topk, double random_amount, void *stream) {
+static int dense_colsum_topk_mask_impl(const void *q, const void *k, const void *v, const int64_t q_strides[3],
+                                       const int64_t k_strides[3], const int64_t v_strides[3], const float *pin, void *o,
+                                       const int64_t *o_strides, float *l, int B, int H, int Nq, int Nk, const void *static_mask,
+                                       int64_t static_stride, int static_rows, const void *group_flags, void *mask, int packed,
+                                       int topk, double random_amount, void *stream) {
     if (int e = check_common(q, k, v, o, B, H, Nq, Nk)) return e;
     CM_CHECK(l && pin && mask, "dense_colsum_topk_mask: p / l / mask missing");
     if (int e = check_strides(q_strides, "q")) return e;
     if (int e = check_strides(k_strides, "k")) return e;
     if (int e = check_strides(v_strides, "v")) return e;
     hipStream_t st = (hipStream_t)stream;
-    if (!use_dense64(B, H, Nq, Nk) || chipmunk_get_option("attn_fused_colsum") == 2 || (Nk & 3) || Nk > 1024 * 120)
+    if (!use_dense64(B, H, Nq, Nk) || chipmunk_get_option("attn_fused_colsum") == 2 || (Nk & (packed ? 7 : 3)) || Nk > 1024 * 120)
         return CHIPMUNK_ERR_UNSUPPORTED;
     AttnParams p = {};
     p.q = (const uint16_t *)q, p.k = (const uint16_t *)k, p.v = (const uint16_t *)v, p.o = (uint16_t *)o;
@@ -1264,8 +1264,26 @@
     if (!part) return CHIPMUNK_ERR_UNSUPPORTED;
     if (int e = chipmunk_dense64_colsum_launch(p, part, st)) return e;
     const int nrb = ((Nq + 255) / 256) * 2;
-    return chipmunk_topk_mask_parts(part, chipmunk_colsum_part_stride(Nk), nrb, p.G, Nq, static_mask, static_stride, static_rows, group_flags, mask, B * H * p.G, Nk,
+    return chipmunk_topk_mask_parts(part, chipmunk_colsum_part_stride(Nk), nrb, p.G, Nq, static_mask, static_stride, static_rows, group_flags, mask, packed, B * H * p.G, Nk,
                                     topk, random_amount, st);
+}
+
+extern "C" int chipmunk_dense_colsum_topk_mask_strided(const void *q, const void *k, const void *v, const int64_t q_strides[3],
+                                               const int64_t k_strides[3], const int64_t v_strides[3], const float *pin, void *o,
+                                               const int64_t *o_strides, float *l, int B, int H, int Nq, int Nk, const void *static_mask,
+                                               int64_t static_stride, int static_rows, const void *group_flags, void *mask,
+                                               int topk, double random_amount, void *stream) {
+    return dense_colsum_topk_mask_impl(q, k, v, q_strides, k_strides, v_strides, pin, o, o_strides, l, B, H, Nq, Nk, static_mask, static_stride,
+                                       static_rows, group_flags, mask, 0, topk, random_amount, stream);
+}
+
+extern "C" int chipmunk_dense_colsum_topk_mask_packed_strided(const void *q, const void *k, const void *v, const int64_t q_strides[3],
+                                               const int64_t k_strides[3], const int64_t v_strides[3], const float *pin, void *o,
+                                               const int64_t *o_strides, float *l, int B, int H, int Nq, int Nk, const void *static_mask,
+                                               int64_t static_stride, int static_rows, const void *group_flags, void *packed,
+                                               int topk, double random_amount, void *stream) {
+    return dense_colsum_topk_mask_impl(q, k, v, q_strides, k_strides, v_strides, pin, o, o_strides, l, B, H, Nq, Nk, static_mask, static_stride,
+                                       static_rows, group_flags, packed, 1, topk, random_amount, stream);
 }
 
 extern "C" int chipmunk_dense_colsum_topk_mask(const void *q, const void *k, const void *v, const int64_t q_strides[3],
diff --git a/chipmunk_amd/csrc/attn64.hip b/chipmunk_amd/csrc/attn64.hip
--- a/chipmunk_amd/csrc/attn64.hip
+++ b/chipmunk_amd/csrc/attn64.hip
@@ -33,6 +33,9 @@
 #ifndef A64_VSPREAD
 #define A64_VSPREAD 0
 #endif
+#ifndef A64_CS_LATE
+#define A64_CS_LATE 1
+#endif
 #ifndef A64_DMA_POS
 #define A64_DMA_POS 2
 #endif
@@ -306,7 +309,7 @@
     float lacc[2][2] = {{0.f, 0.f}, {0.f, 0.f}};
     float alpha[2] = {1.f, 1.f};
     float wq[2] = {0.f, 0.f}, lpq[2] = {-1.0e30f, -1.0e30f}, c4[2] = {0.f, 0.f}, c5 = 0.f;
-    uint32_t csoff = 0, ex_w = 0, ex_r = 0;
+    uint32_t csoff = 0, ex_w = 0, ex_r1 = 0, ex_r2 = 0;
     int cs_extra = 0;
     float cs_own = 0.f;
     __amdgpu_buffer_rsrc_t prsrc = krsrc;
@@ -335,7 +338,8 @@
         const int lead = w < nA ? 0 : nA, members = w < nA ? nA : 4 - nA;
         cs_extra = w == lead ? members : 0;
         ex_w = lds0 + LDS_BYTES + (uint32_t)w * 256u + (uint32_t)lane * 4u;
-        ex_r = lds0 + LDS_BYTES + (uint32_t)(lead + 1) * 256u + (uint32_t)lane * 4u;
+        ex_r1 = lds0 + LDS_BYTES + (uint32_t)(cs_extra >= 2 ? lead + 1 : w) * 256u + (uint32_t)lane * 4u;
+        ex_r2 = lds0 + LDS_BYTES + (uint32_t)(cs_extra >= 3 ? lead + 2 : w) * 256u + (uint32_t)lane * 4u;
         prsrc = make_rsrc(p.cs_part + ((int64_t)bh * (p.G * 2) + (g * 2 + (w < nA ? 0 : 1))) * p.cs_pstride);
     }
 #pragma unroll
@@ -490,6 +494,19 @@
         bool moved = false;
         const int dead = GATHER ? 0 : (t * KT - tile_base(t) < KT ? t * KT - tile_base(t) : KT);
         const int vleft = !GATHER ? KT : (t < ntiles ? valid - (tbeg + t) * KT : 0);
+        float csx1, csx2;
+        auto cs_store = [&](auto uwt) __attribute__((always_inline)) {
+            const int tb2 = tile_base(t - 2), dd = (t - 2) * KT - tb2;
+            if (t > 1 && dd < KT) {
+                const uint32_t off = decltype(uwt)::value ? csoff_mx : csoff;
+                if (dd <= 0 || (int)(off >> 1) >= dd) {
+                    const float x1 = cs_extra >= 2 ? csx1 : 0.f, x2 = cs_extra >= 3 ? csx2 : 0.f;
+                    const uint16_t val = (uint16_t)(pack_bf16x2((cs_own + x1) + x2, 0.f) & 0xffffu);
+                    if (p.probe & 16) __builtin_amdgcn_raw_buffer_store_b16(val, prsrc, off, (uint32_t)tb2 * 2u, 2);
+                    else __builtin_amdgcn_raw_buffer_store_b16(val, prsrc, off, (uint32_t)tb2 * 2u, 0);
+                }
+            }
+        };
         auto phase_b_gap = [&](auto gg) __attribute__((always_inline)) {
             constexpr int G = decltype(gg)::value;
             constexpr int up = G >> 3, db = (G >> 1) & 3, qb = G & 1;
@@ -500,25 +517,14 @@
             if constexpr (CSUM && G == (UWT ? 31 : 17)) {
                 const uint32_t par2 = (uint32_t)(t & 1) * 1024u;
                 const float mine = UWT ? csout : c5;
-                if (!cs_extra) {
-                    asm volatile("ds_write_b32 %0, %1" ::"v"(ex_w + (par2 ^ 1024u)), "v"(mine) : "memory");
-                } else {
-                    float x1 = 0.f, x2 = 0.f;
-                    if (cs_extra >= 2) asm volatile("ds_read_b32 %0, %1" : "=v"(x1) : "v"(ex_r + par2) : "memory");
-                    if (cs_extra >= 3) asm volatile("ds_read_b32 %0, %1 offset:256" : "=v"(x2) : "v"(ex_r + par2) : "memory");
-                    asm volatile("ds_write_b32 %0, %1" ::"v"(ex_w + (par2 ^ 1024u)), "v"(mine) : "memory");
-                    asm volatile("s_waitcnt lgkmcnt(1)" : "+v"(x1), "+v"(x2)::"memory");
-                    const int tb2 = tile_base(t - 2), dd = (t - 2) * KT - tb2;
-                    if (t > 1 && dd < KT) {
-                        const uint32_t off = UWT ? csoff_mx : csoff;
-                        if (dd <= 0 || (int)(off >> 1) >= dd) {
-                            const uint16_t val = (uint16_t)(pack_bf16x2((cs_own + x1) + x2, 0.f) & 0xffffu);
-                            if (p.probe & 16) __builtin_amdgcn_raw_buffer_store_b16(val, prsrc, off, (uint32_t)tb2 * 2u, 2);
-                            else __builtin_amdgcn_raw_buffer_store_b16(val, prsrc, off, (uint32_t)tb2 * 2u, 0);
-                        }
-                    }
-                }
-                cs_own = mine;
+                asm volatile("ds_read_b32 %0, %1" : "=v"(csx1) : "v"(ex_r1 + par2) : "memory");
+                asm volatile("ds_read_b32 %0, %1" : "=v"(csx2) : "v"(ex_r2 + par2) : "memory");
+                asm volatile("ds_write_b32 %0, %1" ::"v"(ex_w + (par2 ^ 1024u)), "v"(mine) : "memory");
+                if constexpr (!A64_CS_LATE) {
+                    asm volatile("s_waitcnt lgkmcnt(1)" : "+v"(csx1), "+v"(csx2)::"memory");
+                    if (cs_extra) cs_store(ic<UWT ? 1 : 0>{});
+                    cs_own = mine;
+                }
             }
             if constexpr (!(A64_ABL & 16) && !GATHER && A64_DMA_POS == 1 && G >= 16 && (G & 1) == 0) {
                 constexpr int PC = (G - 16) >> 1;
@@ -610,7 +616,14 @@
             asm volatile("s_nop 7\n\ts_nop 7\n\ts_nop 7\n\t" A64_SCALE_QB0 : "=&v"(tmp) : "v"(alpha[0]));
             asm volatile(A64_SCALE_QB1 : "=&v"(tmp) : "v"(alpha[1]));
         }
-        asm volatile("s_waitcnt lgkmcnt(0)" ::: "memory");
+        if constexpr (CSUM && A64_CS_LATE) {
+            constexpr bool UWT = decltype(uwc)::value != 0 && !A64_CSUM_VALU;
+            asm volatile("s_waitcnt lgkmcnt(0)" : "+v"(csx1), "+v"(csx2)::"memory");
+            if (cs_extra) cs_store(ic<UWT ? 1 : 0>{});
+            cs_own = UWT ? csout : c5;
+        } else {
+            asm volatile("s_waitcnt lgkmcnt(0)" ::: "memory");
+        }
         __builtin_amdgcn_sched_barrier(0);
         P64_MARK(6);
     };
@@ -686,8 +699,8 @@
         if (cs_extra) {
             float x1 = 0.f, x2 = 0.f;
             const uint32_t par = (uint32_t)((T4 - 1) & 1) * 1024u;
-            if (cs_extra >= 2) asm volatile("ds_read_b32 %0, %1" : "=v"(x1) : "v"(ex_r + par) : "memory");
-            if (cs_extra >= 3) asm volatile("ds_read_b32 %0, %1 offset:256" : "=v"(x2) : "v"(ex_r + par) : "memory");
+            if (cs_extra >= 2) asm volatile("ds_read_b32 %0, %1" : "=v"(x1) : "v"(ex_r1 + par) : "memory");
+            if (cs_extra >= 3) asm volatile("ds_read_b32 %0, %1" : "=v"(x2) : "v"(ex_r2 + par) : "memory");
             asm volatile("s_waitcnt lgkmcnt(0)" : "+v"(x1), "+v"(x2)::"memory");
             const int tb1 = tile_base(T4 - 1), dd = (T4 - 1) * KT - tb1;
             const uint32_t off = (unitw && !A64_CSUM_VALU) ? csoff_mx : csoff;
diff --git a/chipmunk_amd/csrc/attn_params.h b/chipmunk_amd/csrc/attn_params.h
--- a/chipmunk_amd/csrc/attn_params.h
+++ b/chipmunk_amd/csrc/attn_params.h
@@ -30,7 +30,7 @@
 int chipmunk_csp64_launch(const AttnParams &p, int inplace, int grid, hipStream_t stream);
 int chipmunk_dense64_colsum_launch(const AttnParams &p, uint16_t *part, hipStream_t stream);
 int chipmunk_topk_mask_parts(const uint16_t *part, int part_stride, int nrb, int groups_per_bh, int Nq, const void *static_mask, int64_t static_stride,
-                             int static_rows, const void *group_flags, void *mask, int rows, int n, int k, double random_amount,
+                             int static_rows, const void *group_flags, void *mask, int packed, int rows, int n, int k, double random_amount,
                              hipStream_t stream);
 size_t chipmunk_colsum_part_bytes(int B, int H, int Nq, int Nk);
 int chipmunk_colsum_part_stride(int Nk);
diff --git a/chipmunk_amd/csrc/indexed_io.hip b/chipmunk_amd/csrc/indexed_io.hip
--- a/chipmunk_amd/csrc/indexed_io.hip
+++ b/chipmunk_amd/csrc/indexed_io.hip
@@ -497,6 +497,7 @@
     const uint8_t *stat;
     const uint8_t *groups;
     uint8_t *mask;
+    int packed;
     int64_t cs_stride, stat_stride;
     int rows, n, k, stat_rows;
     float random_amount;
@@ -646,7 +647,7 @@
         __syncthreads();
         tie_budget = ties_to_take - before;
     }
-    uint8_t *out = p.mask + (int64_t)row * n;
+    uint8_t *out = p.mask + (p.packed ? ((int64_t)row * n) >> 3 : (int64_t)row * n);
     const uint8_t *st = p.stat ? p.stat + (int64_t)(row % p.stat_rows) * p.stat_stride : nullptr;
     const bool rnd = active && p.random_amount > 0.f;
     auto combined4 = [&](int c0, uint32_t &v0, uint32_t &v1) {
@@ -671,7 +672,7 @@
     }
     const uint32_t salt = p.salt ^ (first * 0x27D4EB2Fu);
     const int nsteps = (n + 4095) / 4096;
-    auto emit = [&](auto keyed, int c, uint32_t v0, uint32_t v1, uint32_t sb) {
+    auto mask4 = [&](auto keyed, int c, uint32_t v0, uint32_t v1, uint32_t sb) {
         uint32_t bytes = 0;
         if constexpr (decltype(keyed)::value) asm volatile("" : "+v"(v0), "+v"(v1));
 #pragma unroll
@@ -686,8 +687,25 @@
             keep = keep || ((sb >> (8 * e)) & 0xffu) != 0;
             bytes |= (keep ? 1u : 0u) << (8 * e);
         }
+        return bytes;
+    };
+    auto put4 = [&](int c, uint32_t bytes) {
         if constexpr (ALIGNED) {
-            *(uint32_t *)(out + c) = bytes;
+            if (p.packed) {
+                const uint32_t b4 = bytes * 0x00204081u >> 21 & 0xfu;
+                uint32_t qd = b4 << (4 * (lane & 3));
+                qd |= (uint32_t)__builtin_amdgcn_update_dpp(0, (int)qd, 0xB1, 0xf, 0xf, true);
+                qd |= (uint32_t)__builtin_amdgcn_update_dpp(0, (int)qd, 0x4E, 0xf, 0xf, true);
+                if (c < n) {
+                    if ((n & 15) == 0) {
+                        if ((lane & 3) == 0) *(uint16_t *)(out + (c >> 3)) = (uint16_t)qd;
+                    } else if ((lane & 1) == 0) {
+                        out[c >> 3] = (uint8_t)(qd >> (4 * (lane & 3)));
+                    }
+                }
+            } else if (c < n) {
+                *(uint32_t *)(out + c) = bytes;
+            }
         } else {
 #pragma unroll
             for (int e = 0; e < 4; ++e)
@@ -709,7 +727,11 @@
             for (int jj = 0; jj < OB; ++jj) {
                 if constexpr (true) {
                     const int c = 4 * tid + 4096 * (j0 + jj);
-                    if (j0 + jj < NV && c < n) emit(std::integral_constant<int, 1>{}, c, key[(j0 + jj) < NV ? (j0 + jj) : 0][0], key[(j0 + jj) < NV ? (j0 + jj) : 0][1], sbv[jj]);
+                    if (j0 + jj < NV) {
+                        uint32_t bytes = 0;
+                        if (c < n) bytes = mask4(std::integral_constant<int, 1>{}, c, key[(j0 + jj) < NV ? (j0 + jj) : 0][0], key[(j0 + jj) < NV ? (j0 + jj) : 0][1], sbv[jj]);
+                        put4(c, bytes);
+                    }
                     asm volatile("" ::: "memory");
                 }
             }
@@ -727,7 +749,7 @@
                 else v1 |= u << (16 * (e - 2));
                 if (st && c + e < n) sb |= (uint32_t)st[c + e] << (8 * e);
             }
-            emit(std::integral_constant<int, 0>{}, c, v0, v1, sb);
+            put4(c, mask4(std::integral_constant<int, 0>{}, c, v0, v1, sb));
         }
     }
 }
@@ -884,14 +906,15 @@
 }
 
 int chipmunk_topk_mask_parts(const uint16_t *part, int part_stride, int nrb, int groups_per_bh, int Nq, const void *static_mask, int64_t static_stride,
-                             int static_rows, const void *group_flags, void *mask, int rows, int n, int k, double random_amount,
+                             int static_rows, const void *group_flags, void *mask, int packed, int rows, int n, int k, double random_amount,
                              hipStream_t s) {
+    CM_CHECK(!packed || (n & 7) == 0, "topk_mask_parts: the packed mask needs n % 8 == 0 (got %d)", n);
     CM_CHECK(part && mask && rows >= 0 && n > 0 && (n & 3) == 0 && n <= 1024 * 120 && k >= 0 && part_stride >= n && (part_stride & 3) == 0, "topk_mask_parts: bad arguments");
     CM_CHECK(!static_mask || (static_rows > 0 && static_stride >= n && (static_stride & 3) == 0 && ((uintptr_t)static_mask & 3) == 0),
              "topk_mask_parts: bad static mask geometry");
     CM_CHECK(((uintptr_t)mask & 3) == 0 && ((uintptr_t)part & 7) == 0, "topk_mask_parts: unaligned buffers");
     if (rows == 0) return CHIPMUNK_OK;
-    TopkMaskParams p = {nullptr, (const uint8_t *)static_mask, (const uint8_t *)group_flags, (uint8_t *)mask, 0, static_stride,
+    TopkMaskParams p = {nullptr, (const uint8_t *)static_mask, (const uint8_t *)group_flags, (uint8_t *)mask, packed, 0, static_stride,
                         rows, n, k, static_mask ? static_rows : 1, (float)random_amount,
                         random_amount > 0.0 ? chipmunk_next_random_salt() : 0u};
     p.parts = part, p.pstride = part_stride, p.nrb = nrb, p.ngroups = groups_per_bh, p.nq = Nq;
@@ -966,9 +989,8 @@
     return CHIPMUNK_OK;
 }
 
-extern "C" int chipmunk_topk_mask(const void *cs, int64_t cs_stride, const void *static_mask, int64_t static_stride,
-                                  int static_rows, const void *group_flags, void *mask, int rows, int n, int k,
-                                  double random_amount, void *stream) {
+static int topk_mask_launch(const void *cs, int64_t cs_stride, const void *static_mask, int64_t static_stride, int static_rows,
+                            const void *group_flags, void *mask, int packed, int rows, int n, int k, double random_amount, void *stream) {
     CM_CHECK(cs && mask, "topk_mask: null pointer");
     CM_CHECK(rows >= 0 && n > 0 && k >= 0, "topk_mask: bad sizes (rows=%d n=%d k=%d)", rows, n, k);
     CM_CHECK(cs_stride >= n, "topk_mask: cs row stride %lld < n %d", (long long)cs_stride, n);
@@ -976,12 +998,13 @@
     CM_CHECK(!static_mask || (static_rows > 0 && static_stride >= n), "topk_mask: bad static mask geometry");
     CM_CHECK(random_amount >= 0.0 && random_amount <= 1.0, "topk_mask: random_amount must be in [0,1]");
     if (rows == 0) return CHIPMUNK_OK;
-    TopkMaskParams p = {(const uint16_t *)cs, (const uint8_t *)static_mask, (const uint8_t *)group_flags, (uint8_t *)mask,
+    TopkMaskParams p = {(const uint16_t *)cs, (const uint8_t *)static_mask, (const uint8_t *)group_flags, (uint8_t *)mask, packed,
                         cs_stride, static_stride, rows, n, k, static_mask ? static_rows : 1, (float)random_amount,
                         random_amount > 0.0 ? chipmunk_next_random_salt() : 0u};
     hipStream_t s = (hipStream_t)stream;
     const bool aligned = n % 4 == 0 && (((uintptr_t)cs) & 7) == 0 && (cs_stride * 2) % 8 == 0 && (((uintptr_t)mask) & 3) == 0 &&
                          (!static_mask || ((((uintptr_t)static_mask) & 3) == 0 && static_stride % 4 == 0));
+    CM_CHECK(!packed || (aligned && n % 8 == 0), "topk_mask_packed: needs n %% 8 == 0 and 8 / 4-byte aligned cs / static mask rows (n=%d)", n);
 #define LAUNCH_TM(KPT)                                                                                       \
     do {                                                                                                     \
         if (aligned) hipLaunchKernelGGL((topk_mask_kernel<KPT, true>), dim3(rows), dim3(1024), 0, s, p);     \
@@ -995,6 +1018,18 @@
     return CHIPMUNK_OK;
 }
 
+extern "C" int chipmunk_topk_mask(const void *cs, int64_t cs_stride, const void *static_mask, int64_t static_stride,
+                                  int static_rows, const void *group_flags, void *mask, int rows, int n, int k,
+                                  double random_amount, void *stream) {
+    return topk_mask_launch(cs, cs_stride, static_mask, static_stride, static_rows, group_flags, mask, 0, rows, n, k, random_amount, stream);
+}
+
+extern "C" int chipmunk_topk_mask_packed(const void *cs, int64_t cs_stride, const void *static_mask, int64_t static_stride,
+                                         int static_rows, const void *group_flags, void *packed, int rows, int n, int k,
+                                         double random_amount, void *stream) {
+    return topk_mask_launch(cs, cs_stride, static_mask, static_stride, static_rows, group_flags, packed, 1, rows, n, k, random_amount, stream);
+}
+
 extern "C" int chipmunk_compact_indices(const int32_t *indices, int64_t idx_stride, const int32_t *counts, const int64_t *offsets,
                                         int32_t *flat, int64_t rows, void *stream) {
     CM_CHECK(indices && counts && offsets && flat, "compact_indices: null pointer");
diff --git a/chipmunk_amd/csrc/torch_registry.cpp b/chipmunk_amd/csrc/torch_registry.cpp
--- a/chipmunk_amd/csrc/torch_registry.cpp
+++ b/chipmunk_amd/csrc/torch_registry.cpp
@@ -599,10 +599,11 @@
 
 std::vector<at::Tensor> dense_colsum_attn_layout(at::Tensor q, at::Tensor k, at::Tensor v, at::Tensor p, bool token_major_o);
 at::Tensor topk_mask(at::Tensor cs, int64_t k, double random_amount, const c10::optional<at::Tensor> &groups,
-                     const c10::optional<at::Tensor> &static_mask);
+                     const c10::optional<at::Tensor> &static_mask, bool packed);
+at::Tensor bitpack(at::Tensor mask);
 std::vector<at::Tensor> dense_colsum_topk_mask(at::Tensor q, at::Tensor k, at::Tensor v, at::Tensor p, int64_t k_top, double random_amount,
                                                const c10::optional<at::Tensor> &groups, const c10::optional<at::Tensor> &static_mask,
-                                               bool token_major_o) {
+                                               bool token_major_o, bool packed) {
     CHECK_DEV(q); CHECK_DEV(k); CHECK_DEV(v); CHECK_DEV(p);
     CHECK_BF16(q); CHECK_BF16(k); CHECK_BF16(v);
     const bool shapes_ok = q.dim() == 4 && k.dim() == 4 && v.dim() == 4 && q.size(3) == 128 && q.stride(3) == 1 && k.stride(3) == 1 &&
@@ -629,17 +630,19 @@
                 gf = gfc.data_ptr();
             }
         }
+        if (ok && packed) ok = Nk % 8 == 0;
         if (ok) {
             c10::DeviceGuard guard(q.device());
             at::Tensor o = alloc_o(q, q, token_major_o);
             const int64_t os[3] = {o.stride(0), o.stride(1), o.stride(2)};
             at::Tensor l = at::empty({B, H, Nq, 1}, q.options().dtype(at::kFloat));
-            at::Tensor mask = at::empty({B, H, G, Nk}, q.options().dtype(at::kBool));
+            at::Tensor mask = packed ? at::empty({B * H * G * Nk / 8}, q.options().dtype(at::kByte))
+                                     : at::empty({B, H, G, Nk}, q.options().dtype(at::kBool));
             const int64_t qs[3] = {q.stride(0), q.stride(1), q.stride(2)}, ks[3] = {k.stride(0), k.stride(1), k.stride(2)},
                           vs[3] = {v.stride(0), v.stride(1), v.stride(2)};
-            const int rc = chipmunk_dense_colsum_topk_mask_strided(q.data_ptr(), k.data_ptr(), v.data_ptr(), qs, ks, vs, p.data_ptr<float>(), o.data_ptr(),
-                                                           os, l.data_ptr<float>(), (int)B, (int)H, (int)Nq, (int)Nk, st, st_stride, (int)st_rows, gf,
-                                                           mask.data_ptr(), (int)k_top, random_amount, cur_stream(q));
+            const int rc = (packed ? chipmunk_dense_colsum_topk_mask_packed_strided : chipmunk_dense_colsum_topk_mask_strided)(
+                q.data_ptr(), k.data_ptr(), v.data_ptr(), qs, ks, vs, p.data_ptr<float>(), o.data_ptr(), os, l.data_ptr<float>(), (int)B, (int)H,
+                (int)Nq, (int)Nk, st, st_stride, (int)st_rows, gf, mask.data_ptr(), (int)k_top, random_amount, cur_stream(q));
             if (rc == CHIPMUNK_OK) return {o, mask, l};
             if (rc != CHIPMUNK_ERR_UNSUPPORTED) check(rc, "dense_colsum_topk_mask");
         }
@@ -648,18 +651,17 @@
     at::Tensor cs = ocl[1];
     const int64_t Nk = k.size(2), G = (q.size(2) + 191) / 192;
     if (cs.size(-1) != Nk || cs.size(-2) != G) cs = cs.slice(-2, 0, G).slice(-1, 0, Nk);
-    return {ocl[0], topk_mask(cs, k_top, random_amount, groups, static_mask), ocl[2]};
+    return {ocl[0], topk_mask(cs, k_top, random_amount, groups, static_mask, packed), ocl[2]};
 }
 
 at::Tensor topk_mask(at::Tensor cs, int64_t k, double random_amount, const c10::optional<at::Tensor> &groups,
-                     const c10::optional<at::Tensor> &static_mask) {
+                     const c10::optional<at::Tensor> &static_mask, bool packed) {
     CHECK_DEV(cs); CHECK_BF16(cs);
     TORCH_CHECK(cs.dim() == 4 && cs.stride(3) == 1, "cs must be [B, H, G, N] with a contiguous last dim");
     const int64_t B = cs.size(0), H = cs.size(1), G = cs.size(2), N = cs.size(3);
     if (!(cs.stride(1) == G * cs.stride(2) && (B == 1 || cs.stride(0) == H * cs.stride(1)))) cs = cs.contiguous();
     const int64_t rows = B * H * G;
     c10::DeviceGuard guard(cs.device());
-    at::Tensor mask = at::empty({B, H, G, N}, cs.options().dtype(at::kBool));
     const void *st = nullptr, *gf = nullptr;
     int64_t st_stride = 0, st_rows = 1;
     at::Tensor stc, gfc;
@@ -680,10 +682,20 @@
         gfc = gfc.expand({B, H, G, 1}).contiguous();
         gf = gfc.data_ptr();
     }
+    const bool bits = packed && N % 8 == 0 && (uintptr_t)cs.data_ptr() % 8 == 0 && cs.stride(2) % 4 == 0 &&
+                      (!st || ((uintptr_t)st % 4 == 0 && st_stride % 4 == 0));
+    if (bits) {
+        at::Tensor out = at::empty({rows * N / 8}, cs.options().dtype(at::kByte));
+        check(chipmunk_topk_mask_packed(cs.data_ptr(), cs.stride(2), st, st_stride, (int)st_rows, gf, out.data_ptr(), (int)rows, (int)N,
+                                        (int)k, random_amount, cur_stream(cs)),
+              "topk_mask_packed");
+        return out;
+    }
+    at::Tensor mask = at::empty({B, H, G, N}, cs.options().dtype(at::kBool));
     check(chipmunk_topk_mask(cs.data_ptr(), cs.stride(2), st, st_stride, (int)st_rows, gf, mask.data_ptr(), (int)rows, (int)N,
                              (int)k, random_amount, cur_stream(cs)),
           "topk_mask");
-    return mask;
+    return packed ? bitpack(mask) : mask;
 }
 
 at::Tensor bitpack(at::Tensor mask) {
@@ -779,8 +791,8 @@
     m.def("topk_delta_indices(Tensor activation, Tensor(cache!) cache, Tensor(indices!) indices, Tensor(counts!) counts, float sparsity_amount, int multiple_of, float random_amount) -> ()");
     m.def("packed_mask_to_indices(Tensor packed, int[] shape, int multiple_of, int pad_to_multiple_of) -> Tensor[]");
     m.def("mask_to_sorted_indices(Tensor mask, int[] shape, int multiple_of, int pad_to_multiple_of) -> Tensor[]");
-    m.def("topk_mask(Tensor cs, int k, float random_amount, Tensor? groups, Tensor? static_mask) -> Tensor");
-    m.def("dense_colsum_topk_mask(Tensor q, Tensor k, Tensor v, Tensor p, int k_top, float random_amount, Tensor? groups, Tensor? static_mask, bool token_major_o=False) -> Tensor[]");
+    m.def("topk_mask(Tensor cs, int k, float random_amount, Tensor? groups, Tensor? static_mask, bool packed=False) -> Tensor");
+    m.def("dense_colsum_topk_mask(Tensor q, Tensor k, Tensor v, Tensor p, int k_top, float random_amount, Tensor? groups, Tensor? static_mask, bool token_major_o=False, bool packed=False) -> Tensor[]");
     m.def("dense_attn_layout(Tensor q, Tensor k, Tensor v, bool token_major_o) -> Tensor[]");
     m.def("dense_colsum_attn_layout(Tensor q, Tensor k, Tensor v, Tensor p, bool token_major_o) -> Tensor[]");
     m.def("compact_indices(Tensor indices, Tensor counts) -> Tensor[]");
diff --git a/chipmunk_amd/modules/attn.py b/chipmunk_amd/modules/attn.py
--- a/chipmunk_amd/modules/attn.py
+++ b/chipmunk_amd/modules/attn.py
@@ -163,11 +163,15 @@
             if inference_step == 1 or cfg["recompute_mask"]:
                 prev_lse = self.storage.get_lse_constants()
                 tk = int(multiple_of * round((cfg["top_keys"] * k.shape[-2]) / multiple_of))
-                mask = bs = None
+                mask = bs = packed_mask = None
                 if (q.is_cuda and cfg["should_compress_indices"] and tk > 0 and amd_key("attn", "fused_colsum_topk")
                         and amd_key("attn", "fused_topk_mask") and k.shape[-2] <= 122880):
                     static, groups = self._static(q.shape[1], _cdiv(q.shape[-2], bm), k.shape[-2])
-                    o, mask, lse = ops.dense_colsum_topk_mask(q, k, v, prev_lse, tk, 0.01, groups, static, tm)
+                    if (amd_key("attn", "packed_mask_step") and k.shape[-2] % 8 == 0 and amd_key("attn", "fused_packed_mask_to_indices")
+                            and amd_key("attn", "sorted_indices")):
+                        o, packed_mask, lse = ops.dense_colsum_topk_mask(q, k, v, prev_lse, tk, 0.01, groups, static, tm, True)
+                    else:
+                        o, mask, lse = ops.dense_colsum_topk_mask(q, k, v, prev_lse, tk, 0.01, groups, static, tm)
                 elif do_padding:
                     o, bs, lse = ops.dense_colsum_attn(q, k, v, prev_lse, tm)
                 else:
@@ -176,16 +180,18 @@
                 lse[..., k.shape[-2]:, :] = 0
                 self.storage.set_lse_constants(lse)
                 if cfg["should_compress_indices"]:
-                    if mask is not None:
+                    if mask is not None or packed_mask is not None:
                         pass
                     elif tk > 0:
                         mask = self.random_and_topk(bs, tk)
                     else:
                         mask = self._static(bs.shape[1], bs.shape[-2], bs.shape[-1])[0]
-                    packed, mask_shape = ops.bitpack(mask)
+                    packed, mask_shape = packed_mask if packed_mask is not None else ops.bitpack(mask)
                     self.mask_shape[self.layer_counter.cur_model_invocation_per_step] = mask_shape
                     self.storage.set_indices(packed)
-                    if mask.is_cuda and amd_key("attn", "fused_packed_mask_to_indices") and amd_key("attn", "sorted_indices"):
+                    if packed_mask is not None:
+                        inds, counts = ops.mask_to_sorted_indices(packed, mask_shape, multiple_of, bm)
+                    elif mask.is_cuda and amd_key("attn", "fused_packed_mask_to_indices") and amd_key("attn", "sorted_indices"):
                         inds, counts = ops.mask_to_sorted_indices(mask, mask.shape, multiple_of, bm)
                     else:
                         inds, counts = ops.mask_to_indices(mask, multiple_of, bm)
diff --git a/chipmunk_amd/ops/_fake.py b/chipmunk_amd/ops/_fake.py
--- a/chipmunk_amd/ops/_fake.py
+++ b/chipmunk_amd/ops/_fake.py
@@ -60,7 +60,9 @@
         return [packed.new_empty((b, h, m, pad_n), dtype=torch.int32), packed.new_empty((b, h, m), dtype=torch.int32)]
 
     @lib.register_fake("chipmunk::topk_mask")
-    def _(cs, k, random_amount, groups, static_mask):
+    def _(cs, k, random_amount, groups, static_mask, packed=False):
+        if packed:
+            return cs.new_empty(((cs.numel() + 7) // 8,), dtype=torch.uint8)
         return cs.new_empty(cs.shape, dtype=torch.bool)
 
     @lib.register_fake("chipmunk::block_mean")
@@ -94,10 +96,12 @@
         return src.new_empty(shape)
 
     @lib.register_fake("chipmunk::dense_colsum_topk_mask")
-    def _(q, k, v, p, k_top, random_amount, groups, static_mask, token_major_o=False):
+    def _(q, k, v, p, k_top, random_amount, groups, static_mask, token_major_o=False, packed=False):
         B, H, Nq, D = q.shape
         G = (Nq + 191) // 192
-        return [_o_like(q, token_major_o), q.new_empty((B, H, G, k.shape[2]), dtype=torch.bool),
+        mask = (q.new_empty(((B * H * G * k.shape[2] + 7) // 8,), dtype=torch.uint8) if packed else
+                q.new_empty((B, H, G, k.shape[2]), dtype=torch.bool))
+        return [_o_like(q, token_major_o), mask,
                 q.new_empty((B, H, Nq, 1), dtype=torch.float32)]
 
     @lib.register_fake("chipmunk::qkv_split_norm")
diff --git a/chipmunk_amd/ops/attn.py b/chipmunk_amd/ops/attn.py
--- a/chipmunk_amd/ops/attn.py
+++ b/chipmunk_amd/ops/attn.py
@@ -47,15 +47,17 @@
 
 
 def dense_colsum_topk_mask(q: torch.Tensor, k: torch.Tensor, v: torch.Tensor, p: torch.Tensor, k_top: int, random_amount: float,
-                           groups, static_mask, token_major_o: bool = False) -> Tuple[torch.Tensor, torch.Tensor, torch.Tensor]:
+                           groups, static_mask, token_major_o: bool = False, packed: bool = False):
     n = q.shape[-2]
     padded = _pad_len(n)
     assert p.shape[-2] in (n, padded), "p must be the l vector of the previous full step"
     o, mask, l = torch.ops.chipmunk.dense_colsum_topk_mask(_last_dim_contiguous(q), _last_dim_contiguous(k), _last_dim_contiguous(v),
                                                            p[..., :n, :].contiguous(), k_top, random_amount, groups, static_mask,
-                                                           token_major_o)
+                                                           token_major_o, packed)
     if padded != n:
         l = F.pad(l, (0, 0, 0, padded - n))
+    if packed:
+        mask = (mask, torch.Size((q.shape[0], q.shape[1], (n + PM - 1) // PM, k.shape[-2])))
     return o, mask, l
 
 
diff --git a/chipmunk_amd/ops/indexed_io.py b/chipmunk_amd/ops/indexed_io.py
--- a/chipmunk_amd/ops/indexed_io.py
+++ b/chipmunk_amd/ops/indexed_io.py
@@ -35,7 +35,9 @@
 
 
 def topk_mask(cs: torch.Tensor, k: int, random_amount: float = 0.0, groups: Optional[torch.Tensor] = None,
-              static_mask: Optional[torch.Tensor] = None) -> torch.Tensor:
+              static_mask: Optional[torch.Tensor] = None, packed: bool = False):
+    if packed:
+        return torch.ops.chipmunk.topk_mask(cs, k, random_amount, groups, static_mask, True), cs.shape
     return torch.ops.chipmunk.topk_mask(cs, k, random_amount, groups, static_mask)
 
 
diff --git a/chipmunk_amd/util/config.py b/chipmunk_amd/util/config.py
--- a/chipmunk_amd/util/config.py
+++ b/chipmunk_amd/util/config.py
@@ -74,6 +74,7 @@
     "mlp.fused_fp8_quantize": True,
     "attn.fused_residual": True,
     "attn.fused_topk_mask": True,
+    "attn.packed_mask_step": True,
     "attn.fused_colsum_topk": True,
     "mlp.fused_scatter": True,
     "attn.token_major_output": False,
@@ -90,6 +91,7 @@
 BASE_CONFIG["attn"]["fused_residual"] = AMD_EXTRA_KEYS["attn.fused_residual"]
 BASE_CONFIG["attn"]["fused_topk_mask"] = AMD_EXTRA_KEYS["attn.fused_topk_mask"]
 BASE_CONFIG["attn"]["fused_colsum_topk"] = AMD_EXTRA_KEYS["attn.fused_colsum_topk"]
+BASE_CONFIG["attn"]["packed_mask_step"] = AMD_EXTRA_KEYS["attn.packed_mask_step"]
 BASE_CONFIG["mlp"]["fused_scatter"] = AMD_EXTRA_KEYS["mlp.fused_scatter"]
 BASE_CONFIG["attn"]["token_major_output"] = AMD_EXTRA_KEYS["attn.token_major_output"]
 BASE_CONFIG["attn"]["keep_unpacked_indices"] = AMD_EXTRA_KEYS["attn.keep_unpacked_indices"]
diff --git a/include/chipmunk_hip.h b/include/chipmunk_hip.h
--- a/include/chipmunk_hip.h
+++ b/include/chipmunk_hip.h
@@ -57,6 +57,12 @@
                                             const int64_t *o_strides, float *l, int B, int H, int Nq, int Nk,
                                             const void *static_mask, int64_t static_stride, int static_rows,
                                             const void *group_flags, void *mask, int k_top, double random_amount, void *stream);
+int chipmunk_dense_colsum_topk_mask_packed_strided(const void *q, const void *k, const void *v, const int64_t q_strides[3],
+                                                   const int64_t k_strides[3], const int64_t v_strides[3], const float *p, void *o,
+                                                   const int64_t *o_strides, float *l, int B, int H, int Nq, int Nk,
+                                                   const void *static_mask, int64_t static_stride, int static_rows,
+                                                   const void *group_flags, void *packed, int k_top, double random_amount,
+                                                   void *stream);
 
 int chipmunk_dense_colsum_attn(const void *q, const void *k, const void *v, const int64_t q_strides[3],
                                const int64_t k_strides[3], const int64_t v_strides[3], const float *p, void *o,
@@ -116,6 +122,9 @@
 int chipmunk_topk_mask(const void *cs, int64_t cs_stride, const void *static_mask, int64_t static_stride,
                        int static_rows, const void *group_flags, void *mask, int rows, int n, int k,
                        double random_amount, void *stream);
+int chipmunk_topk_mask_packed(const void *cs, int64_t cs_stride, const void *static_mask, int64_t static_stride,
+                              int static_rows, const void *group_flags, void *packed, int rows, int n, int k,
+                              double random_amount, void *stream);
 
 int chipmunk_mask_to_indices(const void *mask, int32_t *indices, int32_t *counts, int64_t rows, int n, int pad_n,
                              int multiple_of, void *stream);
```

After: 0.5589, median of 2. About the same (+0.1%).
